# robin-karlsson0/ViT-Adapter

Hardware: AMD Instinct MI355X
Metric: images/sec ViT-Adapter-B 1024x1024 fwd+bwd (+AdamW step) (higher is better)
Workload: dtype bf16; 1 GPU; ViT-Adapter-base_det (det) 1024x1024, per-GPU batch 2, train mode, drop_path 0.3, SyncBN, step = fwd+bwd+AdamW; global_batch=2, parallelism=dp1, hip_graph=True, rccl_ranks=1, gemm_candidates_rejected=0

## Files before the change

vit-adapter_amd/_vah.py:

```python
import ctypes
import os

import torch

_HERE = os.path.dirname(os.path.abspath(__file__))
LIB_PATH = os.path.join(_HERE, 'lib', 'libvitadapter_hip.so')
ABI_VERSION = 37

if not os.path.exists(LIB_PATH):
    raise ImportError(
        'libvitadapter_hip.so is missing (%s): build it with `python vit-adapter_amd/build.py` '
        '(hipcc --offload-arch=gfx950).  There is no CPU or PyTorch fallback.' % LIB_PATH)

lib = ctypes.CDLL(LIB_PATH)

_int, _i64, _f, _p, _str, _pi64 = (ctypes.c_int, ctypes.c_int64, ctypes.c_float, ctypes.c_void_p, ctypes.c_char_p,
                                   ctypes.POINTER(ctypes.c_int64))

SIGNATURES = {
    'vah_abi_version': (_int, []),
    'vah_last_error': (_str, []),
    'vah_msda_forward_f32': (_int, [_p, _p, _p, _p, _p, _i64, _i64, _i64, _i64, _i64, _i64, _i64, _p, _p]),
    'vah_msda_forward_f64': (_int, [_p, _p, _p, _p, _p, _i64, _i64, _i64, _i64, _i64, _i64, _i64, _p, _p]),
    'vah_msda_backward_f32': (_int, [_p, _p, _p, _p, _p, _p, _i64, _i64, _i64, _i64, _i64, _i64, _i64, _p, _p, _p, _p]),
# ... 54 lines not shown
    'vah_conv_taps_nhwc_bf16': (_int, [_p, _i64, _i64, _i64, _i64, _p, _i64, _int, _p, _p, _int, _p, _i64, _i64, _i64, _i64, _int, _int, _int, _p]),
    'vah_conv3x3_dgrad_nhwc_bf16': (_int, [_p, _i64, _i64, _i64, _i64, _p, _i64, _int, _p, _i64, _i64, _p]),
    'vah_conv3x3_wgrad_ws_floats': (_i64, [_i64, _i64]),
    'vah_conv3x3_wgrad_nhwc_bf16': (_int, [_p, _i64, _i64, _i64, _i64, _p, _i64, _i64, _i64, _int, _p, _i64, _p, _p]),
    'vah_image_to_nhwc16_bf16': (_int, [_p, _i64, _i64, _i64, _p, _p]),
    'vah_patchify_bf16': (_int, [_p, _i64, _i64, _i64, _i64, _i64, _p, _p]),
    'vah_bn_nhwc_ws_floats': (_i64, [_i64]),
    'vah_bn_nhwc_stats': (_int, [_p, _i64, _i64, _p, _p, _p]),
    'vah_bn_nhwc_apply': (_int, [_p, _i64, _i64, _p, _p, _p, _p, _int, _p, _p]),
    'vah_bn_nhwc_bwd_stats': (_int, [_p, _p, _i64, _i64, _p, _p, _p, _p, _int, _p, _p, _p]),
    'vah_bn_nhwc_bwd_apply': (_int, [_p, _p, _i64, _i64, _p, _p, _p, _p, _int, _p, _p, _p, _p]),
    'vah_maxpool3s2_nhwc_fwd_bf16': (_int, [_p, _i64, _i64, _i64, _i64, _p, _p, _p]),
    'vah_maxpool3s2_nhwc_bwd_bf16': (_int, [_p, _p, _i64, _i64, _i64, _i64, _p, _p]),
    'vah_gemm_set_tuning': (_int, [_int, _int]),
    'vah_gemm_bf16': (_int, [_int, _int, _i64, _i64, _i64, _p, _i64, _p, _i64, _p, _i64, _int, _int, _p, _int, _p, _i64, _p]),
    'vah_gemm_bf16_fin': (_int, [_int, _int, _i64, _i64, _i64, _p, _i64, _p, _i64, _p, _i64, _int, _p, _i64, _p, _i64, _i64, _p, _p]),
    'vah_gemm_library_version': (_i64, []),
    'vah_gemm_rejected_candidates': (_i64, []),
    'vah_gemm_table_dump': (_i64, [_str, _i64]),
    'vah_gemm_table_load': (_int, [_str]),
    'vah_scale_residual_fwd': (_int, [_p, _p, _p, _p, _i64, _i64, _i64, _p, _p]),
    'vah_scale_residual_bwd': (_int, [_p, _p, _p, _p, _i64, _i64, _i64, _p, _p, _p, _p]),
    'vah_dwconv3x3_tokens_bf16': (_int, [_p, _p, _p, _i64, _i64, _i64, _i64, _int, _p, _p]),
    'vah_dwconv3x3_tokens_wgrad_bf16': (_int, [_p, _p, _i64, _i64, _i64, _i64, _p, _p, _p, _p]),
    'vah_prof_enable': (_int, [_int]),
    'vah_prof_filter': (_int, [_str]),
    'vah_prof_report': (_i64, [_str, _i64]),
}

ATTN_F16_TWINS = {
    'vah_attn_fwd_bf16': 'vah_attn_fwd_f16', 'vah_attn_bwd_bf16': 'vah_attn_bwd_f16',
    'vah_attn_win_fwd_bf16': 'vah_attn_win_fwd_f16', 'vah_attn_win_bwd_bf16': 'vah_attn_win_bwd_f16',
    'vah_attn_bias_fwd_bf16': 'vah_attn_bias_fwd_f16', 'vah_attn_bias_bwd_bf16': 'vah_attn_bias_bwd_f16',
    'vah_relpos_bias_build': 'vah_relpos_bias_build_f16', 'vah_relpos_bias_grad': 'vah_relpos_bias_grad_f16',
}
FUSED_F16_TWINS = {
    'vah_layernorm_fwd_f32_bf16': 'vah_layernorm_fwd_f32_f16', 'vah_layernorm_bwd_f32_bf16': 'vah_layernorm_bwd_f32_f16',
    'vah_residual_layernorm_fwd': 'vah_residual_layernorm_fwd_f16', 'vah_residual_layernorm_bwd': 'vah_residual_layernorm_bwd_f16',
    'vah_layernorm_dual_fwd': 'vah_layernorm_dual_fwd_f16', 'vah_layernorm_dual_bwd': 'vah_layernorm_dual_bwd_f16',
    'vah_scale_residual_fwd': 'vah_scale_residual_fwd_f16', 'vah_scale_residual_bwd': 'vah_scale_residual_bwd_f16',
    'vah_dwconv3x3_tokens_bf16': 'vah_dwconv3x3_tokens_f16', 'vah_dwconv3x3_tokens_wgrad_bf16': 'vah_dwconv3x3_tokens_wgrad_f16',
}
LINEAR_F16_TWINS = {
    'vah_gemm_bf16': 'vah_gemm_f16', 'vah_gemm_bf16_fin': 'vah_gemm_f16_fin',
    'vah_colsum_bf16': 'vah_colsum_f16', 'vah_colsum_bf16_partials': 'vah_colsum_f16_partials',
    'vah_gelu_bwd_bsum_bf16': 'vah_gelu_bwd_bsum_f16',
    'vah_residual_layernorm_bwd_bsum': 'vah_residual_layernorm_bwd_f16_bsum',
    'vah_scale_residual_bwd_bsum': 'vah_scale_residual_bwd_f16_bsum',
}
SPM_F16_TWINS = {
    'vah_conv_taps_nhwc_bf16': 'vah_conv_taps_nhwc_f16', 'vah_conv3x3_dgrad_nhwc_bf16': 'vah_conv3x3_dgrad_nhwc_f16',
    'vah_conv3x3_wgrad_nhwc_bf16': 'vah_conv3x3_wgrad_nhwc_f16', 'vah_image_to_nhwc16_bf16': 'vah_image_to_nhwc16_f16',
    'vah_bn_nhwc_stats': 'vah_bn_nhwc_stats_f16', 'vah_bn_nhwc_apply': 'vah_bn_nhwc_apply_f16',
    'vah_bn_nhwc_bwd_stats': 'vah_bn_nhwc_bwd_stats_f16', 'vah_bn_nhwc_bwd_apply': 'vah_bn_nhwc_bwd_apply_f16',
    'vah_maxpool3s2_nhwc_fwd_bf16': 'vah_maxpool3s2_nhwc_fwd_f16', 'vah_maxpool3s2_nhwc_bwd_bf16': 'vah_maxpool3s2_nhwc_bwd_f16',
}
TAIL_F16_TWINS = {
    'vah_bn_tail_stats': 'vah_bn_tail_stats_f16', 'vah_bn_tail_apply': 'vah_bn_tail_apply_f16',
    'vah_bn_tail_bwd_stats': 'vah_bn_tail_bwd_stats_f16', 'vah_bn_tail_bwd_apply': 'vah_bn_tail_bwd_apply_f16',
    'vah_transpose_tokens': 'vah_transpose_tokens_f16', 'vah_maxpool3s2_fwd_bf16': 'vah_maxpool3s2_fwd_f16',
    'vah_maxpool3s2_bwd_bf16': 'vah_maxpool3s2_bwd_f16', 'vah_pixel_shuffle2_bf16': 'vah_pixel_shuffle2_f16',
}
F16_TWINS = {**ATTN_F16_TWINS, **FUSED_F16_TWINS, **LINEAR_F16_TWINS, **SPM_F16_TWINS, **TAIL_F16_TWINS}

EXPORTS = tuple(SIGNATURES) + tuple(F16_TWINS.values())

_PARENT = {f16: b16 for b16, f16 in F16_TWINS.items()}
for _name in EXPORTS:
    _fn = getattr(lib, _name)
    _fn.restype, _fn.argtypes = SIGNATURES[_PARENT.get(_name, _name)]

BOX_SIGNATURES = {
    'vah_msda_fused_forward_box': (_int, [_p, _int, _p, _p, _p, _p, _int, _i64, _i64, _p, _i64, _i64, _i64, _i64, _i64, _i64, _i64, _i64, _i64,
                                          _i64, _p, _p]),
    'vah_msda_fused_backward_tiled_box': (_int, [_p, _int, _p, _p, _p, _p, _int, _i64, _i64, _p, _i64, _i64, _i64, _p, _i64, _i64, _i64, _i64, _i64,
                                                 _i64, _i64, _p, _int, _p, _p, _int, _i64, _i64, _p, _i64, _p]),
}
for _name, (_res, _args) in BOX_SIGNATURES.items():
    _fn = getattr(lib, _name)
    _fn.restype, _fn.argtypes = _res, _args

_t = [_p, _int, _i64, _i64]
GN_SIGNATURES = {
    'vah_group_norm_supported': (_int, [_i64, _i64]),
    'vah_group_norm_ws_floats': (_i64, [_i64, _i64, _i64, _i64]),
    'vah_group_norm_stats': (_int, _t + [_i64, _i64, _i64, _i64, _f, _p, _p, _p, _i64, _p]),
    'vah_group_norm_apply': (_int, _t + [_i64, _i64, _i64, _i64, _p, _p, _p, _p, _int, _p] + _t + [_p]),
    'vah_group_norm_bwd_stats': (_int, _t + _t + [_i64, _i64, _i64, _i64, _p, _p, _p, _p, _int, _p, _p, _p, _p, _i64, _p]),
    'vah_group_norm_bwd_apply': (_int, _t + _t + [_i64, _i64, _i64, _i64, _p, _p, _p, _p, _int, _p] + _t + [_p]),
}
for _name, (_res, _args) in GN_SIGNATURES.items():
    _fn = getattr(lib, _name)
    _fn.restype, _fn.argtypes = _res, _args

RESIZE_SIGNATURES = {
    'vah_resize_rows_ws_bytes': (_i64, [_i64, _i64, _i64, _i64]),
    'vah_resize_rows_forward': (_int, _t + [_i64, _i64, _i64, _i64, _i64, _i64, _int] + _t + [_p, _i64, _p]),
    'vah_resize_rows_backward': (_int, _t + [_i64, _i64, _i64, _i64, _i64, _i64, _int] + _t + [_p, _i64, _p]),
}
for _name, (_res, _args) in RESIZE_SIGNATURES.items():
    _fn = getattr(lib, _name)
    _fn.restype, _fn.argtypes = _res, _args

_mca_dims = [_i64, _i64, _i64, _i64, _i64, _f]
MCA_SIGNATURES = {
    'vah_mca_splits': (_i64, [_i64]),
    'vah_mca_ws_bytes': (_i64, [_i64, _i64, _i64, _i64]),
    'vah_mca_pack_mask': (_int, _t + [_i64, _i64, _i64, _p, _p]),
    'vah_mca_forward': (_int, _t + _t + _t + [_p] + _mca_dims + _t + [_p, _p, _i64, _p]),
    'vah_mca_backward': (_int, _t + _t + _t + [_p] + _t + _t + [_p] + _mca_dims + _t + _t + _t + [_p, _i64, _p]),
}
for _name, (_res, _args) in MCA_SIGNATURES.items():
    _fn = getattr(lib, _name)
    _fn.restype, _fn.argtypes = _res, _args

POINTS_SIGNATURES = {
    'vah_pts_sample': (_int, [_p, _int, _i64, _i64, _i64, _i64, _i64, _p, _i64, _i64, _p, _p, _i64, _p, _p]),
    'vah_pts_match_cost': (_int, [_p, _p, _p, _p, _p, _i64, _i64, _i64, _i64, _i64, _i64, _f, _f, _f, _f, _p, _p]),
}
for _name, (_res, _args) in POINTS_SIGNATURES.items():
    _fn = getattr(lib, _name)
    _fn.restype, _fn.argtypes = _res, _args

PML_SIGNATURES = {
    'vah_pml_ws_bytes': (_i64, [_i64, _i64, _i64, _i64]),
    'vah_pml_forward': (_int, [_p, _i64, _i64, _i64, _i64, _i64, _p, _int, _i64, _i64, _i64, _i64, _i64, _p, _i64, _p, _p, _i64, _f,
                               _p, _p, _p, _p, _p, _p, _i64, _p]),
    'vah_pml_backward': (_int, [_p, _p, _p, _p, _p, _p, _i64, _i64, _i64, _i64, _f, _p, _p, _i64, _p]),
}
for _name, (_res, _args) in PML_SIGNATURES.items():
    _fn = getattr(lib, _name)
    _fn.restype, _fn.argtypes = _res, _args

_pl = [_p, _i64, _i64, _i64]
SEG_SIGNATURES = {
    'vah_seg_resize_add': (_int, _pl + [_i64, _i64, _i64, _i64, _i64, _i64, _int] + _pl + [_i64, _i64, _i64, _i64, _int, _p]),
    'vah_seg_finish': (_int, _pl + [_i64, _i64, _i64, _i64, _p, _p, _int, _i64, _i64, _int, _int] + _pl + [_int, _p, _i64, _i64, _p]),
    'vah_seg_argmax': (_int, _pl + [_i64, _i64, _i64, _i64, _f, _p, _i64, _i64, _p]),
}
for _name, (_res, _args) in SEG_SIGNATURES.items():
    _fn = getattr(lib, _name)
    _fn.restype, _fn.argtypes = _res, _args

_sce = [_p, _int, _i64, _i64, _i64, _i64, _i64, _i64, _i64, _p, _i64, _i64, _i64, _i64, _int, _i64, _p]
SCE_SIGNATURES = {
    'vah_sce_ws_bytes': (_i64, [_i64, _i64, _i64, _i64, _i64, _i64]),
    'vah_sce_forward': (_int, _sce + [_p, _p, _p, _p, _i64, _p]),
    'vah_sce_backward': (_int, _sce + [_p, _p] + _pl + [_p, _i64, _p]),
}
for _name, (_res, _args) in SCE_SIGNATURES.items():
    _fn = getattr(lib, _name)
    _fn.restype, _fn.argtypes = _res, _args

if lib.vah_abi_version() != ABI_VERSION:
    raise ImportError('libvitadapter_hip.so ABI %d != binding ABI %d: rebuild the library'
                      % (lib.vah_abi_version(), ABI_VERSION))


class _NoSwitch:

    def __enter__(self):
        return None

    def __exit__(self, *exc):
        return False


_NO_SWITCH = _NoSwitch()


def on(device):
    import torch
    if device.index is None or torch.cuda.current_device() == device.index:
        return _NO_SWITCH
    return torch.cuda.device(device)


def raw_stream(device):
    import torch
    idx = device.index if device.index is not None else torch.cuda.current_device()
    try:
        return torch._C._cuda_getCurrentRawStream(idx)
    except AttributeError:
        return torch.cuda.current_stream(device).cuda_stream


def check(rc, what):
    if rc != 0:
        msg = lib.vah_last_error().decode('utf-8', 'replace')
        raise RuntimeError('%s failed (code %d): %s' % (what, rc, msg))


_SYM = {(b16, torch.bfloat16): getattr(lib, b16) for b16 in SIGNATURES}
_SYM.update(((b16, torch.float16), getattr(lib, f16)) for b16, f16 in F16_TWINS.items())


def sym(name, dtype):
    try:
        return _SYM[name, dtype]
    except KeyError:
        raise ValueError('no entry point %s for %s operands' % (name, dtype)) from None


def call(name, dtype, *args):
    fn = sym(name, dtype)
    check(fn(*args), fn.__name__)


def prof_enable(on, prefix=''):
    lib.vah_prof_filter(prefix.encode())
    lib.vah_prof_enable(1 if on else 0)


def prof_report():
    need = lib.vah_prof_report(None, 0)
    buf = ctypes.create_string_buffer(int(need) + 64)
    lib.vah_prof_report(buf, len(buf))
    out = {}
    for line in buf.value.decode().splitlines():
        name, calls, ms, nbytes, dbytes, flops = line.split()
        out[name] = dict(calls=int(calls), total_ms=float(ms), bytes=int(nbytes), def_bytes=int(dbytes),
                         flops=int(flops))
    return out


GEMM_EPI_NONE, GEMM_EPI_BIAS = 0, 1


def gemm_table_dump():
    n = lib.vah_gemm_table_dump(None, 0)
    buf = ctypes.create_string_buffer(int(n))
    lib.vah_gemm_table_dump(buf, n)
    return '#hipblaslt %d\n' % lib.vah_gemm_library_version() + buf.value.decode()


def gemm_table_load(text):
    first = text.split('\n', 1)[0].split()
    if len(first) == 2 and first[0] == '#hipblaslt' and int(first[1]) != lib.vah_gemm_library_version():
        return 0
    n = lib.vah_gemm_table_load(text.encode())
    if n < 0:
        check(n, 'gemm_table_load')
    return n
```

vit-adapter_amd/csrc/gemm.hip:

```cpp
#include <hip/hip_runtime.h>
#include <hipblaslt/hipblaslt-ext.hpp>
#include <hipblaslt/hipblaslt.h>

#include <algorithm>
#include <cstdio>
#include <cstdlib>
#include <cstring>
#include <map>
#include <memory>
#include <mutex>
#include <sstream>
#include <string>
#include <tuple>
#include <type_traits>
#include <vector>

#include "../../include/vitadapter_hip.h"
#include "common.h"

namespace vah {
namespace {

struct Key {
    int f16;
    int ta, tb, d32, epi, bias32;
    int64_t M, N, K, lda, ldb, ldd;
    bool operator<(const Key &o) const {
        return std::tie(f16, ta, tb, d32, epi, bias32, M, N, K, lda, ldb, ldd) <
               std::tie(o.f16, o.ta, o.tb, o.d32, o.epi, o.bias32, o.M, o.N, o.K, o.lda, o.ldb, o.ldd);
    }
    hipDataType t16() const { return f16 ? HIP_R_16F : HIP_R_16BF; }
};

struct Choice {
    hipblasLtMatmulAlgo_t algo;
    size_t workspace = 0;
    int index = -1;
    int split = 1;
    float us = 0.f;
    bool resolved = false;
};

struct Problem;
struct State {
    std::mutex mu;
    hipblasLtHandle_t handle = nullptr;
    std::map<Key, Choice> table;
    std::map<Key, std::shared_ptr<Problem>> problems;
    int mode = 1;
    int candidates = 32;
    void *probe = nullptr;
    int rejected = 0;
};

State &state() {
    static State s;
    return s;
}

const char *status_name(hipblasStatus_t s) {
    switch (s) {
    case HIPBLAS_STATUS_SUCCESS: return "success";
    case HIPBLAS_STATUS_NOT_INITIALIZED: return "not initialized";
    case HIPBLAS_STATUS_ALLOC_FAILED: return "alloc failed";
    case HIPBLAS_STATUS_INVALID_VALUE: return "invalid value";
    case HIPBLAS_STATUS_NOT_SUPPORTED: return "not supported";
    case HIPBLAS_STATUS_EXECUTION_FAILED: return "execution failed";
    default: return "error";
    }
}

struct Problem {
    hipblasLtMatmulDesc_t desc = nullptr;
    hipblasLtMatrixLayout_t la = nullptr, lb = nullptr, ld = nullptr;
    ~Problem() {
        if (la) hipblasLtMatrixLayoutDestroy(la);
        if (lb) hipblasLtMatrixLayoutDestroy(lb);
        if (ld) hipblasLtMatrixLayoutDestroy(ld);
        if (desc) hipblasLtMatmulDescDestroy(desc);
    }
};

struct Call {
    Key k;
    const void *A, *B, *bias;
    void *D;
    void *ws;
    size_t ws_bytes;
    hipStream_t st;
    const float *fin_part = nullptr;
    int fin_nparts = 0, fin_C = 0;
    float *fin_out = nullptr;
    const float *ref = nullptr;
};

hipblasStatus_t make_problem(const Call &c, Problem &p, int split) {
    const Key &k0 = c.k;
    Key k = k0;
    k.K = k0.K / split;
    if (split > 1) {
        k.d32 = 1;
        k.ldd = k0.N;
    }
    hipblasStatus_t s = hipblasLtMatmulDescCreate(&p.desc, HIPBLAS_COMPUTE_32F, HIP_R_32F);
    if (s != HIPBLAS_STATUS_SUCCESS) return s;
    const hipblasOperation_t op1 = k.tb ? HIPBLAS_OP_T : HIPBLAS_OP_N, op2 = k.ta ? HIPBLAS_OP_T : HIPBLAS_OP_N;
    hipblasLtMatmulDescSetAttribute(p.desc, HIPBLASLT_MATMUL_DESC_TRANSA, &op1, sizeof(op1));
    hipblasLtMatmulDescSetAttribute(p.desc, HIPBLASLT_MATMUL_DESC_TRANSB, &op2, sizeof(op2));
    s = hipblasLtMatrixLayoutCreate(&p.la, k.t16(), k.tb ? k.K : k.N, k.tb ? k.N : k.K, k.ldb);
    if (s != HIPBLAS_STATUS_SUCCESS) return s;
    s = hipblasLtMatrixLayoutCreate(&p.lb, k.t16(), k.ta ? k.M : k.K, k.ta ? k.K : k.M, k.lda);
    if (s != HIPBLAS_STATUS_SUCCESS) return s;
    s = hipblasLtMatrixLayoutCreate(&p.ld, k.d32 ? HIP_R_32F : k.t16(), k.N, k.M, k.ldd);
    if (s != HIPBLAS_STATUS_SUCCESS) return s;
    if (split > 1) {
        const int32_t batch = split;
        const int64_t sa = k.ta ? k.K * k.lda : k.K, sb = k.tb ? k.K : k.K * k.ldb, sd = k.M * k.N;
        hipblasLtMatrixLayoutSetAttribute(p.la, HIPBLASLT_MATRIX_LAYOUT_BATCH_COUNT, &batch, sizeof(batch));
        hipblasLtMatrixLayoutSetAttribute(p.lb, HIPBLASLT_MATRIX_LAYOUT_BATCH_COUNT, &batch, sizeof(batch));
        hipblasLtMatrixLayoutSetAttribute(p.ld, HIPBLASLT_MATRIX_LAYOUT_BATCH_COUNT, &batch, sizeof(batch));
        hipblasLtMatrixLayoutSetAttribute(p.la, HIPBLASLT_MATRIX_LAYOUT_STRIDED_BATCH_OFFSET, &sb, sizeof(sb));
        hipblasLtMatrixLayoutSetAttribute(p.lb, HIPBLASLT_MATRIX_LAYOUT_STRIDED_BATCH_OFFSET, &sa, sizeof(sa));
        hipblasLtMatrixLayoutSetAttribute(p.ld, HIPBLASLT_MATRIX_LAYOUT_STRIDED_BATCH_OFFSET, &sd, sizeof(sd));
    }
    uint32_t epi = HIPBLASLT_EPILOGUE_DEFAULT;
    switch (k.epi) {
    case VAH_GEMM_EPI_NONE: break;
    case VAH_GEMM_EPI_BIAS: epi = HIPBLASLT_EPILOGUE_BIAS; break;
    default: return HIPBLAS_STATUS_INVALID_VALUE;
    }
    hipblasLtMatmulDescSetAttribute(p.desc, HIPBLASLT_MATMUL_DESC_EPILOGUE, &epi, sizeof(epi));
    if (c.bias) {
        hipblasLtMatmulDescSetAttribute(p.desc, HIPBLASLT_MATMUL_DESC_BIAS_POINTER, &c.bias, sizeof(c.bias));
        const int32_t bt = k.bias32 ? HIP_R_32F : k.t16();
        hipblasLtMatmulDescSetAttribute(p.desc, HIPBLASLT_MATMUL_DESC_BIAS_DATA_TYPE, &bt, sizeof(bt));
    }
    return HIPBLAS_STATUS_SUCCESS;
}

size_t partial_bytes(const Key &k, int split) {
    return split > 1 ? ((size_t)split * k.M * k.N * sizeof(float) + 255) / 256 * 256 : 0;
}

template <int G, bool FIRST>
__device__ __forceinline__ void add_slices(const float *__restrict__ p, int64_t MN, float4 &acc) {
    float4 v[G];
#pragma unroll
    for (int u = 0; u < G; ++u) v[u] = *reinterpret_cast<const float4 *>(p + u * MN);
#pragma unroll
    for (int u = 0; u < G; ++u) {
        if (FIRST && u == 0) {
            acc = v[0];
        } else {
            acc.x += v[u].x;
            acc.y += v[u].y;
            acc.z += v[u].z;
            acc.w += v[u].w;
        }
    }
}

template <typename OT>
__global__ __launch_bounds__(256) void reduce_splits(const float *__restrict__ part, int split, int64_t MN, int N,
                                                     int64_t ldd, int vec, OT *__restrict__ out, int reduce_blocks,
                                                     const float *__restrict__ fin_part, int fin_nparts, int fin_C,
                                                     float *__restrict__ fin_out) {
    if ((int)blockIdx.x >= reduce_blocks) {
        __shared__ float s_acc[8][32];
        const int col = threadIdx.x & 31, pl = threadIdx.x >> 5;
        const int k = ((int)blockIdx.x - reduce_blocks) * 32 + col;
        float a8[8] = {0.f, 0.f, 0.f, 0.f, 0.f, 0.f, 0.f, 0.f};
        if (k < fin_C) {
            int p = pl;
            for (; p + 56 < fin_nparts; p += 64) {
#pragma unroll
                for (int u = 0; u < 8; ++u) a8[u] += fin_part[(int64_t)(p + 8 * u) * fin_C + k];
            }
            for (; p < fin_nparts; p += 8) a8[0] += fin_part[(int64_t)p * fin_C + k];
        }
        s_acc[pl][col] = ((a8[0] + a8[1]) + (a8[2] + a8[3])) + ((a8[4] + a8[5]) + (a8[6] + a8[7]));
        __syncthreads();
        if (pl == 0 && k < fin_C) {
            float t = 0.f;
#pragma unroll
            for (int u = 0; u < 8; ++u) t += s_acc[u][col];
            fin_out[k] = t;
        }
        return;
    }
    for (int64_t i = ((int64_t)blockIdx.x * 256 + threadIdx.x) * 4; i < MN; i += (int64_t)reduce_blocks * 1024) {
        const float *p = part + i;
        float4 acc;
        int s;
        if (split >= 8) {
            add_slices<8, true>(p, MN, acc);
            s = 8;
        } else if (split >= 4) {
            add_slices<4, true>(p, MN, acc);
            s = 4;
        } else if (split >= 2) {
            add_slices<2, true>(p, MN, acc);
            s = 2;
        } else {
            add_slices<1, true>(p, MN, acc);
            s = 1;
        }
        for (; s + 8 <= split; s += 8) add_slices<8, false>(p + s * MN, MN, acc);
        if (s + 4 <= split) {
            add_slices<4, false>(p + s * MN, MN, acc);
            s += 4;
        }
        if (s + 2 <= split) {
            add_slices<2, false>(p + s * MN, MN, acc);
            s += 2;
        }
        if (s < split) add_slices<1, false>(p + s * MN, MN, acc);
        int64_t o = i;
        if (ldd != N) {
            const int64_t row = i / N;
            o = row * ldd + (i - row * N);
        }
        typedef OT ov4 __attribute__((ext_vector_type(4)));
        ov4 r;
        r[0] = (OT)acc.x;
        r[1] = (OT)acc.y;
        r[2] = (OT)acc.z;
        r[3] = (OT)acc.w;
        if (vec) {
            *reinterpret_cast<ov4 *>(out + o) = r;
        } else {
            out[o] = r[0];
            out[o + 1] = r[1];
            out[o + 2] = r[2];
            out[o + 3] = r[3];
        }
    }
}

template <typename T>
__global__ __launch_bounds__(256) void ref_gemm(int ta, int tb, int M, int N, int K, const T *__restrict__ A, int64_t lda,
                                                const T *__restrict__ B, int64_t ldb, const void *__restrict__ bias,
                                                int bias32, float *__restrict__ ref) {
    __shared__ float sa[16][65], sb[16][65];
    const int tm = blockIdx.y * 64, tn = blockIdx.x * 64;
    const int tx = threadIdx.x & 15, ty = threadIdx.x >> 4;
    float acc[4][4] = {};
    for (int k0 = 0; k0 < K; k0 += 16) {
        for (int i = threadIdx.x; i < 1024; i += 256) {
            const int ma = ta ? (i & 63) : (i >> 4), ka = ta ? (i >> 6) : (i & 15);
            const int m = tm + ma, k = k0 + ka;
            sa[ka][ma] = (m < M && k < K) ? (float)(ta ? A[(int64_t)k * lda + m] : A[(int64_t)m * lda + k]) : 0.f;
            const int nb = tb ? (i >> 4) : (i & 63), kb = tb ? (i & 15) : (i >> 6);
            const int n = tn + nb, k2 = k0 + kb;
            sb[kb][nb] = (n < N && k2 < K) ? (float)(tb ? B[(int64_t)n * ldb + k2] : B[(int64_t)k2 * ldb + n]) : 0.f;
        }
        __syncthreads();
#pragma unroll
        for (int kk = 0; kk < 16; ++kk) {
            float a[4], b[4];
#pragma unroll
            for (int i = 0; i < 4; ++i) {
                a[i] = sa[kk][ty * 4 + i];
                b[i] = sb[kk][tx * 4 + i];
            }
#pragma unroll
            for (int i = 0; i < 4; ++i)
#pragma unroll
                for (int j = 0; j < 4; ++j) acc[i][j] += a[i] * b[j];
        }
        __syncthreads();
    }
    for (int i = 0; i < 4; ++i)
        for (int j = 0; j < 4; ++j) {
            const int m = tm + ty * 4 + i, n = tn + tx * 4 + j;
            if (m >= M || n >= N) continue;
            float v = acc[i][j];
            if (bias) v += bias32 ? ((const float *)bias)[n] : (float)((const T *)bias)[n];
            ref[(int64_t)m * N + n] = v;
        }
}

template <typename OT>
__global__ __launch_bounds__(256) void full_compare(const OT *__restrict__ D, int64_t ldd, int64_t MN, int N,
                                                    const float *__restrict__ ref, unsigned *__restrict__ out2) {
    float md = 0.f, mr = 0.f;
    bool bad = false;
    for (int64_t i = (int64_t)blockIdx.x * 256 + threadIdx.x; i < MN; i += (int64_t)gridDim.x * 256) {
        const int64_t r = i / N;
        float v = (float)D[r * ldd + (i - r * N)];
        const float w = ref[i];
        if constexpr (std::is_same<OT, _Float16>::value) {
            if (isinf(v)) v = v == (float)(_Float16)w ? w : copysignf(65520.f, v);
        }
        const float d = fabsf(v - w);
        bad = bad || !(d == d);
        md = fmaxf(md, d == d ? d : 0.f);
        mr = fmaxf(mr, fabsf(w));
    }
    if (bad || md > 0.f) atomicMax(out2, __float_as_uint(bad ? INFINITY : md));
    if (mr > 0.f) atomicMax(out2 + 1, __float_as_uint(mr));
}

float *make_reference(const Call &c) {
    const Key &k = c.k;
    if (k.M > (64 << 16) || k.N > (int64_t)INT32_MAX || k.K > (int64_t)INT32_MAX) return nullptr;
    float *ref = nullptr;
    if (hipMalloc((void **)&ref, (size_t)k.M * k.N * sizeof(float)) != hipSuccess) return nullptr;
    const dim3 grid((unsigned)((k.N + 63) / 64), (unsigned)((k.M + 63) / 64));
    if (k.f16)
        hipLaunchKernelGGL(ref_gemm<_Float16>, grid, dim3(256), 0, c.st, k.ta, k.tb, (int)k.M, (int)k.N, (int)k.K,
                           (const _Float16 *)c.A, k.lda, (const _Float16 *)c.B, k.ldb, c.bias, k.bias32, ref);
    else
        hipLaunchKernelGGL(ref_gemm<__bf16>, grid, dim3(256), 0, c.st, k.ta, k.tb, (int)k.M, (int)k.N, (int)k.K,
                           (const __bf16 *)c.A, k.lda, (const __bf16 *)c.B, k.ldb, c.bias, k.bias32, ref);
    if (hipGetLastError() != hipSuccess) {
        (void)hipFree(ref);
        return nullptr;
    }
    return ref;
}

hipblasStatus_t run(State &S, const Call &c, Problem &p, const hipblasLtMatmulAlgo_t &algo, size_t ws_need, int split);

bool validate(State &S, const Call &c, Problem &p, const hipblasLtMatmulAlgo_t &algo, size_t ws_need, int split, const float *ref) {
    if (!ref) return true;
    if (!S.probe && hipMalloc(&S.probe, 2 * sizeof(unsigned)) != hipSuccess) return true;
    unsigned *out2 = (unsigned *)S.probe;
    const Key &k = c.k;
    const size_t es = k.d32 ? 4 : 2;
    const int64_t MN = k.M * k.N;
    const unsigned blocks = (unsigned)std::min<int64_t>(4096, (MN + 255) / 256);
    if (c.ws_bytes && hipMemsetAsync(c.ws, 0x01, c.ws_bytes, c.st) != hipSuccess) return true;
    for (int pass = 0; pass < 2; ++pass) {
        if (hipMemsetAsync(out2, 0, 8, c.st) != hipSuccess) return true;
        if (hipMemset2DAsync(c.D, (size_t)k.ldd * es, 0xFF, (size_t)k.N * es, (size_t)k.M, c.st) != hipSuccess) return true;
        if (run(S, c, p, algo, ws_need, split) != HIPBLAS_STATUS_SUCCESS) return false;
        if (k.d32)
            hipLaunchKernelGGL(full_compare<float>, dim3(blocks), dim3(256), 0, c.st, (const float *)c.D, k.ldd, MN, (int)k.N, ref, out2);
        else if (k.f16)
            hipLaunchKernelGGL(full_compare<_Float16>, dim3(blocks), dim3(256), 0, c.st, (const _Float16 *)c.D, k.ldd, MN, (int)k.N, ref, out2);
        else
            hipLaunchKernelGGL(full_compare<__bf16>, dim3(blocks), dim3(256), 0, c.st, (const __bf16 *)c.D, k.ldd, MN, (int)k.N, ref, out2);
        float h[2] = {0.f, 0.f};
        if (hipMemcpyAsync(h, out2, 8, hipMemcpyDeviceToHost, c.st) != hipSuccess || hipStreamSynchronize(c.st) != hipSuccess) return true;
        if (!(h[0] <= 0.015625f * fmaxf(h[1], 1e-20f))) return false;
    }
    return true;
}

hipblasStatus_t run(State &S, const Call &c, Problem &p, const hipblasLtMatmulAlgo_t &algo, size_t ws_need, int split) {
    const size_t pb = partial_bytes(c.k, split);
    if (pb + ws_need > c.ws_bytes) return HIPBLAS_STATUS_ALLOC_FAILED;
    const float alpha = 1.f, beta = 0.f;
    void *d = split > 1 ? c.ws : c.D;
    const hipblasStatus_t s = hipblasLtMatmul(S.handle, p.desc, &alpha, c.B, p.la, c.A, p.lb, &beta, d, p.ld, d, p.ld, &algo,
                                              (char *)c.ws + pb, c.ws_bytes - pb, c.st);
    if (s != HIPBLAS_STATUS_SUCCESS) return s;
    const bool fin = c.fin_part != nullptr;
    if (split == 1 && !fin) return s;
    const int64_t MN = c.k.M * c.k.N;
    const unsigned rblocks = split > 1 ? (unsigned)std::min<int64_t>(8192, (MN / 4 + 255) / 256) : 0u;
    const unsigned fblocks = fin ? (unsigned)((c.fin_C + 31) / 32) : 0u;
    const int vec = c.k.N % 4 == 0 && c.k.ldd % 4 == 0 && (uintptr_t)c.D % (c.k.d32 ? 16 : 8) == 0;
    if (c.k.d32)
        hipLaunchKernelGGL(reduce_splits<float>, dim3(rblocks + fblocks), dim3(256), 0, c.st, (const float *)c.ws, split, MN,
                           (int)c.k.N, c.k.ldd, vec, (float *)c.D, (int)rblocks, c.fin_part, c.fin_nparts, c.fin_C, c.fin_out);
    else if (c.k.f16)
        hipLaunchKernelGGL(reduce_splits<_Float16>, dim3(rblocks + fblocks), dim3(256), 0, c.st, (const float *)c.ws, split, MN,
                           (int)c.k.N, c.k.ldd, vec, (_Float16 *)c.D, (int)rblocks, c.fin_part, c.fin_nparts, c.fin_C, c.fin_out);
    else
        hipLaunchKernelGGL(reduce_splits<__bf16>, dim3(rblocks + fblocks), dim3(256), 0, c.st, (const float *)c.ws, split, MN,
                           (int)c.k.N, c.k.ldd, vec, (__bf16 *)c.D, (int)rblocks, c.fin_part, c.fin_nparts, c.fin_C, c.fin_out);
    return HIPBLAS_STATUS_SUCCESS;
}

float time_algo(State &S, const Call &c, Problem &p, const hipblasLtMatmulAlgo_t &algo, size_t ws_need, int split,
                hipEvent_t e0, hipEvent_t e1, int reps) {
    if (run(S, c, p, algo, ws_need, split) != HIPBLAS_STATUS_SUCCESS) return -1.f;
    if (hipEventRecord(e0, c.st) != hipSuccess) return -1.f;
    for (int i = 0; i < reps; ++i)
        if (run(S, c, p, algo, ws_need, split) != HIPBLAS_STATUS_SUCCESS) return -1.f;
    if (hipEventRecord(e1, c.st) != hipSuccess || hipEventSynchronize(e1) != hipSuccess) return -1.f;
    float ms = 0.f;
    if (hipEventElapsedTime(&ms, e0, e1) != hipSuccess) return -1.f;
    return ms * 1000.f / reps;
}

hipblasStatus_t choose_for_split(State &S, const Call &c, Problem &p, int split, bool must_time, Choice &out) {
    const size_t pb = partial_bytes(c.k, split);
    if (pb >= c.ws_bytes) return HIPBLAS_STATUS_ALLOC_FAILED;
    const size_t ws_lib = c.ws_bytes - pb;
    std::vector<hipblasLtMatmulHeuristicResult_t> cand;
    const bool d32 = split > 1 || c.k.d32;
    if (S.mode == 2) {
        std::vector<hipblasLtMatmulHeuristicResult_t> all;
        const Key &k = c.k;
        hipblasStatus_t s = hipblaslt_ext::getAllAlgos(
            S.handle, hipblaslt_ext::GemmType::HIPBLASLT_GEMM, k.tb ? HIPBLAS_OP_T : HIPBLAS_OP_N,
            k.ta ? HIPBLAS_OP_T : HIPBLAS_OP_N, k.t16(), k.t16(), d32 ? HIP_R_32F : k.t16(),
            d32 ? HIP_R_32F : k.t16(), HIPBLAS_COMPUTE_32F, all);
        if (s == HIPBLAS_STATUS_SUCCESS)
            for (auto &r : all) {
                size_t need = 0;
                const float one = 1.f, zero = 0.f;
                if (hipblaslt_ext::matmulIsAlgoSupported(S.handle, p.desc, &one, p.la, p.lb, &zero, p.ld, p.ld, r.algo,
                                                         need) == HIPBLAS_STATUS_SUCCESS &&
                    need <= ws_lib) {
                    r.workspaceSize = need;
                    cand.push_back(r);
                }
            }
    }
    if (cand.empty()) {
        hipblasLtMatmulPreference_t pref = nullptr;
        hipblasStatus_t s = hipblasLtMatmulPreferenceCreate(&pref);
        if (s != HIPBLAS_STATUS_SUCCESS) return s;
        const uint64_t wsmax = ws_lib;
        hipblasLtMatmulPreferenceSetAttribute(pref, HIPBLASLT_MATMUL_PREF_MAX_WORKSPACE_BYTES, &wsmax, sizeof(wsmax));
        const int want = S.mode == 0 ? 1 : (split > 1 ? std::min(S.candidates, 12) : S.candidates);
        cand.resize(want);
        int got = 0;
        s = hipblasLtMatmulAlgoGetHeuristic(S.handle, p.desc, p.la, p.lb, p.ld, p.ld, pref, want, cand.data(), &got);
        hipblasLtMatmulPreferenceDestroy(pref);
        if (s != HIPBLAS_STATUS_SUCCESS) return s;
        cand.resize(std::max(got, 0));
        if (cand.empty()) return HIPBLAS_STATUS_NOT_SUPPORTED;
    }
    out.split = split;
    if (S.mode == 0 || (cand.size() == 1 && !must_time)) {
        if (!validate(S, c, p, cand[0].algo, cand[0].workspaceSize, split, c.ref)) {
            ++S.rejected;
            return HIPBLAS_STATUS_EXECUTION_FAILED;
        }
        out.algo = cand[0].algo;
        out.workspace = cand[0].workspaceSize;
        out.index = hipblaslt_ext::getIndexFromAlgo(out.algo);
        out.resolved = true;
        return HIPBLAS_STATUS_SUCCESS;
    }
    hipEvent_t e0, e1;
    if (hipEventCreate(&e0) != hipSuccess || hipEventCreate(&e1) != hipSuccess) return HIPBLAS_STATUS_ALLOC_FAILED;
    float best = -1.f;
    size_t best_i = 0;
    std::vector<std::pair<float, size_t>> timed;
    for (size_t i = 0; i < cand.size(); ++i) {
        const float us = time_algo(S, c, p, cand[i].algo, cand[i].workspaceSize, split, e0, e1, 3);
        if (us > 0.f) timed.emplace_back(us, i);
    }
    std::sort(timed.begin(), timed.end());
    int looked = 0;
    for (size_t j = 0; j < timed.size() && looked < 4; ++j) {
        const size_t i = timed[j].second;
        if (!validate(S, c, p, cand[i].algo, cand[i].workspaceSize, split, c.ref)) {
            ++S.rejected;
            continue;
        }
        ++looked;
        const float us = time_algo(S, c, p, cand[i].algo, cand[i].workspaceSize, split, e0, e1, 20);
        if (us > 0.f && (best < 0.f || us < best)) {
            best = us;
            best_i = i;
        }
    }
    (void)hipEventDestroy(e0);
    (void)hipEventDestroy(e1);
    if (best < 0.f) return HIPBLAS_STATUS_EXECUTION_FAILED;
    out.algo = cand[best_i].algo;
    out.workspace = cand[best_i].workspaceSize;
    out.index = hipblaslt_ext::getIndexFromAlgo(out.algo);
    out.us = best;
    out.resolved = true;
    return HIPBLAS_STATUS_SUCCESS;
}

std::vector<int> split_candidates(const State &S, const Call &c) {
    std::vector<int> v{1};
    const Key &k = c.k;
    if (S.mode == 0 || c.bias || k.K < 4096 || k.N % 4) return v;
    const int64_t tiles = ((k.M + 127) / 128) * ((k.N + 127) / 128);
    if (tiles >= 256) return v;
    for (int s = 2; s <= 64; s *= 2) {
        if (k.K % s || k.K / s < 512 || tiles * s > 4096) break;
        if (partial_bytes(k, s) + (8u << 20) > c.ws_bytes) break;
        v.push_back(s);
    }
    return v;
}

hipblasStatus_t choose(State &S, const Call &call, Choice &out) {
    Call c = call;
    c.fin_part = nullptr;
    const std::vector<int> splits = split_candidates(S, c);
    float *ref = S.mode != 0 ? make_reference(c) : nullptr;
    c.ref = ref;
    hipblasStatus_t last = HIPBLAS_STATUS_NOT_SUPPORTED;
    bool have = false;
    for (int split : splits) {
        Problem p;
        hipblasStatus_t s = make_problem(c, p, split);
        Choice ch;
        if (s == HIPBLAS_STATUS_SUCCESS) s = choose_for_split(S, c, p, split, splits.size() > 1, ch);
        if (s != HIPBLAS_STATUS_SUCCESS) {
            last = s;
            continue;
        }
        if (!have || (ch.us > 0.f && ch.us < out.us)) out = ch;
        have = true;
    }
    if (ref) {
        (void)hipStreamSynchronize(c.st);
        (void)hipFree(ref);
    }
    return have ? HIPBLAS_STATUS_SUCCESS : last;
}

bool resolve(State &S, const Call &c, Problem &p, Choice &ch) {
    std::vector<int> idx{ch.index};
    std::vector<hipblasLtMatmulHeuristicResult_t> res;
    if (ch.index < 0 || hipblaslt_ext::getAlgosFromIndex(S.handle, idx, res) != HIPBLAS_STATUS_SUCCESS || res.empty())
        return false;
    size_t need = 0;
    const float one = 1.f, zero = 0.f;
    if (hipblaslt_ext::matmulIsAlgoSupported(S.handle, p.desc, &one, p.la, p.lb, &zero, p.ld, p.ld, res[0].algo, need) !=
            HIPBLAS_STATUS_SUCCESS || need + partial_bytes(c.k, ch.split) > c.ws_bytes)
        return false;
    Call cc = c;
    cc.fin_part = nullptr;
    float *ref = make_reference(cc);
    const bool ok = validate(S, cc, p, res[0].algo, need, ch.split, ref);
    if (ref) {
        (void)hipStreamSynchronize(c.st);
        (void)hipFree(ref);
    }
    if (!ok) {
        ++S.rejected;
        return false;
    }
    ch.algo = res[0].algo;
    ch.workspace = need;
    ch.resolved = true;
    return true;
}

}
}

extern "C" {

int vah_gemm_set_tuning(int mode, int candidates) {
    using namespace vah;
    clear_error();
    if (mode < 0 || mode > 2 || candidates < 1 || candidates > 4096) return fail(VAH_E_SHAPE, "vah_gemm_set_tuning: bad arguments");
    State &S = state();
    std::lock_guard<std::mutex> lock(S.mu);
    S.mode = mode;
    S.candidates = candidates;
    return VAH_OK;
}

static int gemm_impl(const char *fn, int f16, int trans_a, int trans_b, int64_t M, int64_t N, int64_t K, const void *A, int64_t lda,
                     const void *B, int64_t ldb, void *D, int64_t ldd, int d_is_f32, int epilogue, const void *bias,
                     int bias_is_f32, void *workspace, int64_t workspace_bytes, void *stream, const float *fin_part,
                     int64_t fin_nparts, int64_t fin_C, float *fin_out);

int vah_gemm_bf16(int trans_a, int trans_b, int64_t M, int64_t N, int64_t K, const void *A, int64_t lda,
                  const void *B, int64_t ldb, void *D, int64_t ldd, int d_is_f32, int epilogue, const void *bias,
                  int bias_is_f32, void *workspace, int64_t workspace_bytes, void *stream) {
    return gemm_impl("vah_gemm_bf16", 0, trans_a, trans_b, M, N, K, A, lda, B, ldb, D, ldd, d_is_f32, epilogue, bias, bias_is_f32,
                     workspace, workspace_bytes, stream, nullptr, 0, 0, nullptr);
}

int vah_gemm_bf16_fin(int trans_a, int trans_b, int64_t M, int64_t N, int64_t K, const void *A, int64_t lda,
                      const void *B, int64_t ldb, void *D, int64_t ldd, int d_is_f32, void *workspace,
                      int64_t workspace_bytes, const float *fin_part, int64_t fin_nparts, int64_t fin_C, float *fin_out,
                      void *stream) {
    using namespace vah;
    if (!fin_part || !fin_out || fin_nparts < 1 || fin_C < 1 || fin_nparts > (1 << 20) || fin_C > (1 << 24)) {
        clear_error();
        return fail(VAH_E_SHAPE, "vah_gemm_bf16_fin: bad finalize job");
    }
    return gemm_impl("vah_gemm_bf16_fin", 0, trans_a, trans_b, M, N, K, A, lda, B, ldb, D, ldd, d_is_f32, VAH_GEMM_EPI_NONE, nullptr,
                     0, workspace, workspace_bytes, stream, fin_part, fin_nparts, fin_C, fin_out);
}

int vah_gemm_f16(int trans_a, int trans_b, int64_t M, int64_t N, int64_t K, const void *A, int64_t lda,
                 const void *B, int64_t ldb, void *D, int64_t ldd, int d_is_f32, int epilogue, const void *bias,
                 int bias_is_f32, void *workspace, int64_t workspace_bytes, void *stream) {
    return gemm_impl("vah_gemm_f16", 1, trans_a, trans_b, M, N, K, A, lda, B, ldb, D, ldd, d_is_f32, epilogue, bias, bias_is_f32,
                     workspace, workspace_bytes, stream, nullptr, 0, 0, nullptr);
}

int vah_gemm_f16_fin(int trans_a, int trans_b, int64_t M, int64_t N, int64_t K, const void *A, int64_t lda,
                     const void *B, int64_t ldb, void *D, int64_t ldd, int d_is_f32, void *workspace,
                     int64_t workspace_bytes, const float *fin_part, int64_t fin_nparts, int64_t fin_C, float *fin_out,
                     void *stream) {
    using namespace vah;
    if (!fin_part || !fin_out || fin_nparts < 1 || fin_C < 1 || fin_nparts > (1 << 20) || fin_C > (1 << 24)) {
        clear_error();
        return fail(VAH_E_SHAPE, "vah_gemm_f16_fin: bad finalize job");
    }
    return gemm_impl("vah_gemm_f16_fin", 1, trans_a, trans_b, M, N, K, A, lda, B, ldb, D, ldd, d_is_f32, VAH_GEMM_EPI_NONE, nullptr,
                     0, workspace, workspace_bytes, stream, fin_part, fin_nparts, fin_C, fin_out);
}

static int gemm_impl(const char *fn, int f16, int trans_a, int trans_b, int64_t M, int64_t N, int64_t K, const void *A, int64_t lda,
                     const void *B, int64_t ldb, void *D, int64_t ldd, int d_is_f32, int epilogue, const void *bias,
                     int bias_is_f32, void *workspace, int64_t workspace_bytes, void *stream, const float *fin_part,
                     int64_t fin_nparts, int64_t fin_C, float *fin_out) {
    using namespace vah;
    clear_error();
    if (M < 0 || N < 0 || K < 0) return fail(VAH_E_SHAPE, "%s: negative dimension", fn);
    if (M == 0 || N == 0) return VAH_OK;
    if (K == 0) return fail(VAH_E_SHAPE, "%s: K = 0 (zero-fill the output instead)", fn);
    if (!A || !B || !D) return fail(VAH_E_NULL, "%s: null pointer", fn);
    if (lda < (trans_a ? M : K) || ldb < (trans_b ? K : N) || ldd < N) return fail(VAH_E_SHAPE, "%s: leading dimension too small", fn);
    if (epilogue != VAH_GEMM_EPI_NONE && epilogue != VAH_GEMM_EPI_BIAS) return fail(VAH_E_SHAPE, "%s: unknown epilogue", fn);
    if ((epilogue == VAH_GEMM_EPI_BIAS) != (bias != nullptr)) return fail(VAH_E_NULL, "%s: bias does not match the epilogue", fn);
    if (workspace_bytes < 0 || (workspace_bytes > 0 && !workspace)) return fail(VAH_E_NULL, "%s: workspace", fn);
    if (f16 && bias && !bias_is_f32 && d_is_f32)
        return fail(VAH_E_UNSUPPORTED, "%s: an fp16 bias into an fp32 output is not supported (pass the bias in fp32)", fn);

    State &S = state();
    std::lock_guard<std::mutex> lock(S.mu);
    if (!S.handle) {
        const hipblasStatus_t s = hipblasLtCreate(&S.handle);
        if (s != HIPBLAS_STATUS_SUCCESS) return fail(VAH_E_UNSUPPORTED, "%s: hipblasLtCreate: %s", fn, status_name(s));
    }
    Call c{{f16 ? 1 : 0, trans_a ? 1 : 0, trans_b ? 1 : 0, d_is_f32 ? 1 : 0, epilogue, bias_is_f32 ? 1 : 0, M, N, K, lda, ldb, ldd},
           A, B, bias, D, workspace, (size_t)workspace_bytes, (hipStream_t)stream};
    c.fin_part = fin_part;
    c.fin_nparts = (int)fin_nparts;
    c.fin_C = (int)fin_C;
    c.fin_out = fin_out;
    hipblasStatus_t s = HIPBLAS_STATUS_SUCCESS;
    const char *role = f16 ? (trans_a ? (fin_part ? "gemm_tn_fin_f16" : "gemm_tn_f16") : (trans_b ? "gemm_nt_f16" : "gemm_nn_f16"))
                           : (trans_a ? (fin_part ? "gemm_tn_fin" : "gemm_tn") : (trans_b ? "gemm_nt" : "gemm_nn"));
    LaunchScope scope(role, (M * K + K * N) * 2 + M * N * (d_is_f32 ? 4 : 2), c.st, 0, 2 * M * N * K);
    auto it = S.table.find(c.k);
    if (it != S.table.end() && !it->second.resolved) {
        Problem p;
        const int split = it->second.split;
        if (split < 1 || K % split || make_problem(c, p, split) != HIPBLAS_STATUS_SUCCESS ||
            partial_bytes(c.k, split) >= c.ws_bytes || !resolve(S, c, p, it->second)) {
            S.table.erase(it);
            S.problems.erase(c.k);
            it = S.table.end();
        }
    }
    if (it == S.table.end()) {
        Choice ch;
        s = choose(S, c, ch);
        if (s != HIPBLAS_STATUS_SUCCESS)
            return fail(VAH_E_UNSUPPORTED, "%s: no algorithm for %lldx%lldx%lld ta=%d tb=%d f32=%d epi=%d: %s", fn,
                        (long long)M, (long long)N, (long long)K, trans_a, trans_b, d_is_f32, epilogue, status_name(s));
        it = S.table.emplace(c.k, ch).first;
    }
    std::shared_ptr<Problem> &pp = S.problems[c.k];
    if (!pp) {
        pp = std::make_shared<Problem>();
        s = make_problem(c, *pp, it->second.split);
        if (s != HIPBLAS_STATUS_SUCCESS) {
            S.problems.erase(c.k);
            return fail(VAH_E_UNSUPPORTED, "%s: descriptor: %s", fn, status_name(s));
        }
    } else if (c.bias) {
        hipblasLtMatmulDescSetAttribute(pp->desc, HIPBLASLT_MATMUL_DESC_BIAS_POINTER, &c.bias, sizeof(c.bias));
    }
    Problem &p = *pp;
    s = run(S, c, p, it->second.algo, it->second.workspace, it->second.split);
    if (s != HIPBLAS_STATUS_SUCCESS) return fail(VAH_E_UNSUPPORTED, "%s: hipblasLtMatmul: %s", fn, status_name(s));
    return check_launch(fn);
}

int64_t vah_gemm_rejected_candidates(void) {
    vah::State &S = vah::state();
    std::lock_guard<std::mutex> lock(S.mu);
    return S.rejected;
}

int64_t vah_gemm_library_version(void) {
    using namespace vah;
    clear_error();
    State &S = state();
    std::lock_guard<std::mutex> lock(S.mu);
    if (!S.handle && hipblasLtCreate(&S.handle) != HIPBLAS_STATUS_SUCCESS)
        return fail(VAH_E_UNSUPPORTED, "vah_gemm_library_version: hipblasLtCreate failed");
    int v = 0;
    if (hipblasLtGetVersion(S.handle, &v) != HIPBLAS_STATUS_SUCCESS)
        return fail(VAH_E_UNSUPPORTED, "vah_gemm_library_version: hipblasLtGetVersion failed");
    return v;
}

int64_t vah_gemm_table_dump(char *buf, int64_t cap) {
    using namespace vah;
    State &S = state();
    std::lock_guard<std::mutex> lock(S.mu);
    std::ostringstream os;
    for (auto &kv : S.table) {
        const Key &k = kv.first;
        if (k.f16) os << "f16 ";
        os << k.ta << ' ' << k.tb << ' ' << k.d32 << ' ' << k.epi << ' ' << k.bias32 << ' ' << k.M << ' ' << k.N << ' '
           << k.K << ' ' << k.lda << ' ' << k.ldb << ' ' << k.ldd << ' ' << kv.second.index << ' ' << kv.second.split << ' '
           << kv.second.us << '\n';
    }
    const std::string t = os.str();
    if (buf && cap > 0) {
        const size_t n = std::min<size_t>(t.size(), (size_t)cap - 1);
        memcpy(buf, t.data(), n);
        buf[n] = 0;
    }
    return (int64_t)t.size() + 1;
}

int vah_gemm_table_load(const char *text) {
    using namespace vah;
    clear_error();
    if (!text) return fail(VAH_E_NULL, "vah_gemm_table_load: null text");
    State &S = state();
    std::lock_guard<std::mutex> lock(S.mu);
    S.problems.clear();
    std::istringstream is(text);
    std::string line;
    int n = 0;
    while (std::getline(is, line)) {
        if (line.empty() || line[0] == '#') continue;
        std::istringstream ls(line);
        Key k;
        Choice ch;
        k.f16 = line.compare(0, 4, "f16 ") == 0;
        if (k.f16) ls.ignore(4);
        if (!(ls >> k.ta >> k.tb >> k.d32 >> k.epi >> k.bias32 >> k.M >> k.N >> k.K >> k.lda >> k.ldb >> k.ldd >> ch.index >> ch.split >> ch.us))
            return fail(VAH_E_SHAPE, "vah_gemm_table_load: malformed line '%s'", line.c_str());
        ch.resolved = false;
        S.table[k] = ch;
        ++n;
    }
    return n;
}

}
```

vit-adapter_amd/csrc/tail_ops.hip:

```cpp
#include <hip/hip_runtime.h>

#include <algorithm>
#include <cstdint>
#include <cstdlib>
#include <cstring>

#include "../../include/vitadapter_hip.h"
#include "common.h"
#include "elem16.h"

namespace vah {
namespace {

constexpr int kTilePx = 8192;
constexpr int kTailParts = 512;

struct Operands {
    const void *a, *b;
    const float *x;
    int a_bf16, b_bf16, scale;
    int C, H, W, Hl, Wl;
    int rows_per_block, chunks;
    int relu, y_bf16, dy_bf16;
    const float *shift;
    unsigned quad_magic;
    unsigned oct_magic, lo_magic;
};

struct Tap {
    int i0, i1;
    float w1;
};

__device__ __forceinline__ Tap tap_of(int d, int n_lo, int s) {
    const int sh1 = 32 - __builtin_clz((unsigned)s);
    const int n = max(2 * d + 1 - s, 0);
    Tap t;
    t.i0 = min(n >> sh1, n_lo - 1);
    t.i1 = min(t.i0 + 1, n_lo - 1);
    t.w1 = (float)(n & (2 * s - 1)) * (0.5f / (float)s);
    return t;
}

struct Raw4 {
    uint32_t w0, w1, w2, w3;
};

__device__ __forceinline__ Raw4 load_raw(const void *p, int64_t idx, int is_bf16) {
    Raw4 r;
    r.w0 = r.w1 = r.w2 = r.w3 = 0u;
    if (is_bf16) {
        const uint2 v = *reinterpret_cast<const uint2 *>(reinterpret_cast<const uint16_t *>(p) + idx);
        r.w0 = v.x;
        r.w1 = v.y;
    } else {
        const uint4 v = *reinterpret_cast<const uint4 *>(reinterpret_cast<const float *>(p) + idx);
        r.w0 = v.x;
        r.w1 = v.y;
        r.w2 = v.z;
        r.w3 = v.w;
    }
    return r;
}

template <typename T>
__device__ __forceinline__ float4 widen4(uint32_t w0, uint32_t w1);
template <>
__device__ __forceinline__ float4 widen4<__bf16>(uint32_t w0, uint32_t w1) {
    return make_float4(__uint_as_float(w0 << 16), __uint_as_float(w0 & 0xffff0000u), __uint_as_float(w1 << 16),
                       __uint_as_float(w1 & 0xffff0000u));
}
template <>
__device__ __forceinline__ float4 widen4<_Float16>(uint32_t w0, uint32_t w1) {
    const f16x2 lo = __builtin_bit_cast(f16x2, w0), hi = __builtin_bit_cast(f16x2, w1);
    return make_float4((float)lo[0], (float)lo[1], (float)hi[0], (float)hi[1]);
}

template <typename T>
__device__ __forceinline__ float4 decode(const Raw4 &r, int is_bf16) {
    const float4 h = widen4<T>(r.w0, r.w1);
    const float4 f = make_float4(__uint_as_float(r.w0), __uint_as_float(r.w1), __uint_as_float(r.w2),
                                 __uint_as_float(r.w3));
    return is_bf16 ? h : f;
}

template <typename T>
__device__ __forceinline__ void store4(void *p, int64_t idx, int is_bf16, float4 v) {
    if (is_bf16) {
        vec4<T> o;
        o[0] = (T)v.x;
        o[1] = (T)v.y;
        o[2] = (T)v.z;
        o[3] = (T)v.w;
        *reinterpret_cast<vec4<T> *>(reinterpret_cast<T *>(p) + idx) = o;
    } else {
        *reinterpret_cast<float4 *>(reinterpret_cast<float *>(p) + idx) = v;
    }
}

template <typename T>
__device__ __forceinline__ float4 sum4(const Operands &o, int64_t plane, int y, int x4, const void *dy = nullptr,
                                       Raw4 *dy_raw = nullptr) {
    const int64_t idx = (plane * o.H + y) * o.W + x4;
    const Raw4 ra = load_raw(o.a, idx, o.a_bf16);
    Raw4 rb;
    rb.w0 = rb.w1 = rb.w2 = rb.w3 = 0u;
    if (o.b) rb = load_raw(o.b, idx, o.b_bf16);
    if (dy) *dy_raw = load_raw(dy, idx, o.dy_bf16);
    float sft = 0.f;
    if (o.shift) sft = o.shift[plane % o.C];
    float4 xs = make_float4(0.f, 0.f, 0.f, 0.f);
    float c0[4] = {0.f, 0.f, 0.f, 0.f}, c1[4] = {0.f, 0.f, 0.f, 0.f};
    Tap ty;
    ty.i0 = ty.i1 = 0;
    ty.w1 = 0.f;
    int nx0 = 0, bcol = 0;
    const int sc = o.scale, sh1 = 32 - __builtin_clz((unsigned)sc), mask = 2 * sc - 1;
    if (o.x) {
        const float *xp = o.x + plane * o.Hl * o.Wl;
        if (sc == 1) {
            xs = *reinterpret_cast<const float4 *>(xp + (int64_t)y * o.Wl + x4);
        } else {
            ty = tap_of(y, o.Hl, sc);
            const float *r0 = xp + (int64_t)ty.i0 * o.Wl, *r1 = xp + (int64_t)ty.i1 * o.Wl;
            nx0 = 2 * x4 + 1 - sc;
            bcol = nx0 >> sh1;
#pragma unroll
            for (int j = 0; j < 4; ++j) {
                const int cj = min(max(bcol + j, 0), o.Wl - 1);
                c0[j] = r0[cj];
                c1[j] = r1[cj];
            }
        }
    }
    __builtin_amdgcn_sched_barrier(0);
    float4 t = decode<T>(ra, o.a_bf16);
    const float4 vb = decode<T>(rb, o.b_bf16);
    t.x += sft + vb.x;
    t.y += sft + vb.y;
    t.z += sft + vb.z;
    t.w += sft + vb.w;
    if (o.x) {
        if (sc == 1) {
            t.x += xs.x;
            t.y += xs.y;
            t.z += xs.z;
            t.w += xs.w;
        } else {
            float u[4];
            if (sc == 4) {
                const float t0 = c0[0] + 0.625f * (c0[1] - c0[0]), b0 = c1[0] + 0.625f * (c1[1] - c1[0]);
                const float t1 = c0[0] + 0.875f * (c0[1] - c0[0]), b1 = c1[0] + 0.875f * (c1[1] - c1[0]);
                const float t2 = c0[1] + 0.125f * (c0[2] - c0[1]), b2 = c1[1] + 0.125f * (c1[2] - c1[1]);
                const float t3 = c0[1] + 0.375f * (c0[2] - c0[1]), b3 = c1[1] + 0.375f * (c1[2] - c1[1]);
                u[0] = t0 + ty.w1 * (b0 - t0);
                u[1] = t1 + ty.w1 * (b1 - t1);
                u[2] = t2 + ty.w1 * (b2 - t2);
                u[3] = t3 + ty.w1 * (b3 - t3);
            } else if (sc == 2) {
                const float t0 = c0[0] + 0.75f * (c0[1] - c0[0]), b0 = c1[0] + 0.75f * (c1[1] - c1[0]);
// ... 388 lines not shown
    const int64_t plane = blockIdx.x / o.chunks;
    const int chunk = blockIdx.x % o.chunks;
    const int c = (int)(plane % o.C);
    const int r0 = chunk * o.rows_per_block, r1 = min(o.H, r0 + o.rows_per_block);
    const int wv4 = o.W >> 2;
    const float add = (SHIFT ? o.shift[c] : 0.f) + 0.f;
    const float sc = rstd[c] * (gamma ? gamma[c] : 1.f);
    const float sh = (beta ? beta[c] : 0.f) - mean[c] * sc;
    for (int i = threadIdx.x; i < (r1 - r0) * wv4; i += 256) {
        const int iy = (int)__umulhi((unsigned)i, o.quad_magic), yy = r0 + iy, x4 = (i - iy * wv4) * 4;
        const float4 t = sum4_form<T, A16, S>(o, plane, yy, x4, add);
        *reinterpret_cast<float4 *>(y + (plane * o.H + yy) * o.W + x4) =
            make_float4(t.x * sc + sh, t.y * sc + sh, t.z * sc + sh, t.w * sc + sh);
    }
}

template <typename T, bool A16, int S, bool SHIFT>
__global__ __launch_bounds__(256) void tail_bwd_stats_form_kernel(Operands o, const float *__restrict__ mean,
                                                                  const float *__restrict__ rstd,
                                                                  const float *__restrict__ dy, float *__restrict__ part) {
    __shared__ float s_red[4];
    const int64_t plane = blockIdx.x / o.chunks;
    const int chunk = blockIdx.x % o.chunks;
    const int c = (int)(plane % o.C);
    const int64_t n = plane / o.C;
    const int r0 = chunk * o.rows_per_block, r1 = min(o.H, r0 + o.rows_per_block);
    const int wv8 = o.W >> 3;
    const float add = (SHIFT ? o.shift[c] : 0.f) + 0.f;
    const float mu = mean[c], rs = rstd[c];
    float s1 = 0.f, s2 = 0.f;
    for (int i = threadIdx.x; i < (r1 - r0) * wv8; i += 256) {
        int yy, x8;
        item8(o, i, wv8, r0, yy, x8);
        float t[8], g[8];
        sum8<T, A16, S, true>(o, plane, yy, x8, add, dy, t, g);
        s1 += (g[0] + g[1]) + (g[2] + g[3]);
        s2 += (g[0] * (t[0] - mu) + g[1] * (t[1] - mu)) + (g[2] * (t[2] - mu) + g[3] * (t[3] - mu));
        s1 += (g[4] + g[5]) + (g[6] + g[7]);
        s2 += (g[4] * (t[4] - mu) + g[5] * (t[5] - mu)) + (g[6] * (t[6] - mu) + g[7] * (t[7] - mu));
    }
    s1 = block_sum(s1, s_red);
    s2 = block_sum(s2, s_red) * rs;
    if (threadIdx.x == 0) {
        float *row = part + (n * o.chunks + chunk) * 2 * o.C;
        row[c] = s1;
        row[o.C + c] = s2;
    }
}

template <int S, bool TILE>
__device__ __forceinline__ float adjoint_taps(const float *p, int stride, int j, int n_lo, int lo, int hi) {
    float acc = 0.f;
#pragma unroll
    for (int u = 0; u < 2 * S; ++u) {
        const float wc = (float)(u < S ? 2 * u + 1 : 4 * S - 2 * u - 1) * (0.5f / (float)S);
        const int pos = S * j - S / 2 + u;
        const bool inner = u >= S / 2 && u < S + S / 2;
        const bool at_border = u < S ? j == 0 : j == n_lo - 1;
        const float w = inner && at_border ? 1.f : wc;
        if (!TILE && inner) {
            acc = __builtin_fmaf(w, p[pos * stride], acc);
        } else {
            const bool there = (inner || !at_border) && (!TILE || (pos >= lo && pos < hi));
            const int at = TILE ? min(max(pos, lo), hi - 1) - lo : (u < S ? max(pos, 0) : min(pos, S * n_lo - 1));
            const float sum = __builtin_fmaf(w, p[at * stride], acc);
            acc = there ? sum : acc;
        }
    }
    return acc;
}

template <typename T, bool A16, int S, bool SHIFT>
__global__ __launch_bounds__(256) void tail_bwd_apply_form_kernel(Operands o, const float *__restrict__ mean,
                                                                  const float *__restrict__ rstd,
                                                                  const float *__restrict__ gamma,
                                                                  const float *__restrict__ dy,
                                                                  const float *__restrict__ mdy,
                                                                  const float *__restrict__ mdyx, void *__restrict__ da,
                                                                  float *__restrict__ dxlo) {
    extern __shared__ __attribute__((aligned(16))) float s_tile[];
    const int64_t plane = blockIdx.x / o.chunks;
    const int chunk = blockIdx.x % o.chunks;
    const int c = (int)(plane % o.C);
    const int r0 = chunk * o.rows_per_block, r1 = min(o.H, r0 + o.rows_per_block);
    const int rows = r1 - r0;
    const int wv8 = o.W >> 3;
    const float add = (SHIFT ? o.shift[c] : 0.f) + 0.f;
    const float mu = mean[c], rs = rstd[c];
    const float k = rs * (gamma ? gamma[c] : 1.f), m1 = mdy[c], m2 = mdyx[c];
    for (int i = threadIdx.x; i < rows * wv8; i += 256) {
        int yy, x8;
        item8(o, i, wv8, r0, yy, x8);
        const int64_t idx = (plane * o.H + yy) * o.W + x8;
        float t[8], g[8], d[8];
        sum8<T, A16, S, true>(o, plane, yy, x8, add, dy, t, g);
#pragma unroll
        for (int e = 0; e < 8; ++e) d[e] = k * (g[e] - m1 - (t[e] - mu) * rs * m2);
        const float4 d0 = make_float4(d[0], d[1], d[2], d[3]), d1 = make_float4(d[4], d[5], d[6], d[7]);
        if constexpr (A16) {
            vec8<T> v;
#pragma unroll
            for (int e = 0; e < 8; ++e) v[e] = (T)d[e];
            *reinterpret_cast<vec8<T> *>(reinterpret_cast<T *>(da) + idx) = v;
        } else {
            *reinterpret_cast<float4 *>(reinterpret_cast<float *>(da) + idx) = d0;
            *reinterpret_cast<float4 *>(reinterpret_cast<float *>(da) + idx + 4) = d1;
        }
        float *lo = S == 1 ? dxlo + idx : s_tile + (yy - r0) * o.W + x8;
        *reinterpret_cast<float4 *>(lo) = d0;
        *reinterpret_cast<float4 *>(lo + 4) = d1;
    }
    if constexpr (S > 1) {
        __syncthreads();
        float *s_col = s_tile + rows * o.W;
        const int Wl = o.Wl;
        for (int i = threadIdx.x; i < rows * Wl; i += 256) {
            const int ry = (int)__umulhi((unsigned)i, o.lo_magic), j = i - ry * Wl;
            s_col[i] = adjoint_taps<S, false>(s_tile + ry * o.W, 1, j, Wl, 0, o.W);
        }
        __syncthreads();
        const int i_lo = tap_of(r0, o.Hl, S).i0, i_hi = tap_of(r1 - 1, o.Hl, S).i1;
        float *out = dxlo + plane * o.Hl * Wl;
        for (int i = threadIdx.x; i < (i_hi - i_lo + 1) * Wl; i += 256) {
            const int ly = (int)__umulhi((unsigned)i, o.lo_magic), li = i_lo + ly, j = i - ly * Wl;
            const float acc = adjoint_taps<S, true>(s_col + j, Wl, li, o.Hl, r0, r1);
            const bool owned = S * (li - 1) >= r0 && S * (li + 2) - 1 <= r1 - 1;
            if (owned || (li == 0 && r0 == 0 && S * (li + 2) - 1 <= r1 - 1) ||
                (li == o.Hl - 1 && r1 == o.H && S * (li - 1) >= r0))
                out[(int64_t)li * Wl + j] += acc;
            else
                atomicAdd(out + (int64_t)li * Wl + j, acc);
        }
    }
}

__global__ __launch_bounds__(256) void tail_finalize(const float *__restrict__ part, int nparts, int K,
                                                     float *__restrict__ out) {
    __shared__ float s_acc[8][32];
    const int col = threadIdx.x & 31, pl = threadIdx.x >> 5;
    const int k = blockIdx.x * 32 + col;
    float acc = 0.f;
    if (k < K)
        for (int p = pl; p < nparts; p += 8) acc += part[(int64_t)p * K + k];
    s_acc[pl][col] = acc;
    __syncthreads();
    if (pl == 0 && k < K) {
        float t = 0.f;
#pragma unroll
        for (int u = 0; u < 8; ++u) t += s_acc[u][col];
        out[k] = t;
    }
}

__global__ __launch_bounds__(256) void bn_finalize_kernel(const float *__restrict__ sums, int C, float eps, float momentum,
                                                          float *__restrict__ running_mean,
                                                          float *__restrict__ running_var, float *__restrict__ mean,
                                                          float *__restrict__ rstd) {
    const int c = blockIdx.x * 256 + threadIdx.x;
    if (c >= C) return;
    const float count = sums[2 * C];
    const float mu = sums[c] / count;
    const float var = nanmax(sums[C + c] / count - mu * mu, 0.f);
    mean[c] = mu;
    rstd[c] = rsqrtf(var + eps);
    if (running_mean) {
        running_mean[c] = (1.f - momentum) * running_mean[c] + momentum * mu;
        running_var[c] = (1.f - momentum) * running_var[c] + momentum * var * (count / fmaxf(count - 1.f, 1.f));
    }
}

template <typename E, bool TO_PLANES>
__global__ __launch_bounds__(256) void transpose_tokens_kernel(const void *__restrict__ src, void *__restrict__ dst,
                                                               int64_t T_total, int64_t t0, int T, int C,
                                                               int planes_bf16, const float *__restrict__ vec) {
    __shared__ float tile[32][33];
    const int b = blockIdx.z;
    const int tt = blockIdx.x * 32, cc = blockIdx.y * 32;
    const int lx = threadIdx.x & 31, ly = threadIdx.x >> 5;
    const int64_t tok_off = ((int64_t)b * T_total + t0) * C;
    const int64_t plane_base = (int64_t)b * C * T;
    if (TO_PLANES) {
        const float *tok = reinterpret_cast<const float *>(src) + tok_off;
        float v4[4];
#pragma unroll
        for (int u = 0; u < 4; ++u)
            v4[u] = tok[(int64_t)min(tt + ly + 8 * u, T - 1) * C + min(cc + lx, C - 1)];
        __builtin_amdgcn_sched_barrier(0);
#pragma unroll
        for (int u = 0; u < 4; ++u) tile[ly + 8 * u][lx] = (tt + ly + 8 * u < T && cc + lx < C) ? v4[u] : 0.f;
        __syncthreads();
#pragma unroll
        for (int r = ly; r < 32; r += 8)
            if (cc + r < C && tt + lx < T) {
                const int64_t o = plane_base + (int64_t)(cc + r) * T + tt + lx;
                if (planes_bf16) reinterpret_cast<E *>(dst)[o] = (E)tile[lx][r];
                else reinterpret_cast<float *>(dst)[o] = tile[lx][r];
            }
    } else {
        float v4[4];
        int64_t o4[4];
#pragma unroll
        for (int u = 0; u < 4; ++u)
            o4[u] = plane_base + (int64_t)min(cc + ly + 8 * u, C - 1) * T + min(tt + lx, T - 1);
        if (planes_bf16) {
#pragma unroll
            for (int u = 0; u < 4; ++u) v4[u] = (float)reinterpret_cast<const E *>(src)[o4[u]];
        } else {
#pragma unroll
            for (int u = 0; u < 4; ++u) v4[u] = reinterpret_cast<const float *>(src)[o4[u]];
        }
        __builtin_amdgcn_sched_barrier(0);
#pragma unroll
        for (int u = 0; u < 4; ++u) tile[ly + 8 * u][lx] = (cc + ly + 8 * u < C && tt + lx < T) ? v4[u] : 0.f;
        __syncthreads();
        float *tok = reinterpret_cast<float *>(dst) + tok_off;
        const float add = (vec && cc + lx < C) ? vec[cc + lx] : 0.f;
#pragma unroll
        for (int r = ly; r < 32; r += 8)
            if (tt + r < T && cc + lx < C) tok[(int64_t)(tt + r) * C + cc + lx] = tile[lx][r] + add;
    }
}

template <typename T>
__global__ __launch_bounds__(256) void maxpool3s2_fwd_kernel(const T *__restrict__ x, int H, int W, int Ho, int Wo,
                                                             T *__restrict__ y, unsigned char *__restrict__ idx) {
    const int ox = blockIdx.x * 64 + (threadIdx.x & 63);
    const int oy = blockIdx.y * 4 + (threadIdx.x >> 6);
    if (ox >= Wo || oy >= Ho) return;
    const int64_t plane = blockIdx.z;
    const T *xp = x + plane * H * W;
    float win[9];
#pragma unroll
    for (int k = 0; k < 9; ++k) {
        const int iy = min(max(2 * oy - 1 + k / 3, 0), H - 1), ix = min(max(2 * ox - 1 + k % 3, 0), W - 1);
        win[k] = (float)xp[(int64_t)iy * W + ix];
    }
    __builtin_amdgcn_sched_barrier(0);
    float best = -INFINITY;
    int pos = 0;
    bool any = false;
#pragma unroll
    for (int k = 0; k < 9; ++k) {
        const int iy = 2 * oy - 1 + k / 3, ix = 2 * ox - 1 + k % 3;
        const bool in = iy >= 0 && iy < H && ix >= 0 && ix < W;
        const float v = win[k];
        if (in && (!any || v > best || v != v)) {
            best = v;
            pos = k;
            any = true;
        }
    }
    const int64_t o = (plane * Ho + oy) * Wo + ox;
    y[o] = (T)best;
    idx[o] = (unsigned char)pos;
}

template <typename T>
__global__ __launch_bounds__(256) void maxpool3s2_bwd_kernel(const T *__restrict__ gy,
                                                             const unsigned char *__restrict__ idx, int H, int W, int Ho,
                                                             int Wo, T *__restrict__ gx) {
    const int ix0 = (blockIdx.x * 64 + (threadIdx.x & 63)) * 8;
    const int iy = blockIdx.y * 4 + (threadIdx.x >> 6);
    if (ix0 >= W || iy >= H) return;
    const int64_t plane = blockIdx.z;
    const T *gp = gy + plane * Ho * Wo;
    const unsigned char *ip = idx + plane * Ho * Wo;
    float acc[8] = {0.f, 0.f, 0.f, 0.f, 0.f, 0.f, 0.f, 0.f};
    const int oy0 = iy >> 1, oy1 = (iy + 1) >> 1;
    const int oxb = ix0 >> 1;
    float g[2][5];
    int p[2][5];
#pragma unroll
    for (int a = 0; a < 2; ++a) {
        const int oyc = min(a == 0 ? oy0 : oy1, Ho - 1);
#pragma unroll
        for (int u = 0; u < 5; ++u) {
            const int64_t at = (int64_t)oyc * Wo + min(oxb + u, Wo - 1);
            g[a][u] = (float)gp[at];
            p[a][u] = (int)ip[at];
        }
    }
    __builtin_amdgcn_sched_barrier(0);
#pragma unroll
    for (int a = 0; a < 2; ++a) {
        const int oy = a == 0 ? oy0 : oy1;
        if ((a == 1 && oy1 == oy0) || oy >= Ho) continue;
        const int ky3 = (iy - (2 * oy - 1)) * 3;
#pragma unroll
        for (int u = 0; u < 5; ++u)
            if (oxb + u >= Wo) p[a][u] = -1;
#pragma unroll
        for (int e = 0; e < 8; ++e) {
            const int u0 = e >> 1;
            const int kx0 = (e & 1) ? 2 : 1;
            if (p[a][u0] == ky3 + kx0) acc[e] += g[a][u0];
            if (e & 1)
                if (p[a][u0 + 1] == ky3 + 0) acc[e] += g[a][u0 + 1];
        }
    }
    T *o = gx + (plane * H + iy) * (int64_t)W + ix0;
    if (ix0 + 8 <= W && (W & 7) == 0) {
        vec8<T> v;
#pragma unroll
        for (int e = 0; e < 8; ++e) v[e] = (T)acc[e];
        *reinterpret_cast<vec8<T> *>(o) = v;
    } else {
        for (int e = 0; e < 8 && ix0 + e < W; ++e) o[e] = (T)acc[e];
    }
}

constexpr size_t kTailLdsMax = 150 * 1024;

int plan_tail(const char *fn, Operands &o, int has_x, int scale, int64_t N, int64_t C, int64_t H, int64_t W) {
    if (N < 1 || C < 1 || H < 1 || W < 4 || W % 4 || W > kTilePx) return fail(VAH_E_SHAPE, "%s: bad shape", fn);
    if (scale != 1 && scale != 2 && scale != 4 && scale != 8) return fail(VAH_E_SHAPE, "%s: scale must be 1, 2, 4 or 8", fn);
    if (has_x && (H % scale || W % scale || (W / scale) % 4)) return fail(VAH_E_SHAPE, "%s: H, W not multiples of the scale", fn);
    if (N * C * H * W >= ((int64_t)1 << 40)) return fail(VAH_E_SHAPE, "%s: too large", fn);
    if (N > kTailParts) return fail(VAH_E_SHAPE, "%s: batch %lld above %d", fn, (long long)N, kTailParts);
    o.scale = scale;
    o.C = (int)C;
// ... 210 lines not shown

template <typename T>
int transpose_tokens_launch(const char *fn, const void *src, int64_t B, int64_t T_total, int64_t t0, int64_t Tn, int64_t C,
                            void *dst, int to_planes, int planes_bf16, const float *vec, void *stream) {
    clear_error();
    if (B < 0 || T_total < 0 || t0 < 0 || Tn < 0 || t0 + Tn > T_total || C < 1 || B > 65535 || C > 65535 * 32 || Tn >= ((int64_t)1 << 31))
        return fail(VAH_E_SHAPE, "%s: bad dims", fn);
    if (B == 0 || Tn == 0) return VAH_OK;
    if (!src || !dst) return fail(VAH_E_NULL, "%s: null pointer", fn);
    if (to_planes && vec) return fail(VAH_E_UNSUPPORTED, "%s: vec only applies to planes -> tokens", fn);
    const dim3 grid((unsigned)((Tn + 31) / 32), (unsigned)((C + 31) / 32), (unsigned)B);
    hipStream_t st = (hipStream_t)stream;
    LaunchScope scope(tname<T>("transpose_tokens", "transpose_tokens_f16"), B * Tn * C * (4 + (planes_bf16 ? 2 : 4)), st);
    if (to_planes)
        hipLaunchKernelGGL((transpose_tokens_kernel<T, true>), grid, dim3(256), 0, st, src, dst, T_total, t0, (int)Tn, (int)C,
                           planes_bf16, vec);
    else
        hipLaunchKernelGGL((transpose_tokens_kernel<T, false>), grid, dim3(256), 0, st, src, dst, T_total, t0, (int)Tn, (int)C,
                           planes_bf16, vec);
    return check_launch(fn);
}

template <typename T>
int maxpool_fwd_launch(const char *fn, const void *x, int64_t planes, int64_t H, int64_t W, void *y, void *idx, void *stream) {
    clear_error();
    if (planes < 0 || H < 1 || W < 1 || H > (1 << 20) || W > (1 << 20)) return fail(VAH_E_SHAPE, "%s: bad dims", fn);
    const int64_t Ho = (H - 1) / 2 + 1, Wo = (W - 1) / 2 + 1, total = planes * Ho * Wo;
    if (total == 0) return VAH_OK;
    if (!x || !y || !idx) return fail(VAH_E_NULL, "%s: null pointer", fn);
    hipStream_t st = (hipStream_t)stream;
    LaunchScope scope(tname<T>("maxpool_fwd", "maxpool_fwd_f16"), planes * (H * W * 2 + Ho * Wo * 3), st);
    if (planes > 65535 || (Ho + 3) / 4 > 65535) return fail(VAH_E_SHAPE, "%s: too many planes / rows", fn);
    hipLaunchKernelGGL(maxpool3s2_fwd_kernel<T>, dim3((unsigned)((Wo + 63) / 64), (unsigned)((Ho + 3) / 4), (unsigned)planes),
                       dim3(256), 0, st, (const T *)x, (int)H, (int)W, (int)Ho, (int)Wo, (T *)y, (unsigned char *)idx);
    return check_launch(fn);
}

template <typename T>
int maxpool_bwd_launch(const char *fn, const void *gy, const void *idx, int64_t planes, int64_t H, int64_t W, void *gx,
                       void *stream) {
    clear_error();
    if (planes < 0 || H < 1 || W < 1 || H > (1 << 20) || W > (1 << 20)) return fail(VAH_E_SHAPE, "%s: bad dims", fn);
    const int64_t Ho = (H - 1) / 2 + 1, Wo = (W - 1) / 2 + 1, total = planes * H * W;
    if (total == 0) return VAH_OK;
    if (!gy || !idx || !gx) return fail(VAH_E_NULL, "%s: null pointer", fn);
    hipStream_t st = (hipStream_t)stream;
    LaunchScope scope(tname<T>("maxpool_bwd", "maxpool_bwd_f16"), planes * (H * W * 2 + Ho * Wo * 3), st);
    if (planes > 65535 || (H + 3) / 4 > 65535) return fail(VAH_E_SHAPE, "%s: too many planes / rows", fn);
    if ((uintptr_t)gx % 16) return fail(VAH_E_ALIGN, "%s: misaligned", fn);
    hipLaunchKernelGGL(maxpool3s2_bwd_kernel<T>, dim3((unsigned)((W + 511) / 512), (unsigned)((H + 3) / 4), (unsigned)planes),
                       dim3(256), 0, st, (const T *)gy, (const unsigned char *)idx, (int)H, (int)W, (int)Ho, (int)Wo, (T *)gx);
    return check_launch(fn);
}

template <typename T>
int pixel_shuffle2_launch(const char *fn, const void *src, int64_t B, int64_t C, int64_t h, int64_t w, void *dst, int inverse,
                          const void *add, void *stream) {
    clear_error();
    if (B < 0 || C < 1 || h < 1 || w < 8 || w % 8) return fail(VAH_E_SHAPE, "%s: w must be a multiple of 8", fn);
    if (B == 0) return VAH_OK;
    if (!src || !dst) return fail(VAH_E_NULL, "%s: null pointer", fn);
    if (((uintptr_t)src | (uintptr_t)dst) % 16) return fail(VAH_E_ALIGN, "%s: 16-byte alignment", fn);
    const int64_t items = B * C * 2 * h * (w / 8);
    hipStream_t st = (hipStream_t)stream;
    LaunchScope scope(tname<T>("pixel_shuffle2", "pixel_shuffle2_f16"), B * C * 4 * h * w * 4, st);
    if (add && (inverse || (uintptr_t)add % 16)) return fail(VAH_E_SHAPE, "%s: add is a forward-only, 16-byte aligned operand", fn);
    if (inverse)
        hipLaunchKernelGGL((pixel_shuffle2_kernel<T, true>), dim3((unsigned)((items + 255) / 256)), dim3(256), 0, st, (const T *)src,
                           (T *)dst, (const T *)nullptr, (int)B, (int)C, (int)h, (int)w, items);
    else
        hipLaunchKernelGGL((pixel_shuffle2_kernel<T, false>), dim3((unsigned)((items + 255) / 256)), dim3(256), 0, st, (const T *)src,
                           (T *)dst, (const T *)add, (int)B, (int)C, (int)h, (int)w, items);
    return check_launch(fn);
}

}
}

extern "C" {

int64_t vah_bn_tail_ws_floats(int64_t C) { return (int64_t)vah::kTailParts * 2 * C; }

int vah_bn_tail_supported(int64_t N, int64_t C, int64_t H, int64_t W, int scale, int has_x) {
    using namespace vah;
    clear_error();
    Operands o;
    return plan_tail("vah_bn_tail_supported", o, has_x != 0, scale, N, C, H, W) == VAH_OK ? 1 : 0;
}

int vah_bn_tail_stats(const void *a, int a_bf16, const void *b, int b_bf16, const float *x, int scale, int64_t N,
                      int64_t C, int64_t H, int64_t W, const float *shift, float *sums, float *ws, void *stream) {
    return vah::tail_stats_launch<__bf16>("vah_bn_tail_stats", a, a_bf16, b, b_bf16, x, scale, N, C, H, W, shift, sums, ws, stream);
}
int vah_bn_tail_stats_f16(const void *a, int a_f16, const void *b, int b_f16, const float *x, int scale, int64_t N,
                          int64_t C, int64_t H, int64_t W, const float *shift, float *sums, float *ws, void *stream) {
    return vah::tail_stats_launch<_Float16>("vah_bn_tail_stats_f16", a, a_f16, b, b_f16, x, scale, N, C, H, W, shift, sums, ws, stream);
}

int vah_bn_tail_apply(const void *a, int a_bf16, const void *b, int b_bf16, const float *x, int scale, int64_t N,
                      int64_t C, int64_t H, int64_t W, const float *mean, const float *rstd, const float *gamma,
                      const float *beta, int relu, const float *shift, void *y, int y_bf16, void *stream) {
    return vah::tail_apply_launch<__bf16>("vah_bn_tail_apply", a, a_bf16, b, b_bf16, x, scale, N, C, H, W, mean, rstd, gamma, beta,
                                          relu, shift, y, y_bf16, stream);
}
int vah_bn_tail_apply_f16(const void *a, int a_f16, const void *b, int b_f16, const float *x, int scale, int64_t N,
                          int64_t C, int64_t H, int64_t W, const float *mean, const float *rstd, const float *gamma,
                          const float *beta, int relu, const float *shift, void *y, int y_f16, void *stream) {
    return vah::tail_apply_launch<_Float16>("vah_bn_tail_apply_f16", a, a_f16, b, b_f16, x, scale, N, C, H, W, mean, rstd, gamma,
                                            beta, relu, shift, y, y_f16, stream);
}

int vah_bn_tail_bwd_stats(const void *a, int a_bf16, const void *b, int b_bf16, const float *x, int scale, int64_t N,
                          int64_t C, int64_t H, int64_t W, const float *mean, const float *rstd, const float *gamma,
                          const float *beta, int relu, const float *shift, const void *dy, int dy_bf16, float *sums,
                          float *ws, void *stream) {
    return vah::tail_bwd_stats_launch<__bf16>("vah_bn_tail_bwd_stats", a, a_bf16, b, b_bf16, x, scale, N, C, H, W, mean, rstd, gamma,
                                              beta, relu, shift, dy, dy_bf16, sums, ws, stream);
}
int vah_bn_tail_bwd_stats_f16(const void *a, int a_f16, const void *b, int b_f16, const float *x, int scale, int64_t N,
                              int64_t C, int64_t H, int64_t W, const float *mean, const float *rstd, const float *gamma,
                              const float *beta, int relu, const float *shift, const void *dy, int dy_f16, float *sums,
                              float *ws, void *stream) {
    return vah::tail_bwd_stats_launch<_Float16>("vah_bn_tail_bwd_stats_f16", a, a_f16, b, b_f16, x, scale, N, C, H, W, mean, rstd,
                                                gamma, beta, relu, shift, dy, dy_f16, sums, ws, stream);
}

int vah_bn_tail_bwd_apply(const void *a, int a_bf16, const void *b, int b_bf16, const float *x, int scale, int64_t N,
                          int64_t C, int64_t H, int64_t W, const float *mean, const float *rstd, const float *gamma,
                          const float *beta, int relu, const float *shift, const void *dy, int dy_bf16, const float *mdy,
                          const float *mdyx, void *da, void *db, float *dxlo, void *stream) {
    return vah::tail_bwd_apply_launch<__bf16>("vah_bn_tail_bwd_apply", a, a_bf16, b, b_bf16, x, scale, N, C, H, W, mean, rstd, gamma,
                                              beta, relu, shift, dy, dy_bf16, mdy, mdyx, da, db, dxlo, stream);
}
int vah_bn_tail_bwd_apply_f16(const void *a, int a_f16, const void *b, int b_f16, const float *x, int scale, int64_t N,
                              int64_t C, int64_t H, int64_t W, const float *mean, const float *rstd, const float *gamma,
                              const float *beta, int relu, const float *shift, const void *dy, int dy_f16, const float *mdy,
                              const float *mdyx, void *da, void *db, float *dxlo, void *stream) {
    return vah::tail_bwd_apply_launch<_Float16>("vah_bn_tail_bwd_apply_f16", a, a_f16, b, b_f16, x, scale, N, C, H, W, mean, rstd,
                                                gamma, beta, relu, shift, dy, dy_f16, mdy, mdyx, da, db, dxlo, stream);
}

int vah_bn_finalize_stats(const float *sums, int64_t C, float eps, float momentum, float *running_mean,
                          float *running_var, float *mean, float *rstd, void *stream) {
    using namespace vah;
    clear_error();
    const char *fn = "vah_bn_finalize_stats";
    if (C < 1) return fail(VAH_E_SHAPE, "%s: bad C", fn);
    if (!sums || !mean || !rstd || ((running_mean != nullptr) != (running_var != nullptr))) return fail(VAH_E_NULL, "%s: null pointer", fn);
    hipLaunchKernelGGL(bn_finalize_kernel, dim3((unsigned)((C + 255) / 256)), dim3(256), 0, (hipStream_t)stream, sums, (int)C, eps,
                       momentum, running_mean, running_var, mean, rstd);
    return check_launch(fn);
}

int vah_transpose_tokens(const void *src, int64_t B, int64_t T_total, int64_t t0, int64_t T, int64_t C, void *dst,
                         int to_planes, int planes_bf16, const float *vec, void *stream) {
    return vah::transpose_tokens_launch<__bf16>("vah_transpose_tokens", src, B, T_total, t0, T, C, dst, to_planes, planes_bf16, vec,
                                                stream);
}
int vah_transpose_tokens_f16(const void *src, int64_t B, int64_t T_total, int64_t t0, int64_t T, int64_t C, void *dst,
                             int to_planes, int planes_f16, const float *vec, void *stream) {
    return vah::transpose_tokens_launch<_Float16>("vah_transpose_tokens_f16", src, B, T_total, t0, T, C, dst, to_planes, planes_f16,
                                                  vec, stream);
}

int vah_maxpool3s2_fwd_bf16(const void *x, int64_t planes, int64_t H, int64_t W, void *y, void *idx, void *stream) {
    return vah::maxpool_fwd_launch<__bf16>("vah_maxpool3s2_fwd_bf16", x, planes, H, W, y, idx, stream);
}
int vah_maxpool3s2_fwd_f16(const void *x, int64_t planes, int64_t H, int64_t W, void *y, void *idx, void *stream) {
    return vah::maxpool_fwd_launch<_Float16>("vah_maxpool3s2_fwd_f16", x, planes, H, W, y, idx, stream);
}

int vah_maxpool3s2_bwd_bf16(const void *gy, const void *idx, int64_t planes, int64_t H, int64_t W, void *gx, void *stream) {
    return vah::maxpool_bwd_launch<__bf16>("vah_maxpool3s2_bwd_bf16", gy, idx, planes, H, W, gx, stream);
}
int vah_maxpool3s2_bwd_f16(const void *gy, const void *idx, int64_t planes, int64_t H, int64_t W, void *gx, void *stream) {
    return vah::maxpool_bwd_launch<_Float16>("vah_maxpool3s2_bwd_f16", gy, idx, planes, H, W, gx, stream);
}

int vah_pixel_shuffle2_bf16(const void *src, int64_t B, int64_t C, int64_t h, int64_t w, void *dst, int inverse, const void *add,
                            void *stream) {
    return vah::pixel_shuffle2_launch<__bf16>("vah_pixel_shuffle2_bf16", src, B, C, h, w, dst, inverse, add, stream);
}
int vah_pixel_shuffle2_f16(const void *src, int64_t B, int64_t C, int64_t h, int64_t w, void *dst, int inverse, const void *add,
                           void *stream) {
    return vah::pixel_shuffle2_launch<_Float16>("vah_pixel_shuffle2_f16", src, B, C, h, w, dst, inverse, add, stream);
}

}
```

vit-adapter_amd/vitadapter/fused.py:

```python
import math
import os

import torch
import torch.nn.functional as F

import _vah

ENABLED = {'pair_core': True, 'layer_norm': True, 'residual': True, 'residual_ln': True, 'dwconv': True, 'linear': True, 'bn_tail': True,
           'bn_relu': True, 'bias_fold': True, 'keep_feat': True, 'maps': True, 'maps_in': True, 'linear_pair': True, 'maxpool': True, 'conv1x1': True, 'ln_dual': True, 'wgrad_fin': True, 'spm_nhwc': True, 'up_gemm': True, 'patch_gemm': True, 'wgrad_overlap': True, 'drop_pool': True,
           'fp16_rows': True, 'fp16_spm': True, 'fp16_tail': True, 'bias_partials': True,
           'fp16_linear': True,
           'fp16_msda': True,
           'group_norm': True,
           'bilinear_rows': True,
           'masked_attn': True,
           'point_loss': True,
           'point_mask_loss': True,
           'seg_logits': True,
           'seg_ce_loss': True}
for _k in os.environ.get('VAH_FUSED_DISABLE', '').split(','):
    if _k:
        ENABLED[_k.strip()] = False


def _stream(t):
    return _vah.raw_stream(t.device)


def _scratch(K, device):
    return torch.empty(_vah.lib.vah_reduce_ws_floats(K), dtype=torch.float32, device=device)


def _bf16_autocast():
    return torch.is_autocast_enabled() and torch.get_autocast_dtype('cuda') == torch.bfloat16


def takes_16(dtype, switch):
    return dtype == torch.bfloat16 or (dtype == torch.float16 and ENABLED[switch])


def autocast_16(switch):
    if not torch.is_autocast_enabled():
        return None
    dtype = torch.get_autocast_dtype('cuda')
    return dtype if takes_16(dtype, switch) else None


def tail_dtype():
    return autocast_16('fp16_tail')


_tail_dtype = tail_dtype


class _LayerNormBF16(torch.autograd.Function):

    @staticmethod
    def forward(ctx, x, weight, bias, eps, keep, dtype=torch.bfloat16):
        C = x.shape[-1]
        xc = x.contiguous()
        x2 = xc.view(-1, C)
        rows = x2.shape[0]
        y = torch.empty(x.shape, dtype=dtype, device=x.device)
        mean = torch.empty(rows, dtype=torch.float32, device=x.device)
        rstd = torch.empty(rows, dtype=torch.float32, device=x.device)
        w, b = weight.contiguous(), bias.contiguous()
        with _vah.on(x.device):
            _vah.call('vah_layernorm_fwd_f32_bf16', dtype, x2.data_ptr(), w.data_ptr(), b.data_ptr(), rows, C, float(eps), y.data_ptr(),
                      mean.data_ptr(), rstd.data_ptr(), _stream(x))
        ctx.save_for_backward(x2, w, mean, rstd)
        ctx.shape, ctx.dtype = x.shape, dtype
        ctx.set_materialize_grads(False)
        if keep:
            return xc, y
        return y

    @staticmethod
    def backward(ctx, *grads):
        gres, g = grads if len(grads) == 2 else (None, grads[0])
        x2, w, mean, rstd = ctx.saved_tensors
        rows, C = x2.shape
        if g is None:
            return (gres, None, None, None, None, None)
        g = g.contiguous().to(ctx.dtype)
        if gres is not None:
            gres = gres.contiguous().float()
        dx = torch.empty_like(x2)
        dwb = torch.empty(2, C, dtype=torch.float32, device=x2.device)
        ws = _scratch(2 * C, x2.device)
        with _vah.on(x2.device):
            _vah.call('vah_layernorm_bwd_f32_bf16', ctx.dtype, x2.data_ptr(), g.data_ptr(), w.data_ptr(), mean.data_ptr(), rstd.data_ptr(),
                      gres.data_ptr() if gres is not None else None, rows, C, dx.data_ptr(), dwb[0].data_ptr(), dwb[1].data_ptr(), ws.data_ptr(),
                      _stream(x2))
        return dx.view(ctx.shape), dwb[0], dwb[1], None, None, None


def _ln_fusable(norm, x):
    return (ENABLED['layer_norm'] and x.is_cuda and x.dtype == torch.float32 and autocast_16('fp16_rows') is not None
            and isinstance(norm, torch.nn.LayerNorm) and norm.elementwise_affine
            and x.shape[-1] % 4 == 0 and x.shape[-1] <= 2048 and x.numel() > 0)


class _LayerNormDualBF16(torch.autograd.Function):

    @staticmethod
    def forward(ctx, x, wa, ba, wb, bb, eps, dtype=torch.bfloat16):
        C = x.shape[-1]
        xc = x.contiguous()
        x2 = xc.view(-1, C)
        rows = x2.shape[0]
        ya = torch.empty(x.shape, dtype=dtype, device=x.device)
        yb = torch.empty(x.shape, dtype=dtype, device=x.device)
        mean = torch.empty(rows, dtype=torch.float32, device=x.device)
        rstd = torch.empty(rows, dtype=torch.float32, device=x.device)
        wa, ba, wb, bb = (t.contiguous() for t in (wa, ba, wb, bb))
        with _vah.on(x.device):
            _vah.call('vah_layernorm_dual_fwd', dtype, x2.data_ptr(), wa.data_ptr(), ba.data_ptr(), wb.data_ptr(), bb.data_ptr(), rows, C,
                      float(eps), ya.data_ptr(), yb.data_ptr(), mean.data_ptr(), rstd.data_ptr(), _stream(x))
        ctx.save_for_backward(x2, wa, wb, mean, rstd)
        ctx.shape, ctx.dtype = x.shape, dtype
        ctx.set_materialize_grads(False)
        return xc, ya, yb

    @staticmethod
    def backward(ctx, gres, ga, gb):
        x2, wa, wb, mean, rstd = ctx.saved_tensors
        rows, C = x2.shape
        if ga is None and gb is None:
            return (gres, None, None, None, None, None, None)
        ga = ga.contiguous().to(ctx.dtype) if ga is not None else None
        gb = gb.contiguous().to(ctx.dtype) if gb is not None else None
        if gres is not None:
            gres = gres.contiguous().float()
        dx = torch.empty_like(x2)
        dp = torch.empty(4, C, dtype=torch.float32, device=x2.device)
        ws = _scratch(2 * C, x2.device)
        with _vah.on(x2.device):
            _vah.call('vah_layernorm_dual_bwd', ctx.dtype, x2.data_ptr(), ga.data_ptr() if ga is not None else None,
                      gb.data_ptr() if gb is not None else None, wa.data_ptr(), wb.data_ptr(), mean.data_ptr(), rstd.data_ptr(),
                      gres.data_ptr() if gres is not None else None, rows, C, dx.data_ptr(), dp.data_ptr(), ws.data_ptr(), _stream(x2))
        return dx.view(ctx.shape), dp[0], dp[1], dp[2], dp[3], None, None


def layer_norm_dual_ok(norm_a, norm_b, x):
    return (ENABLED['ln_dual'] and _ln_fusable(norm_a, x) and _ln_fusable(norm_b, x) and norm_a.eps == norm_b.eps
            and x.shape[-1] <= 1024)


def layer_norm_dual_keep(norm_a, norm_b, x):
    if layer_norm_dual_ok(norm_a, norm_b, x):
        return _LayerNormDualBF16.apply(x, norm_a.weight, norm_a.bias, norm_b.weight, norm_b.bias, norm_a.eps, autocast_16('fp16_rows'))
    x, ya = layer_norm_keep(norm_a, x, fan_out=True)
    x, yb = layer_norm_keep(norm_b, x)
    return x, ya, yb


def layer_norm(norm, x):
    if _ln_fusable(norm, x):
        return _LayerNormBF16.apply(x, norm.weight, norm.bias, norm.eps, False, autocast_16('fp16_rows'))
    return norm(x)


def layer_norm_keep(norm, x, fan_out=False):
    if fan_out and not ENABLED['keep_feat']:
        return x, layer_norm(norm, x)
    if _ln_fusable(norm, x):
        return _LayerNormBF16.apply(x, norm.weight, norm.bias, norm.eps, True, autocast_16('fp16_rows'))
    return x, norm(x)


class _Bf16Copies:

    def __init__(self):
        self.entries = {}
        self.epoch = 0

    def get(self, p, dtype=torch.bfloat16):
        e = self.entries.get((id(p), dtype))
        if (e is not None and e[2] == self.epoch and (self.epoch & 1) and e[0]() is p and e[1].device == p.device
                and e[1].dtype == dtype):
            return e[1]
        return p.detach().to(dtype)

    def begin(self, params, dtype=torch.bfloat16):
        import weakref
        self.epoch += 1 if (self.epoch & 1) == 0 else 2
        if not params:
            return
        flat = torch.empty(sum(p.numel() for p in params), dtype=dtype, device=params[0].device)
        views = [v.view(p.shape) for v, p in zip(flat.split([p.numel() for p in params]), params)]
        torch._foreach_copy_(views, [p.detach() for p in params])
        if len(self.entries) > 4096:
            self.entries = {k: v for k, v in self.entries.items() if v[0]() is not None}
        for p, v in zip(params, views):
            self.entries[(id(p), dtype)] = (weakref.ref(p), v, self.epoch)

    def end(self):
        if self.epoch & 1:
            self.epoch += 1


BF16_COPIES = _Bf16Copies()


class _DropPool:

    def __init__(self):
        self.rows = self.seq = self.module = None
        self.pos, self.recording = 0, []

    def begin(self, module, device):
        self.module, self.recording, self.pos, self.rows = module, [], 0, None
        d = module.__dict__
        self.seq = d.get('_vah_drop_trace')
        if 'vah_drop_pool_ok' not in d:
            d['vah_drop_pool_ok'] = not any(getattr(m, 'with_cp', False) for m in module.modules())
        if not (self.seq and d['vah_drop_pool_ok'] and ENABLED.get('drop_pool', True)):
            self.seq = None
            return
        keeps = d.get('_vah_drop_keeps')
        if keeps is None or keeps.device != device or keeps.shape[0] != len(self.seq):
            keeps = d['_vah_drop_keeps'] = torch.tensor([k for k, _ in self.seq], dtype=torch.float32, device=device)[:, None]
        B = self.seq[0][1]
        if any(b != B for _, b in self.seq):
            self.seq = None
            return
        self.rows = torch.rand((len(self.seq), B), device=device).add_(keeps).floor_().div_(keeps)

    def take(self, x, keep):
        B = x.shape[0]
        if self.module is not None:
            self.recording.append((keep, B))
            if self.rows is not None:
                if self.pos < len(self.seq) and self.seq[self.pos] == (keep, B) and self.rows.device == x.device:
                    self.pos += 1
                    return self.rows[self.pos - 1]
                self.rows = None
        return x.new_empty((B,)).bernoulli_(keep).div_(keep)

    def end(self):
        if self.module is not None:
            d = self.module.__dict__
            if d.get('_vah_drop_trace') != self.recording:
                d['_vah_drop_trace'] = self.recording
                d.pop('_vah_drop_keeps', None)
        self.module = self.rows = self.seq = None


DROP_POOL = _DropPool()


class forward_epoch:

    def __init__(self, module):
        self.module = module

    def __enter__(self):
        module = self.module
        t16 = autocast_16('fp16_linear')
        if not (ENABLED['linear'] and t16 is not None):
            return self
        params = module.__dict__.get('_vah_linear_params')
        if params is None:
            params = [p for m in module.modules() if isinstance(m, torch.nn.Linear)
                      for p in (m.weight, m.bias) if p is not None]
            module.__dict__['_vah_linear_params'] = params
        live = [p for p in params if p.dtype == torch.float32 and p.is_cuda]
        if live:
            BF16_COPIES.begin(live, t16)
            SIDE.begin_epoch()
            BIAS_PARTIALS.begin_epoch()
            if module.training:
                DROP_POOL.begin(module, live[0].device)
        return self

    def __exit__(self, *exc):
        BF16_COPIES.end()
        DROP_POOL.end()
        return False


_GEMM_WS_BYTES = 32 << 20
WGRAD_F32 = os.environ.get('VAH_LINEAR_WGRAD', 'f32') == 'f32'
GEMM_TABLE = os.path.join(os.path.dirname(os.path.dirname(os.path.abspath(__file__))), 'tuning',
                          'gemm_table_mi355x_base_det_1024.txt')
GEMM_TABLE_F16 = GEMM_TABLE[:-len('.txt')] + '_f16.txt'


def _configure_gemm():
    spec = os.environ.get('VAH_GEMM_TUNING')
    if spec:
        parts = [int(v) for v in spec.split(',')]
        _vah.check(_vah.lib.vah_gemm_set_tuning(parts[0], parts[1] if len(parts) > 1 else 32), 'gemm_set_tuning')
    dump = os.environ.get('VAH_GEMM_TABLE_DUMP')
    if dump:
        import atexit
        atexit.register(lambda: open(dump, 'w').write(_vah.gemm_table_dump()))


_configure_gemm()
_GEMM_TABLE_LOADED = False


def _load_gemm_table():
    global _GEMM_TABLE_LOADED
    _GEMM_TABLE_LOADED = True
    path = os.environ.get('VAH_GEMM_TABLE')
    for path in ((GEMM_TABLE, GEMM_TABLE_F16) if path is None else (path,)):
        if path and os.path.exists(path):
            _vah.gemm_table_load(open(path).read())


def gemm_16(a, b, trans_a=False, trans_b=False, out_dtype=None, bias=None, out=None):
    t16 = a.dtype
    assert t16 in (torch.bfloat16, torch.float16) and b.dtype == t16, (a.dtype, b.dtype)
    if out_dtype is None:
        out_dtype = t16
    assert out_dtype in (t16, torch.float32) and (bias is None or bias.dtype in (t16, torch.float32))
    M, K = (a.shape[1], a.shape[0]) if trans_a else a.shape
    N = b.shape[0] if trans_b else b.shape[1]
    assert (b.shape[1] if trans_b else b.shape[0]) == K and a.is_contiguous() and b.is_contiguous()
    if out is not None:
        assert out.shape == (M, N) and out.is_contiguous()
        d, out_dtype = out, out.dtype
    else:
        d = torch.empty((M, N), dtype=out_dtype, device=a.device)
    if M == 0 or N == 0:
        return d
    if K == 0:
        return d.zero_()
    if bias is not None and bias.dtype == torch.float16 and out_dtype == torch.float32:
        bias = bias.float()
    if not _GEMM_TABLE_LOADED:
        _load_gemm_table()
    ws_bytes = _GEMM_WS_BYTES
    if bias is None and K >= 4096:
        ws_bytes += min(64 * M * N * 4, 160 << 20)
    ws = torch.empty(ws_bytes, dtype=torch.uint8, device=a.device)
    epilogue = _vah.GEMM_EPI_BIAS if bias is not None else _vah.GEMM_EPI_NONE
    with _vah.on(a.device):
        _vah.call('vah_gemm_bf16', t16, int(trans_a), int(trans_b), M, N, K, a.data_ptr(), a.shape[1], b.data_ptr(), b.shape[1], d.data_ptr(), N,
                  int(out_dtype == torch.float32), epilogue, bias.data_ptr() if bias is not None else None,
                  int(bias is not None and bias.dtype == torch.float32), ws.data_ptr(), ws_bytes, _stream(a))
    return d


gemm_bf16 = gemm_16


def _wgrad_bgrad(g2, x2, partials=None):
    import ctypes
    R, N = g2.shape
    K = x2.shape[1]
    t16 = g2.dtype
    assert x2.dtype == t16
    if not _GEMM_TABLE_LOADED:
        _load_gemm_table()
    dev = g2.device
    gw = torch.empty((N, K), dtype=torch.float32, device=dev)
    gb = torch.empty(N, dtype=torch.float32, device=dev)
    ws_bytes = _GEMM_WS_BYTES + (min(64 * N * K * 4, 160 << 20) if R >= 4096 else 0)
    ws = torch.empty(ws_bytes, dtype=torch.uint8, device=dev)
    with _vah.on(dev):
        st = _stream(g2)
        if partials is not None:
            cws, nparts = partials[0], ctypes.c_int64(partials[1])
        else:
            cws, nparts = _scratch(N, dev), ctypes.c_int64(0)
            _vah.call('vah_colsum_bf16_partials', t16, g2.data_ptr(), R, N, cws.data_ptr(), ctypes.byref(nparts), st)
        _vah.call('vah_gemm_bf16_fin', t16, 1, 0, N, K, R, g2.data_ptr(), N, x2.data_ptr(), K, gw.data_ptr(), K, 1, ws.data_ptr(), ws_bytes,
                  cws.data_ptr(), nparts.value, N, gb.data_ptr(), st)
    return gw, gb


class _SideStream:

    def __init__(self):
        self.streams = {}
        self.pending = {}

    def begin_epoch(self):
        for idx in list(self.pending):
            self.join(idx)

    def note(self, weight, bias):
        import weakref
        if not weight.is_leaf or (bias is not None and not bias.is_leaf) or not (BF16_COPIES.epoch & 1):
            return None
        if not weight.requires_grad or (bias is not None and not bias.requires_grad):
            return None
        return tuple(weakref.ref(p) for p in (weight, bias) if p is not None)

    @staticmethod
    def _only_accumulated(p):
        if p is None or getattr(p, '_backward_hooks', None) or getattr(p, '_post_accumulate_grad_hooks', None):
            return False
        with torch.enable_grad():
            acc = p.view_as(p).grad_fn.next_functions[0][0]
        try:
            return bool(torch._C._will_engine_execute_node(acc))
        except RuntimeError:
            return False

    def may_defer(self, token, dev):
        if token is None or not (ENABLED['wgrad_overlap'] and dev.type == 'cuda'):
            return False
        if torch.cuda.is_current_stream_capturing():
            return False
        import torch.distributed as dist
        if dist.is_available() and dist.is_initialized():
            return False
        return all(self._only_accumulated(r()) for r in token)

    def fork(self, dev, keep):
        idx = dev.index if dev.index is not None else torch.cuda.current_device()
        side = self.streams.get(idx)
        if side is None:
            side = self.streams[idx] = torch.cuda.Stream(device=dev)
        cur = torch.cuda.current_stream(dev)
        side.wait_stream(cur)
        entry = self.pending.get(idx)
        if entry is None:
            self.pending[idx] = entry = (cur, [], [])
            torch.autograd.Variable._execution_engine.queue_callback(lambda: self.join(idx))
        entry[1].extend(keep)
        return side

    def deliver(self, dev, token, grads):
        idx = dev.index if dev.index is not None else torch.cuda.current_device()
        self.pending[idx][2].extend((r(), g) for r, g in zip(token, grads))

    def join(self, idx):
        entry = self.pending.pop(idx, None)
        if entry is None:
            return
        main, keep, grads = entry
        main.wait_stream(self.streams[idx])
        with torch.no_grad(), torch.cuda.stream(main):
            for p, g in grads:
                if p is None:
                    continue
                if g.dtype != p.dtype:
                    g = g.to(p.dtype)
                if p.grad is None:
                    p.grad = g.view_as(p)
                else:
                    p.grad.add_(g.view_as(p))
        keep.clear()


SIDE = _SideStream()


class _BiasPartials:

    ATTR = '_vah_bias_dy'

    def __init__(self):
        self.passes = {}

    @staticmethod
    def mark(y, bias):
        if ENABLED['bias_partials'] and bias is not None and bias.requires_grad and torch.is_grad_enabled():
            setattr(y, _BiasPartials.ATTR, True)
        return y

    @staticmethod
    def wanted(z):
        return bool(ENABLED['bias_partials'] and getattr(z, _BiasPartials.ATTR, False) and takes_16(z.dtype, 'fp16_linear')
                    and z.shape[-1] % 8 == 0)

    @staticmethod
    def _key(t):
        return (t.untyped_storage().data_ptr(), t.storage_offset())

    def record(self, dz, bpart, nparts):
        idx = dz.device.index
        entries = self.passes.get(idx)
        if entries is None:
            entries = self.passes[idx] = {}
            try:
                torch.autograd.Variable._execution_engine.queue_callback(lambda: self.end_pass(idx))
            except RuntimeError:
                pass
        entries[self._key(dz)] = (dz, dz._version, bpart, int(nparts))

    def take(self, g2):
        entries = self.passes.get(g2.device.index)
        if not entries:
            return None
        key = self._key(g2)
        e = entries.get(key)
        if e is None:
            return None
        dz, version, bpart, nparts = e
        if (g2.dim() != 2 or not g2.is_contiguous() or not dz.is_contiguous() or dz.dtype != g2.dtype
                or dz.shape[-1] != g2.shape[1] or dz.numel() != g2.numel() or dz._version != version
                or g2._version != version or nparts < 1):
            return None
        del entries[key]
        return bpart, nparts

    def end_pass(self, idx):
        self.passes.pop(idx, None)

    def begin_epoch(self):
        self.passes.clear()


BIAS_PARTIALS = _BiasPartials()


def _bias_partials_out(C, device):
    import ctypes
    return torch.empty(_vah.lib.vah_reduce_ws_floats(C), dtype=torch.float32, device=device), ctypes.c_int64(0)


class _LinearBF16(torch.autograd.Function):

    @staticmethod
    def forward(ctx, x, weight, bias, t16=torch.bfloat16):
        K = x.shape[-1]
        x2 = x.reshape(-1, K)
        if x2.dtype != t16:
            x2 = x2.to(t16)
        x2 = x2.contiguous()
        wb = BF16_COPIES.get(weight, t16)
        y = gemm_16(x2, wb, trans_b=True, bias=bias.detach() if bias is not None else None)
        ctx.save_for_backward(x2, wb)
        ctx.has_bias = bias is not None
        ctx.side = SIDE.note(weight, bias)
        ctx.in_shape = x.shape
        ctx.in_dtype = x.dtype
        return y.view(*x.shape[:-1], weight.shape[0])

    @staticmethod
    def backward(ctx, g):
        x2, wb = ctx.saved_tensors
        N = wb.shape[0]
        t16 = wb.dtype
        g2 = g.reshape(-1, N)
        if g2.dtype != t16:
            g2 = g2.to(t16)
        g2 = g2.contiguous()
        gx = gw = gb = None
        want_b = ctx.has_bias and ctx.needs_input_grad[2]
        fin = ctx.needs_input_grad[1] and want_b and WGRAD_F32 and g2.shape[0] > 0 and ENABLED['wgrad_fin']
        partials = BIAS_PARTIALS.take(g2) if fin else None
        deferred = fin and SIDE.may_defer(ctx.side, g2.device)
        if deferred:
            keep = (g2, x2) if partials is None else (g2, x2, partials[0])
            with torch.cuda.stream(SIDE.fork(g2.device, keep)):
                SIDE.deliver(g2.device, ctx.side, _wgrad_bgrad(g2, x2, partials))
        if ctx.needs_input_grad[0]:
            gx = gemm_16(g2, wb).view(ctx.in_shape)
            if gx.dtype != ctx.in_dtype:
                gx = gx.to(ctx.in_dtype)
        if deferred:
            pass
        elif fin:
            gw, gb = _wgrad_bgrad(g2, x2, partials)
        else:
            if ctx.needs_input_grad[1]:
                if WGRAD_F32:
                    gw = gemm_16(g2, x2, trans_a=True, out_dtype=torch.float32)
                else:
                    gw = gemm_16(g2, x2, trans_a=True).float()
            if want_b:
                gb = torch.empty(N, dtype=torch.float32, device=g2.device)
                ws = _scratch(N, g2.device)
                with _vah.on(g2.device):
                    _vah.call('vah_colsum_bf16', t16, g2.data_ptr(), g2.shape[0], N, gb.data_ptr(), ws.data_ptr(), _stream(g2))
        return gx, gw, gb, None


class _PairCopies:

    def __init__(self):
        self.entries = {}

    def get(self, a, b, dtype=torch.bfloat16):
        key = (id(a.weight), id(b.weight), dtype)
        epoch = BF16_COPIES.epoch
        e = self.entries.get(key)
        if e is not None and e[0] == epoch and (epoch & 1) and e[1].device == a.weight.device and e[3]() is a.weight:
            return e[1], e[2]
        import weakref
        with torch.no_grad():
            w = torch.cat([a.weight.detach(), b.weight.detach()], 0).to(dtype)
            bias = torch.cat([a.bias.detach(), b.bias.detach()], 0).float()
        if len(self.entries) > 1024:
            self.entries.clear()
        self.entries[key] = (epoch, w, bias, weakref.ref(a.weight))
        return w, bias


PAIR_COPIES = _PairCopies()


class _LinearPairBF16(torch.autograd.Function):

    @staticmethod
    def forward(ctx, x, wa, ba, wb, bb, pair, f32_out=False):
        K = x.shape[-1]
        x2 = x.reshape(-1, K)
        w, bias = pair
        t16 = w.dtype
        if x2.dtype != t16:
            x2 = x2.to(t16)
        x2 = x2.contiguous()
        y = gemm_16(x2, w, trans_b=True, bias=bias, out_dtype=torch.float32 if f32_out else t16)
        na = wa.shape[0]
        ctx.save_for_backward(x2, w)
        ctx.na, ctx.in_shape, ctx.in_dtype = na, x.shape, x.dtype
        lead = x.shape[:-1]
        return y[:, :na].contiguous().view(*lead, na), y[:, na:].contiguous().view(*lead, w.shape[0] - na)

    @staticmethod
    def backward(ctx, ga, gb):
        x2, w = ctx.saved_tensors
        na = ctx.na
        nb = w.shape[0] - na
        R = x2.shape[0]
        g = torch.empty((R, na + nb), dtype=w.dtype, device=x2.device)
        g[:, :na] = ga.reshape(R, na) if ga is not None else 0
        g[:, na:] = gb.reshape(R, nb) if gb is not None else 0
        gx = gw = gbias = None
        if ctx.needs_input_grad[0]:
            gx = gemm_16(g, w).view(ctx.in_shape)
            if gx.dtype != ctx.in_dtype:
                gx = gx.to(ctx.in_dtype)
        want_w = ctx.needs_input_grad[1] or ctx.needs_input_grad[3]
        want_b = ctx.needs_input_grad[2] or ctx.needs_input_grad[4]
        if want_w and want_b and R > 0 and ENABLED['wgrad_fin']:
            gw, gbias = _wgrad_bgrad(g, x2)
        else:
            if want_w:
                gw = gemm_16(g, x2, trans_a=True, out_dtype=torch.float32)
            if want_b:
                gbias = torch.empty(na + nb, dtype=torch.float32, device=g.device)
                ws = _scratch(na + nb, g.device)
                with _vah.on(g.device):
                    _vah.call('vah_colsum_bf16', g.dtype, g.data_ptr(), R, na + nb, gbias.data_ptr(), ws.data_ptr(), _stream(g))
        return (gx, gw[:na] if gw is not None else None, gbias[:na] if gbias is not None else None,
                gw[na:] if gw is not None else None, gbias[na:] if gbias is not None else None, None, None)


def linear_pair(lin_a, lin_b, x, f32_out=False):
    wa, wb = lin_a.weight, lin_b.weight
    t16 = autocast_16('fp16_linear')
    if f32_out and t16 != torch.bfloat16:
        t16 = None
    if (ENABLED['linear'] and ENABLED['linear_pair'] and x.is_cuda and t16 is not None and wa.dtype == torch.float32
            and wb.dtype == torch.float32 and lin_a.bias is not None and lin_b.bias is not None
            and x.dtype in (t16, torch.float32) and (wa.shape[0] + wb.shape[0]) % 8 == 0
            and wa.shape[1] % 8 == 0 and wa.shape[1] == wb.shape[1] and x.numel() > 0
            and type(lin_a) is torch.nn.Linear and type(lin_b) is torch.nn.Linear):
        return _LinearPairBF16.apply(x, wa, lin_a.bias, wb, lin_b.bias, PAIR_COPIES.get(lin_a, lin_b, t16), f32_out)
    if f32_out and x.is_cuda and _bf16_autocast():
        with torch.autocast('cuda', enabled=False):
            xf = x.float()
            return torch.nn.functional.linear(xf, wa.float(), lin_a.bias), torch.nn.functional.linear(xf, wb.float(), lin_b.bias)
    return linear(lin_a, x), linear(lin_b, x)


class _PairCoreCopies:

    def __init__(self):
        self.entries = {}

    def get(self, a, b, M):
        key = (id(a.weight), id(b.weight))
        epoch = BF16_COPIES.epoch
        e = self.entries.get(key)
        if e is not None and e[0] == epoch and (epoch & 1) and e[1].device == a.weight.device and e[4]() is a.weight:
            return e[1], e[2], e[3]
        import weakref
        na, nb = a.weight.shape[0], b.weight.shape[0]
        po, pl = na // M, nb // M
        dev = a.weight.device
        if e is not None and e[4]() is a.weight and e[3][0].device == dev and e[3][0].numel() == na + nb:
            perm = e[3]
        else:
            fw = torch.cat([torch.cat((torch.arange(m * po, (m + 1) * po), na + torch.arange(m * pl, (m + 1) * pl))) for m in range(M)])
            inv = torch.empty_like(fw)
            inv[fw] = torch.arange(fw.numel())
            perm = (fw.to(dev), inv.to(dev))
        with torch.no_grad():
            w = torch.cat([a.weight.detach(), b.weight.detach()], 0).index_select(0, perm[0]).to(torch.bfloat16)
            bias = torch.cat([a.bias.detach(), b.bias.detach()], 0).float().index_select(0, perm[0])
        if len(self.entries) > 1024:
            self.entries.clear()
        self.entries[key] = (epoch, w, bias, perm, weakref.ref(a.weight))
        return w, bias, perm


PAIR_CORE_COPIES = _PairCoreCopies()


class _MSDAPairCore(torch.autograd.Function):

    @staticmethod
    def forward(ctx, query, value, shapes, lsi, ref, wa, ba, wb, bb, copies, M, L, P):
        from ops.functions import ms_deform_attn_fused as mf
        K = query.shape[-1]
        x2 = query.reshape(-1, K)
        if x2.dtype != torch.bfloat16:
            x2 = x2.to(torch.bfloat16)
        x2 = x2.contiguous()
        w, bias, perm = copies
        y = gemm_16(x2, w, trans_b=True, bias=bias, out_dtype=torch.float32)
        N, Lq = query.shape[0], query.shape[1]
        PS = 3 * L * P
        yv = y.view(N, Lq, M, PS)
        offsets = yv[..., :2 * L * P].unflatten(-1, (L, P, 2))
        logits = yv[..., 2 * L * P:]
        value = value.contiguous()
        refc = ref.detach().float().contiguous().view(ref.shape[0], Lq, -1, ref.shape[-1])
        out = mf.fused_forward(value, shapes, lsi, offsets, logits, PS, PS, refc, carrier=ref if refc.shape[0] == 1 else None,
                               token=BF16_COPIES.epoch)
        ctx.save_for_backward(x2, w, y, value, shapes, lsi, refc, perm[1])
        ctx.dims = (N, Lq, M, L, P, wa.shape[0])
        ctx.in_shape, ctx.in_dtype = query.shape, query.dtype
        return out

    @staticmethod
    @torch.autograd.function.once_differentiable
    def backward(ctx, gout):
        x2, w, y, value, shapes, lsi, refc, inv = ctx.saved_tensors
        N, Lq, M, L, P, na = ctx.dims
        S, D = value.shape[1], value.shape[3]
        PS = 3 * L * P
        R = x2.shape[0]
        gout = gout.contiguous().to(value.dtype)
        g = torch.empty((R, M * PS), dtype=torch.bfloat16, device=x2.device)
        grad_value = torch.empty_like(value)
        ws_bytes = _vah.lib.vah_msda_tile_ws_bytes(N, S, M * (D // 32), L, Lq, P)
        ws = torch.empty(ws_bytes, dtype=torch.uint8, device=value.device)
        from ops.functions.ms_deform_attn_fused import box_entry
        name, comps = box_entry('vah_msda_fused_backward_tiled', refc.shape[3])
        with _vah.on(value.device):
            rc = getattr(_vah.lib, name)(
                value.data_ptr(), 1, shapes.data_ptr(), lsi.data_ptr(), y.data_ptr(), y.data_ptr() + 2 * L * P * 4, 0, PS, PS,
                refc.data_ptr(), refc.shape[2], refc.shape[0], *comps, gout.data_ptr(), N, S, M, D, L, Lq, P, grad_value.data_ptr(), 1,
                g.data_ptr(), g.data_ptr() + 2 * L * P * 2, 1, PS, PS, ws.data_ptr(), ws_bytes, _stream(value))
        _vah.check(rc, name)
        gx = gw = gbias = None
        if ctx.needs_input_grad[0]:
            gx = gemm_16(g, w).view(ctx.in_shape)
            if gx.dtype != ctx.in_dtype:
                gx = gx.to(ctx.in_dtype)
        if any(ctx.needs_input_grad[5:9]):
            gwp, gbp = _wgrad_bgrad(g, x2)
            gw, gbias = gwp.index_select(0, inv), gbp.index_select(0, inv)
        return (gx, grad_value if ctx.needs_input_grad[1] else None, None, None, None,
                gw[:na] if gw is not None else None, gbias[:na] if gbias is not None else None,
                gw[na:] if gw is not None else None, gbias[na:] if gbias is not None else None, None, None, None, None)


def msda_pair_core_ok(mod, query, value, reference_points):
    import os
    from ops.functions.ms_deform_attn_fused import ref_points_ok
    a, b = mod.sampling_offsets, mod.attention_weights
    M, L, P = mod.n_heads, mod.n_levels, mod.n_points
    return (ENABLED['linear'] and ENABLED['linear_pair'] and ENABLED['pair_core'] and query.is_cuda and _bf16_autocast()
            and value.dtype == torch.bfloat16 and value.dim() == 4 and value.shape[-1] in (32, 64) and P == 4 and L in (1, 3, 4)
            and (M * 3 * L * P) % 8 == 0
            and type(a) is torch.nn.Linear and type(b) is torch.nn.Linear and a.bias is not None and b.bias is not None
            and a.weight.dtype == torch.float32 and b.weight.dtype == torch.float32 and a.weight.shape[1] % 8 == 0
            and ref_points_ok(reference_points, value.shape[0], L)
            and query.numel() > 0 and value.numel() > 0 and query.dtype in (torch.bfloat16, torch.float32)
            and os.environ.get('VAH_MSDA_FUSED', '1') != '0' and os.environ.get('VAH_MSDA_TILED', '1') != '0'
            and _vah.lib.vah_msda_tile_ws_bytes(value.shape[0], value.shape[1], M * (value.shape[-1] // 32), L,
                                                query.shape[1], P) >= 0)


def msda_pair_core(mod, query, value, shapes, lsi, reference_points):
    a, b = mod.sampling_offsets, mod.attention_weights
    return _MSDAPairCore.apply(query, value, shapes, lsi, reference_points, a.weight, a.bias, b.weight, b.bias,
                               PAIR_CORE_COPIES.get(a, b, mod.n_heads), mod.n_heads, mod.n_levels, mod.n_points)


class _Conv1x1BF16(torch.autograd.Function):

    @staticmethod
    def forward(ctx, x, weight):
        B, Ci, H, W = x.shape
        Co = weight.shape[0]
        x = x.contiguous()
        wb = BF16_COPIES.get(weight).view(Co, Ci)
        out = torch.empty((B, Co, H, W), dtype=torch.bfloat16, device=x.device)
        for b in range(B):
            gemm_16(wb, x[b].view(Ci, H * W), out=out[b].view(Co, H * W))
        ctx.save_for_backward(x, wb)
        return out

    @staticmethod
    def backward(ctx, g):
        x, wb = ctx.saved_tensors
        B, Ci, H, W = x.shape
        Co = wb.shape[0]
        g = g.contiguous().to(torch.bfloat16)
        dx = dw = None
        if ctx.needs_input_grad[0]:
            dx = torch.empty_like(x)
            for b in range(B):
                gemm_16(wb, g[b].view(Co, H * W), trans_a=True, out=dx[b].view(Ci, H * W))
        if ctx.needs_input_grad[1]:
            for b in range(B):
                part = gemm_16(g[b].view(Co, H * W), x[b].view(Ci, H * W), trans_b=True, out_dtype=torch.float32)
                dw = part if dw is None else dw.add_(part)
            dw = dw.view(Co, Ci, 1, 1)
        return dx, dw


class _UpFromTokens(torch.autograd.Function):

    @staticmethod
    def forward(ctx, rows, weight, h, w, addend, t16):
        B, T, C = rows.shape
        Co = weight.shape[1]
        xb = rows.detach().to(t16).contiguous()
        if t16 == torch.bfloat16:
            wc = BF16_COPIES.get(weight).permute(2, 3, 1, 0).reshape(4 * Co, C).contiguous()
            U = torch.empty((B, 4 * Co, T), dtype=torch.bfloat16, device=rows.device)
            for b in range(B):
                gemm_16(wc, xb[b], trans_b=True, out=U[b])
        else:
            wc = weight.detach().to(t16).permute(2, 3, 1, 0).reshape(4 * Co, C).contiguous()
            U = torch.bmm(wc.unsqueeze(0).expand(B, 4 * Co, C), xb.transpose(1, 2))
        out = torch.empty((B, Co, 2 * h, 2 * w), dtype=t16, device=rows.device)
        add = addend.contiguous() if addend is not None else None
        with _vah.on(rows.device):
            _vah.call('vah_pixel_shuffle2_bf16', t16, U.data_ptr(), B, Co, h, w, out.data_ptr(), 0, add.data_ptr() if add is not None else None,
                      _stream(rows))
        ctx.save_for_backward(xb, wc)
        ctx.meta = (h, w, Co, rows.dtype, t16)
        return out

    @staticmethod
    def backward(ctx, g):
        xb, wc = ctx.saved_tensors
        h, w, Co, in_dtype, t16 = ctx.meta
        B, T, C = xb.shape
        g = g.contiguous().to(t16)
        dU = torch.empty((B, 4 * Co, T), dtype=t16, device=g.device)
        with _vah.on(g.device):
            _vah.call('vah_pixel_shuffle2_bf16', t16, g.data_ptr(), B, Co, h, w, dU.data_ptr(), 1, None, _stream(g))
        dx = dw = None
        if ctx.needs_input_grad[0]:
            if t16 == torch.bfloat16:
                dx = torch.empty((B, T, C), dtype=torch.bfloat16, device=g.device)
                for b in range(B):
                    gemm_16(dU[b], wc, trans_a=True, out=dx[b])
            else:
                dx = torch.matmul(dU.transpose(1, 2), wc)
            if dx.dtype != in_dtype:
                dx = dx.to(in_dtype)
        if ctx.needs_input_grad[1]:
            if t16 == torch.bfloat16:
                for b in range(B):
                    part = gemm_16(dU[b], xb[b], out_dtype=torch.float32)
                    dw = part if dw is None else dw.add_(part)
            else:
                dw = torch.bmm(dU, xb).float().sum(0)
            dw = dw.view(2, 2, Co, C).permute(3, 2, 0, 1).contiguous()
        return dx, dw, None, None, (g if ctx.needs_input_grad[4] else None), None


def up_from_tokens(up, rows, h, w, addend=None):
    wt = up.weight
    t16 = autocast_16('fp16_tail')
    if (ENABLED['up_gemm'] and ENABLED['linear'] and rows.is_cuda and t16 is not None and isinstance(up, torch.nn.ConvTranspose2d)
            and up.kernel_size == (2, 2) and up.stride == (2, 2) and up.padding == (0, 0) and up.output_padding == (0, 0)
            and up.groups == 1 and up.dilation == (1, 1) and wt.dtype == torch.float32 and rows.dim() == 3
            and rows.shape[1] == h * w and rows.shape[2] == wt.shape[0] and w % 8 == 0 and wt.shape[0] % 8 == 0
            and wt.shape[1] % 8 == 0 and rows.dtype in (torch.float32, t16) and rows.numel() > 0
            and (addend is None or (addend.dtype == t16 and tuple(addend.shape) == (rows.shape[0], wt.shape[1], 2 * h, 2 * w)))):
        return _UpFromTokens.apply(rows, wt, h, w, addend, t16)
    return None


def patch_embed(conv, x):
    w = conv.weight
    ps = conv.kernel_size[0]
    if (ENABLED['patch_gemm'] and ENABLED['linear'] and x.is_cuda and x.dtype == torch.float32 and not x.requires_grad
            and _bf16_autocast() and x.dim() == 4 and isinstance(conv, torch.nn.Conv2d) and conv.kernel_size == (ps, ps)
            and conv.stride == (ps, ps) and conv.padding == (0, 0) and conv.groups == 1 and conv.dilation == (1, 1)
            and ps % 8 == 0 and x.shape[2] % ps == 0 and x.shape[3] % ps == 0 and w.dtype == torch.float32
            and w.shape[0] % 8 == 0 and x.numel() > 0):
        B, C, H, W = x.shape
        x = x.contiguous()
        rows = torch.empty((B * (H // ps) * (W // ps), C * ps * ps), dtype=torch.bfloat16, device=x.device)
        with _vah.on(x.device):
            _vah.check(_vah.lib.vah_patchify_bf16(x.data_ptr(), B, C, H, W, ps, rows.data_ptr(), _stream(x)), 'patchify')
        y = _LinearBF16.apply(rows, w.view(w.shape[0], -1), conv.bias)
        return y.view(B, (H // ps) * (W // ps), w.shape[0]), H // ps, W // ps
    return None


def conv1x1(conv, x):
    w = conv.weight
    if (ENABLED['conv1x1'] and ENABLED['linear'] and x.is_cuda and x.dtype == torch.bfloat16 and _bf16_autocast()
            and x.dim() == 4 and w.dtype == torch.float32 and w.shape[2:] == (1, 1) and conv.stride == (1, 1)
            and conv.padding == (0, 0) and conv.groups == 1 and w.shape[0] % 8 == 0 and w.shape[1] % 8 == 0
            and (x.shape[2] * x.shape[3]) % 8 == 0 and x.numel() > 0):
        return _Conv1x1BF16.apply(x, w)
    return F.conv2d(x, w, None)


def linear(lin, x):
    w = lin.weight
    t16 = autocast_16('fp16_linear')
    if (ENABLED['linear'] and x.is_cuda and t16 is not None and w.dtype == torch.float32
            and x.dtype in (t16, torch.float32) and w.shape[0] % 8 == 0
            and w.shape[1] % 8 == 0 and x.numel() > 0 and type(lin) is torch.nn.Linear):
        return BIAS_PARTIALS.mark(_LinearBF16.apply(x, w, lin.bias, t16), lin.bias)
    return lin(x)


class _GeluBF16(torch.autograd.Function):

    @staticmethod
    def forward(ctx, h):
        ctx.save_for_backward(h)
        return F.gelu(h)

    @staticmethod
    def backward(ctx, da):
        (h,) = ctx.saved_tensors
        C = h.shape[-1]
        hc = h.contiguous()
        da = da.contiguous().to(h.dtype)
        dh = torch.empty(h.shape, dtype=h.dtype, device=h.device)
        bpart, nparts = _bias_partials_out(C, h.device)
        import ctypes
        with _vah.on(h.device):
            _vah.call('vah_gelu_bwd_bsum_bf16', h.dtype, da.data_ptr(), hc.data_ptr(), h.numel() // C, C, dh.data_ptr(), bpart.data_ptr(),
                      ctypes.byref(nparts), _stream(h))
        BIAS_PARTIALS.record(dh, bpart, nparts.value)
        return dh


def gelu(act, h):
    if (isinstance(act, torch.nn.GELU) and act.approximate == 'none' and h.is_cuda and autocast_16('fp16_linear') is not None
            and BIAS_PARTIALS.wanted(h) and h.numel() > 0 and h.requires_grad and torch.is_grad_enabled()):
        return _GeluBF16.apply(h)
    return act(h)


def _scale_residual_bwd(g, z, gp, s, dims, bias_partials):
    import ctypes
    B, rpb, C = dims
    dz = torch.empty_like(z)
    dgamma = torch.empty(C, dtype=torch.float32, device=g.device) if gp is not None else None
    ws = _scratch(C, g.device) if gp is not None else None
    args = (g.data_ptr(), z.data_ptr(), gp.data_ptr() if gp is not None else None,
            s.data_ptr() if s is not None else None, B, rpb, C, dz.data_ptr(),
            dgamma.data_ptr() if dgamma is not None else None, ws.data_ptr() if ws is not None else None)
    with _vah.on(g.device):
        if bias_partials:
            bpart, nparts = _bias_partials_out(C, g.device)
            _vah.call('vah_scale_residual_bwd_bsum', z.dtype, *args, bpart.data_ptr(), ctypes.byref(nparts), _stream(g))
            BIAS_PARTIALS.record(dz, bpart, nparts.value)
        else:
            _vah.call('vah_scale_residual_bwd', z.dtype, *args, _stream(g))
    return dz, dgamma


class _ScaleResidual(torch.autograd.Function):
    @staticmethod
    def forward(ctx, x, z, gamma, s, bias_partials=False):
        B, C = x.shape[0], x.shape[-1]
        rpb = x.numel() // (B * C)
        x, z = x.contiguous(), z.contiguous()
        y = torch.empty_like(x)
        gp = gamma.contiguous() if gamma is not None else None
        with _vah.on(x.device):
            _vah.call('vah_scale_residual_fwd', z.dtype, x.data_ptr(), z.data_ptr(), gp.data_ptr() if gp is not None else None,
                      s.data_ptr() if s is not None else None, B, rpb, C, y.data_ptr(), _stream(x))
        ctx.save_for_backward(z, gp, s)
        ctx.dims = (B, rpb, C)
# ... 1 lines not shown
        return y

    @staticmethod
    def backward(ctx, g):
        z, gp, s = ctx.saved_tensors
        g = g.contiguous()
        dz, dgamma = _scale_residual_bwd(g, z, gp, s, ctx.dims, ctx.bias_partials)
        return g, dz, dgamma, None, None


def residual(x, z, gamma=None, drop_path=None):
    prob = float(getattr(drop_path, 'drop_prob', 0.) or 0.)
    training = bool(getattr(drop_path, 'training', False))
    if (ENABLED['residual'] and x.is_cuda and x.dtype == torch.float32 and takes_16(z.dtype, 'fp16_rows')
            and x.shape == z.shape and x.shape[-1] % 4 == 0 and x.numel() > 0
            and (gamma is None or gamma.dtype == torch.float32)):
        s = None
        if prob > 0. and training:
            s = DROP_POOL.take(x, 1.0 - prob)
        return _ScaleResidual.apply(x, z, gamma, s, BIAS_PARTIALS.wanted(z))
    t = gamma * z if gamma is not None else z
    return x + (drop_path(t) if drop_path is not None else t)


class _ResidualLN(torch.autograd.Function):

    @staticmethod
    def forward(ctx, x, z, gamma, s, weight, bias, eps, bias_partials=False):
        B, C = x.shape[0], x.shape[-1]
        rpb = x.numel() // (B * C)
        x, z = x.contiguous(), z.contiguous()
        t = torch.empty_like(x)
        h = torch.empty(x.shape, dtype=z.dtype, device=x.device)
        rows = B * rpb
        mean = torch.empty(rows, dtype=torch.float32, device=x.device)
        rstd = torch.empty(rows, dtype=torch.float32, device=x.device)
        gp = gamma.contiguous() if gamma is not None else None
        w, b = weight.contiguous(), bias.contiguous()
        with _vah.on(x.device):
            _vah.call('vah_residual_layernorm_fwd', z.dtype, x.data_ptr(), z.data_ptr(), gp.data_ptr() if gp is not None else None,
                      s.data_ptr() if s is not None else None, B, rpb, C, w.data_ptr(), b.data_ptr(), float(eps), t.data_ptr(), h.data_ptr(),
                      mean.data_ptr(), rstd.data_ptr(), _stream(x))
        ctx.save_for_backward(t, z, gp, s, w, mean, rstd)
        ctx.dims = (B, rpb, C)
        ctx.bias_partials = bias_partials
        ctx.set_materialize_grads(False)
        return t, h

    @staticmethod
    def backward(ctx, gt, gh):
        t, z, gp, s, w, mean, rstd = ctx.saved_tensors
        B, rpb, C = ctx.dims
        dev = t.device
        if gt is not None:
            gt = gt.contiguous().float()
        if gh is None:
            if gt is None:
                return (None,) * 8
            dz, dgamma = _scale_residual_bwd(gt, z, gp, s, ctx.dims, ctx.bias_partials)
            return gt, dz, dgamma, None, None, None, None, None
        gh = gh.contiguous().to(z.dtype)
        dt = torch.empty_like(t)
        dz = torch.empty_like(z)
        grads = torch.empty(3, C, dtype=torch.float32, device=dev)
        ws = _scratch(3 * C, dev)
        args = (t.data_ptr(), gh.data_ptr(), w.data_ptr(), mean.data_ptr(), rstd.data_ptr(),
                gt.data_ptr() if gt is not None else None, z.data_ptr(),
                gp.data_ptr() if gp is not None else None, s.data_ptr() if s is not None else None, B, rpb, C,
                dt.data_ptr(), dz.data_ptr(), grads[2].data_ptr() if gp is not None else None,
                grads[0].data_ptr(), grads[1].data_ptr(), ws.data_ptr())
        with _vah.on(dev):
            if ctx.bias_partials and gp is None:
                import ctypes
                bpart, nparts = _bias_partials_out(C, dev)
                _vah.call('vah_residual_layernorm_bwd_bsum', z.dtype, *args, bpart.data_ptr(), ctypes.byref(nparts), _stream(t))
                BIAS_PARTIALS.record(dz, bpart, nparts.value)
            else:
                _vah.call('vah_residual_layernorm_bwd', z.dtype, *args, _stream(t))
        return dt, dz, grads[2] if gp is not None else None, None, grads[0], grads[1], None, None


def _drop_path_scale(x, drop_path):
    prob = float(getattr(drop_path, 'drop_prob', 0.) or 0.)
    if prob > 0. and bool(getattr(drop_path, 'training', False)):
        return DROP_POOL.take(x, 1.0 - prob)
    return None


def residual_ln(x, z, gamma, drop_path, norm):
    if (ENABLED['residual'] and ENABLED['residual_ln'] and _ln_fusable(norm, x) and z.dtype == autocast_16('fp16_rows')
            and x.shape == z.shape
            and x.dim() >= 2 and (gamma is None or gamma.dtype == torch.float32) and x.shape[-1] <= 1024):
        return _ResidualLN.apply(x, z, gamma, _drop_path_scale(x, drop_path), norm.weight, norm.bias, norm.eps,
                                 gamma is None and BIAS_PARTIALS.wanted(z))
    ac = autocast_16('fp16_rows')
    if ENABLED['fp16_rows'] and ac is not None and z.dtype != ac and z.dtype in (torch.bfloat16, torch.float16):
        t = gamma * z if gamma is not None else z
        t = x + (drop_path(t) if drop_path is not None else t)
        return t, norm(t)
    return layer_norm_keep(norm, residual(x, z, gamma, drop_path))


class _DWConvTokens(torch.autograd.Function):
    @staticmethod
    def forward(ctx, x, weight, bias, H, W):
        B, N, C = x.shape
        x = x.contiguous()
        w = weight.detach().float().contiguous()
        b = bias.detach().float().contiguous() if bias is not None else None
        y = torch.empty_like(x)
        with _vah.on(x.device):
            _vah.call('vah_dwconv3x3_tokens_bf16', x.dtype, x.data_ptr(), w.data_ptr(), b.data_ptr() if b is not None else None, B, H, W, C, 0,
                      y.data_ptr(), _stream(x))
        ctx.save_for_backward(x, w)
        ctx.dims = (B, H, W, C, bias is not None, weight.dtype)
        return y

    @staticmethod
    def backward(ctx, g):
        x, w = ctx.saved_tensors
        B, H, W, C, has_bias, wdtype = ctx.dims
        g = g.contiguous().to(x.dtype)
        dx = torch.empty_like(x)
        dw = torch.empty(C * 9 + C, dtype=torch.float32, device=x.device)
        ws = _scratch(10 * C, x.device)
        with _vah.on(x.device):
            _vah.call('vah_dwconv3x3_tokens_bf16', x.dtype, g.data_ptr(), w.data_ptr(), None, B, H, W, C, 1, dx.data_ptr(), _stream(x))
            _vah.call('vah_dwconv3x3_tokens_wgrad_bf16', x.dtype, x.data_ptr(), g.data_ptr(), B, H, W, C, dw.data_ptr(),
                      dw[C * 9:].data_ptr() if has_bias else None, ws.data_ptr(), _stream(x))
        return (dx, dw[:C * 9].view(C, 1, 3, 3).to(wdtype),
                dw[C * 9:].to(wdtype) if has_bias else None, None, None)


def dwconv_tokens(conv, x, H, W):
    B, N, C = x.shape
    if (ENABLED['dwconv'] and x.is_cuda and takes_16(x.dtype, 'fp16_rows') and C % 4 == 0 and C <= 1024
            and H % 2 == 0 and W % 2 == 0 and N == 21 * (H // 2) * (W // 2) and x.numel() > 0
            and conv.weight.shape == (C, 1, 3, 3)):
        return _DWConvTokens.apply(x, conv.weight, conv.bias, H, W)
    return None


def _sync_group(norm):
    import torch.distributed as dist
    if not isinstance(norm, torch.nn.SyncBatchNorm) or not dist.is_available() or not dist.is_initialized():
        return None
    group = norm.process_group if norm.process_group is not None else dist.group.WORLD
    if dist.get_world_size(group) > 1:
        return group
    from . import data_parallel
    return group if data_parallel.one_rank_group() else None


class _BNTail(torch.autograd.Function):

    @staticmethod
    def forward(ctx, a, b, x, weight, bias, shift, norm, scale, relu, out_dtype, t16):
        N, C, H, W = a.shape
        sh = shift.detach().float().contiguous() if shift is not None else None
        shp = sh.data_ptr() if sh is not None else None
        a = a.contiguous()
        b = b.contiguous() if b is not None else None
        x = x.contiguous().float() if x is not None else None
        dev, st = a.device, _stream(a)
        ops = (a.data_ptr(), int(a.dtype == t16), b.data_ptr() if b is not None else None,
               int(b is not None and b.dtype == t16), x.data_ptr() if x is not None else None,
               scale, N, C, H, W)
        training = norm.training or norm.running_mean is None
        group = _sync_group(norm) if training else None
        w = weight.detach().float().contiguous() if weight is not None else None
        bb = bias.detach().float().contiguous() if bias is not None else None
        with _vah.on(dev):
            if training:
                sums = torch.empty(2 * C + 1, dtype=torch.float32, device=dev)
                ws = torch.empty(_vah.lib.vah_bn_tail_ws_floats(C), dtype=torch.float32, device=dev)
                _vah.call('vah_bn_tail_stats', t16, *ops, shp, sums.data_ptr(), ws.data_ptr(), st)
                sums[2 * C:].fill_(float(N * H * W))
                if group is not None:
                    import torch.distributed as dist
                    dist.all_reduce(sums, group=group)
                mean = torch.empty(C, dtype=torch.float32, device=dev)
                rstd = torch.empty(C, dtype=torch.float32, device=dev)
                track = norm.running_mean is not None
                _vah.check(_vah.lib.vah_bn_finalize_stats(
                    sums.data_ptr(), C, float(norm.eps), float(norm.momentum),
                    norm.running_mean.data_ptr() if track else None, norm.running_var.data_ptr() if track else None,
                    mean.data_ptr(), rstd.data_ptr(), st), 'bn_finalize_stats')
                if track:
                    with torch.no_grad():
                        norm.num_batches_tracked += 1
                count = sums[2 * C:]
            else:
                count = None
                mean = norm.running_mean.float().contiguous()
                rstd = torch.rsqrt(norm.running_var.float() + norm.eps)
            y = torch.empty((N, C, H, W), dtype=out_dtype, device=dev)
            _vah.call('vah_bn_tail_apply', t16, *ops, mean.data_ptr(), rstd.data_ptr(), w.data_ptr() if w is not None else None,
                      bb.data_ptr() if bb is not None else None, int(relu), shp, y.data_ptr(), int(out_dtype == t16), st)
        ctx.save_for_backward(a, b, x, mean, rstd, w, bb, count, sh)
        ctx.meta = (scale, training, group, weight is not None, bias is not None, relu, t16)
        return y

    @staticmethod
    def backward(ctx, dy):
        a, b, x, mean, rstd, w, bb, count, sh = ctx.saved_tensors
        scale, training, group, has_w, has_b, relu, t16 = ctx.meta
        shp = sh.data_ptr() if sh is not None else None
        N, C, H, W = a.shape
        dy = dy.contiguous()
        if dy.dtype not in (torch.float32, t16):
            dy = dy.float()
        dy_bf16 = int(dy.dtype == t16)
        dev, st = a.device, _stream(a)
        ops = (a.data_ptr(), int(a.dtype == t16), b.data_ptr() if b is not None else None,
               int(b is not None and b.dtype == t16), x.data_ptr() if x is not None else None,
               scale, N, C, H, W)
        wp = w.data_ptr() if w is not None else None
        bp = bb.data_ptr() if bb is not None else None
        with _vah.on(dev):
            sums = torch.empty(2 * C, dtype=torch.float32, device=dev)
            ws = torch.empty(_vah.lib.vah_bn_tail_ws_floats(C), dtype=torch.float32, device=dev)
            _vah.call('vah_bn_tail_bwd_stats', t16, *ops, mean.data_ptr(), rstd.data_ptr(), wp, bp, int(relu), shp, dy.data_ptr(), dy_bf16,
                      sums.data_ptr(), ws.data_ptr(), st)
            local = sums.clone() if (training and group is not None) else sums
            dweight = local[C:] if has_w else None
            dbias = local[:C] if has_b else None
            if training:
                if group is not None:
                    import torch.distributed as dist
                    dist.all_reduce(sums, group=group)
                means = sums / count
            else:
                means = torch.zeros_like(sums)
            need_a, need_b, need_x = ctx.needs_input_grad[:3]
            da = torch.empty_like(a) if need_a else None
            db = torch.empty_like(b) if (b is not None and need_b) else None
            dx = None
            if x is not None and need_x:
                dx = torch.zeros_like(x) if scale > 1 else torch.empty_like(x)
            if da is not None or db is not None or dx is not None:
                _vah.call('vah_bn_tail_bwd_apply', t16, *ops, mean.data_ptr(), rstd.data_ptr(), wp, bp, int(relu), shp, dy.data_ptr(), dy_bf16,
                          means[:C].data_ptr(), means[C:].data_ptr(), da.data_ptr() if da is not None else None,
                          db.data_ptr() if db is not None else None, dx.data_ptr() if dx is not None else None, st)
        dshift = None
        if sh is not None and ctx.needs_input_grad[5]:
            dshift = torch.zeros_like(sh) if training else (w if w is not None else 1.0) * rstd * local[:C]
        return da, db, dx, dweight, dbias, dshift, None, None, None, None, None


def _bn_fusable(norm, a):
    t16 = autocast_16('fp16_tail')
    return (isinstance(norm, torch.nn.modules.batchnorm._BatchNorm) and a.is_cuda and t16 is not None
            and a.dim() == 4 and a.dtype in (t16, torch.float32) and a.shape[3] <= 8192
            and a.numel() > 0 and norm.momentum is not None
            and (not norm.training or a.shape[0] * a.shape[2] * a.shape[3] > 1)
            and (norm.training or norm.running_mean is not None)
            and (norm.weight is None or norm.weight.dtype == torch.float32))


def _tail_shape_ok(a, scale, has_x):
    N, C, H, W = a.shape
    return bool(_vah.lib.vah_bn_tail_supported(N, C, H, W, scale, int(has_x)))


def tail_takes_conv_bias(norm, ref):
    return ENABLED['bn_tail'] and ENABLED['bias_fold'] and _bn_fusable(norm, ref)


def halve(x):
    if (ENABLED['bn_tail'] and x.is_cuda and autocast_16('fp16_tail') is not None and x.dim() == 4 and x.shape[2] % 2 == 0
            and x.shape[3] % 2 == 0):
        return F.avg_pool2d(x.float(), 2)
    return F.interpolate(x, scale_factor=0.5, mode='bilinear', align_corners=False)


def bn_tail(norm, a, b=None, x=None, scale=1, shift=None):
    t16 = autocast_16('fp16_tail')
    if (ENABLED['bn_tail'] and _bn_fusable(norm, a) and x is not None
            and (b is None or (b.shape == a.shape and b.dtype in (t16, torch.float32)))
            and scale in (1, 2, 4, 8) and a.shape[3] % (4 * scale) == 0 and a.shape[2] % scale == 0
            and tuple(x.shape) == (a.shape[0], a.shape[1], a.shape[2] // scale, a.shape[3] // scale)
            and x.dtype in (t16, torch.float32) and _tail_shape_ok(a, scale, True)):
        return _BNTail.apply(a, b, x, norm.weight, norm.bias, shift, norm, scale, False, torch.float32, t16)
    t = a if b is None else a + b
    if shift is not None:
        t = t + shift.view(1, -1, 1, 1).to(t.dtype)
    if x is not None:
        t = t + (x if scale == 1 else F.interpolate(x, scale_factor=scale, mode='bilinear', align_corners=False))
    return norm(t)


BN_RELU_MIN_NUMEL = int(os.environ.get('VAH_BN_RELU_MIN_NUMEL', 8 << 20))


def bn_relu(norm, a):
    if (ENABLED['bn_relu'] and _bn_fusable(norm, a) and a.shape[3] % 4 == 0 and a.numel() >= BN_RELU_MIN_NUMEL
            and _tail_shape_ok(a, 1, False)):
        return _BNTail.apply(a, None, None, norm.weight, norm.bias, None, norm, 1, True, a.dtype, autocast_16('fp16_tail'))
    return F.relu(norm(a))


class _TokensToMaps(torch.autograd.Function):

    @staticmethod
    def forward(ctx, tokens, hw, t16):
        B, T, C = tokens.shape
        tokens = tokens.contiguous()
        outs, t0 = [], 0
        with _vah.on(tokens.device):
            for h, w in hw:
                o = torch.empty((B, C, h, w), dtype=torch.float32, device=tokens.device)
                _vah.call('vah_transpose_tokens', t16, tokens.data_ptr(), B, T, t0, h * w, C, o.data_ptr(), 1, 0, None, _stream(tokens))
                outs.append(o)
                t0 += h * w
        ctx.hw, ctx.shape, ctx.t16 = hw, (B, T, C), t16
        ctx.set_materialize_grads(False)
        return tuple(outs)

    @staticmethod
    def backward(ctx, *grads):
        B, T, C = ctx.shape
        dev = next(g.device for g in grads if g is not None)
        gt = torch.empty((B, T, C), dtype=torch.float32, device=dev)
        t0 = 0
        with _vah.on(dev):
            for (h, w), g in zip(ctx.hw, grads):
                if g is None:
                    gt[:, t0:t0 + h * w].zero_()
                else:
                    g = g.contiguous().float()
                    _vah.call('vah_transpose_tokens', ctx.t16, g.data_ptr(), B, T, t0, h * w, C, gt.data_ptr(), 0, 0, None, _stream(g))
                t0 += h * w
        return gt, None, None


def _maps_dtype():
    return torch.float16 if autocast_16('fp16_tail') == torch.float16 else torch.bfloat16


def tokens_to_maps(tokens, hw):
    hw = tuple((int(h), int(w)) for h, w in hw)
    assert sum(h * w for h, w in hw) == tokens.shape[1]
    if (ENABLED['maps'] and tokens.is_cuda and tokens.dtype == torch.float32 and tokens.dim() == 3
            and tokens.numel() > 0 and tokens.shape[0] <= 65535):
# ... 653 lines not shown
```

vit-adapter_amd/vitadapter/spm_nhwc.py:

```python
import torch
import torch.nn.functional as F

import _vah
from . import conv, fused


def _stream(t):
    return _vah.raw_stream(t.device)


def image_to_nhwc16(x, dtype=torch.bfloat16):
    N, C, H, W = x.shape
    assert C == 3 and x.dtype == torch.float32
    x = x.contiguous()
    y = torch.empty((N, H, W, 16), dtype=dtype, device=x.device)
    with _vah.on(x.device):
        _vah.call('vah_image_to_nhwc16_bf16', dtype, x.data_ptr(), N, H, W, y.data_ptr(), _stream(x))
    return y


class _Conv3x3(torch.autograd.Function):

    @staticmethod
    def forward(ctx, x, weight, stride):
        cin = x.shape[-1]
        w = weight.detach()
        if w.shape[1] != cin:
            w = F.pad(w, (0, 0, 0, 0, 0, cin - w.shape[1]))
        wb = w.to(x.dtype)
        ctx.save_for_backward(x, wb)
        ctx.stride, ctx.wcin = stride, weight.shape[1]
        return conv.conv3x3_forward(x, conv.forward_weight(wb, x.dtype), stride)

    @staticmethod
    def backward(ctx, gy):
        x, wb = ctx.saved_tensors
        gy = gy.contiguous().to(x.dtype)
        gx = gw = None
        if ctx.needs_input_grad[0]:
            gx = conv.conv3x3_input_grad(gy, conv.dgrad_weight(wb, x.dtype), ctx.stride, x.shape[1:3])
        if ctx.needs_input_grad[1]:
            gw = conv.conv3x3_weight_grad(x, gy, ctx.stride).permute(0, 3, 1, 2)[:, :ctx.wcin].contiguous()
        return gx, gw, None


class _BNRelu(torch.autograd.Function):

    @staticmethod
    def forward(ctx, x, weight, bias, norm, relu):
        C = x.shape[-1]
        rows = x.numel() // C
        x = x.contiguous()
        dev, st = x.device, _stream(x)
        training = norm.training or norm.running_mean is None
        group = fused._sync_group(norm) if training else None
        w = weight.detach().float().contiguous() if weight is not None else None
        b = bias.detach().float().contiguous() if bias is not None else None
        with _vah.on(dev):
            if training:
                sums = torch.empty(2 * C + 1, dtype=torch.float32, device=dev)
                ws = torch.empty(_vah.lib.vah_bn_nhwc_ws_floats(C), dtype=torch.float32, device=dev)
                _vah.call('vah_bn_nhwc_stats', x.dtype, x.data_ptr(), rows, C, sums.data_ptr(), ws.data_ptr(), st)
                sums[2 * C:].fill_(float(rows))
                if group is not None:
                    import torch.distributed as dist
                    dist.all_reduce(sums, group=group)
                mean = torch.empty(C, dtype=torch.float32, device=dev)
                rstd = torch.empty(C, dtype=torch.float32, device=dev)
                track = norm.running_mean is not None
                _vah.check(_vah.lib.vah_bn_finalize_stats(
                    sums.data_ptr(), C, float(norm.eps), float(norm.momentum),
                    norm.running_mean.data_ptr() if track else None, norm.running_var.data_ptr() if track else None,
                    mean.data_ptr(), rstd.data_ptr(), st), 'bn_finalize_stats')
                if track:
                    with torch.no_grad():
                        norm.num_batches_tracked += 1
                count = sums[2 * C:]
            else:
                count = None
                mean = norm.running_mean.float().contiguous()
                rstd = torch.rsqrt(norm.running_var.float() + norm.eps)
            y = torch.empty_like(x)
            _vah.call('vah_bn_nhwc_apply', x.dtype, x.data_ptr(), rows, C, mean.data_ptr(), rstd.data_ptr(), w.data_ptr() if w is not None else None,
                      b.data_ptr() if b is not None else None, int(relu), y.data_ptr(), st)
        ctx.save_for_backward(x, mean, rstd, w, b, count)
        ctx.meta = (training, group, weight is not None, bias is not None, relu)
        return y

    @staticmethod
    def backward(ctx, dy):
        x, mean, rstd, w, b, count = ctx.saved_tensors
        training, group, has_w, has_b, relu = ctx.meta
        C = x.shape[-1]
        rows = x.numel() // C
        dy = dy.contiguous().to(x.dtype)
        dev, st = x.device, _stream(x)
        wp = w.data_ptr() if w is not None else None
        bp = b.data_ptr() if b is not None else None
        with _vah.on(dev):
            sums = torch.empty(2 * C, dtype=torch.float32, device=dev)
            ws = torch.empty(_vah.lib.vah_bn_nhwc_ws_floats(C), dtype=torch.float32, device=dev)
            _vah.call('vah_bn_nhwc_bwd_stats', x.dtype, x.data_ptr(), dy.data_ptr(), rows, C, mean.data_ptr(), rstd.data_ptr(), wp, bp, int(relu),
                      sums.data_ptr(), ws.data_ptr(), st)
            local = sums.clone() if (training and group is not None) else sums
            dweight = local[C:] if has_w else None
            dbias = local[:C] if has_b else None
            dx = None
            if ctx.needs_input_grad[0]:
                if training:
                    if group is not None:
                        import torch.distributed as dist
                        dist.all_reduce(sums, group=group)
                    means = sums / count
                else:
                    means = torch.zeros_like(sums)
                dx = torch.empty_like(x)
                _vah.call('vah_bn_nhwc_bwd_apply', x.dtype, x.data_ptr(), dy.data_ptr(), rows, C, mean.data_ptr(), rstd.data_ptr(), wp, bp,
                          int(relu), means[:C].data_ptr(), means[C:].data_ptr(), dx.data_ptr(), st)
        return dx, dweight, dbias, None, None


class _MaxPool(torch.autograd.Function):

    @staticmethod
    def forward(ctx, x):
        N, H, W, C = x.shape
        x = x.contiguous()
        y = torch.empty((N, (H - 1) // 2 + 1, (W - 1) // 2 + 1, C), dtype=x.dtype, device=x.device)
        idx = torch.empty(y.shape, dtype=torch.uint8, device=x.device)
        with _vah.on(x.device):
            _vah.call('vah_maxpool3s2_nhwc_fwd_bf16', x.dtype, x.data_ptr(), N, H, W, C, y.data_ptr(), idx.data_ptr(), _stream(x))
        ctx.save_for_backward(idx)
        ctx.in_shape, ctx.in_dtype = x.shape, x.dtype
        return y

    @staticmethod
    def backward(ctx, gy):
        idx, = ctx.saved_tensors
        N, H, W, C = ctx.in_shape
        gy = gy.contiguous().to(ctx.in_dtype)
        gx = torch.empty(ctx.in_shape, dtype=ctx.in_dtype, device=gy.device)
        with _vah.on(gy.device):
            _vah.call('vah_maxpool3s2_nhwc_bwd_bf16', ctx.in_dtype, gy.data_ptr(), idx.data_ptr(), N, H, W, C, gx.data_ptr(), _stream(gy))
        return gx


class _Conv1x1ToPlanes(torch.autograd.Function):

    @staticmethod
    def forward(ctx, x, weight):
        B, H, W, Ci = x.shape
        Co = weight.shape[0]
        wb = fused.BF16_COPIES.get(weight).view(Co, Ci)
        out = torch.empty((B, Co, H, W), dtype=torch.bfloat16, device=x.device)
        for b in range(B):
            fused.gemm_bf16(wb, x[b].view(H * W, Ci), trans_b=True, out=out[b].view(Co, H * W))
        ctx.save_for_backward(x, wb)
        return out

    @staticmethod
    def backward(ctx, g):
        x, wb = ctx.saved_tensors
        B, H, W, Ci = x.shape
        Co = wb.shape[0]
        g = g.contiguous().to(torch.bfloat16)
        dx = dw = None
        if ctx.needs_input_grad[0]:
            dx = torch.empty_like(x)
            for b in range(B):
                fused.gemm_bf16(g[b].view(Co, H * W), wb, trans_a=True, out=dx[b].view(H * W, Ci))
        if ctx.needs_input_grad[1]:
            for b in range(B):
                part = fused.gemm_bf16(g[b].view(Co, H * W), x[b].view(H * W, Ci), out_dtype=torch.float32)
                dw = part if dw is None else dw.add_(part)
            dw = dw.view(Co, Ci, 1, 1)
        return dx, dw


def autocast_dtype():
    return fused.autocast_16('fp16_spm')


def takes(spm, x, fold):
    if not (fold or autocast_dtype() == torch.float16):
        return False
    return usable(spm, x) and not (spm.with_cp and x.requires_grad)


def usable(spm, x):
    if not (fused.ENABLED.get('spm_nhwc', True) and x.is_cuda and x.dtype == torch.float32 and not x.requires_grad and x.dim() == 4 and x.shape[1] == 3
            and autocast_dtype() is not None and x.shape[2] % 32 == 0 and x.shape[3] % 32 == 0 and x.numel() > 0):
        return False
    convs = [spm.stem[0], spm.stem[3], spm.stem[6], spm.conv2[0], spm.conv3[0], spm.conv4[0]]
    for i, c in enumerate(convs):
        if not (isinstance(c, torch.nn.Conv2d) and c.kernel_size == (3, 3) and c.padding == (1, 1) and c.bias is None
                and c.groups == 1 and c.dilation == (1, 1) and c.out_channels % 64 == 0 and c.out_channels <= 256
                and (c.out_channels & (c.out_channels - 1)) == 0 and (i == 0 or c.in_channels % 64 == 0)
                and c.weight.dtype == torch.float32):
            return False
    norms = [spm.stem[1], spm.stem[4], spm.stem[7], spm.conv2[1], spm.conv3[1], spm.conv4[1]]
    return all(isinstance(n, torch.nn.modules.batchnorm._BatchNorm) and n.momentum is not None
               and (n.training or n.running_mean is not None) for n in norms)


def _cbr(conv_mod, norm, x):
    y = _Conv3x3.apply(x, conv_mod.weight, conv_mod.stride[0])
    return _BNRelu.apply(y, norm.weight, norm.bias, norm, True)


def _fc1_planes_f16(fc1, c1, with_bias):
    B, H, W, Ci = c1.shape
    Co = fc1.weight.shape[0]
    w = fc1.weight.view(1, Co, Ci).expand(B, Co, Ci)
    rows_t = c1.view(B, H * W, Ci).transpose(1, 2)
    if with_bias and fc1.bias is not None:
        out = torch.baddbmm(fc1.bias.view(1, Co, 1), w, rows_t)
    else:
        out = torch.bmm(w, rows_t)
    return out.view(B, Co, H, W)


def forward(spm, x, level_embed, c1_bias=False):
    dtype = autocast_dtype() or torch.bfloat16
    t = image_to_nhwc16(x, dtype)
    t = _cbr(spm.stem[0], spm.stem[1], t)
    t = _cbr(spm.stem[3], spm.stem[4], t)
    t = _cbr(spm.stem[6], spm.stem[7], t)
    c1 = _MaxPool.apply(t)
    c2 = _cbr(spm.conv2[0], spm.conv2[1], c1)
    c3 = _cbr(spm.conv3[0], spm.conv3[1], c2)
# ... 14 lines not shown
```

Before: 80.23 images/sec.

## Batch per-step weight copies into one epoch kernel and fuse row permutation into GEMM

Adds an epoch_copies kernel that builds every per-step bf16/f32 weight copy and pre-laid-out weight (conv9, upsample, etc.) in one launch from a job table, replacing many small cast/permute kernels. The MSDA weight-gradient GEMM gains a row-map variant that scatters rows during split-K reduction, which removes the separate index_select. BN finalize moves the count fill and the num_batches_tracked increment into one kernel. These changes cut kernel launches and extra passes over memory, at the cost of more layout bookkeeping and new ABI surface.

```diff
diff --git a/include/vitadapter_hip_epoch.h b/include/vitadapter_hip_epoch.h
--- /dev/null
+++ b/include/vitadapter_hip_epoch.h
@@ -0,0 +1,32 @@
+#ifndef VITADAPTER_HIP_EPOCH_H
+#define VITADAPTER_HIP_EPOCH_H
+
+#include <stdint.h>
+
+#ifdef __cplusplus
+extern "C" {
+#endif
+
+int64_t vah_epoch_job_bytes(void);
+int64_t vah_epoch_chunk_elems(void);
+int vah_epoch_copies(const void *jobs, int64_t njobs, const void *chunks, int64_t nchunks, int dtype16,
+                     void *out16, int64_t cap16, float *out32, int64_t cap32, void *stream);
+
+int vah_gemm_bf16_fin_rowmap(int trans_a, int trans_b, int64_t M, int64_t N, int64_t K, const void *A, int64_t lda,
+                             const void *B, int64_t ldb, void *D, int64_t ldd, int d_is_f32, void *workspace,
+                             int64_t workspace_bytes, const float *fin_part, int64_t fin_nparts, int64_t fin_C,
+                             float *fin_out, const int32_t *row_map, int *applied, void *stream);
+int vah_gemm_f16_fin_rowmap(int trans_a, int trans_b, int64_t M, int64_t N, int64_t K, const void *A, int64_t lda,
+                            const void *B, int64_t ldb, void *D, int64_t ldd, int d_is_f32, void *workspace,
+                            int64_t workspace_bytes, const float *fin_part, int64_t fin_nparts, int64_t fin_C,
+                            float *fin_out, const int32_t *row_map, int *applied, void *stream);
+
+int vah_bn_finalize_stats_book(float *sums, int64_t C, float count, float eps, float momentum, float *running_mean,
+                               float *running_var, float *mean, float *rstd, int64_t *num_batches_tracked,
+                               void *stream);
+
+#ifdef __cplusplus
+}
+#endif
+
+#endif
diff --git a/vit-adapter_amd/_vah.py b/vit-adapter_amd/_vah.py
--- a/vit-adapter_amd/_vah.py
+++ b/vit-adapter_amd/_vah.py
@@ -230,6 +230,20 @@
     _fn = getattr(lib, _name)
     _fn.restype, _fn.argtypes = _res, _args
 
+_pint = ctypes.POINTER(ctypes.c_int)
+_fin_rowmap = [_int, _int, _i64, _i64, _i64, _p, _i64, _p, _i64, _p, _i64, _int, _p, _i64, _p, _i64, _i64, _p, _p, _pint, _p]
+EPOCH_SIGNATURES = {
+    'vah_epoch_job_bytes': (_i64, []),
+    'vah_epoch_chunk_elems': (_i64, []),
+    'vah_epoch_copies': (_int, [_p, _i64, _p, _i64, _int, _p, _i64, _p, _i64, _p]),
+    'vah_gemm_bf16_fin_rowmap': (_int, _fin_rowmap),
+    'vah_gemm_f16_fin_rowmap': (_int, _fin_rowmap),
+    'vah_bn_finalize_stats_book': (_int, [_p, _i64, _f, _f, _f, _p, _p, _p, _p, _p, _p]),
+}
+for _name, (_res, _args) in EPOCH_SIGNATURES.items():
+    _fn = getattr(lib, _name)
+    _fn.restype, _fn.argtypes = _res, _args
+
 if lib.vah_abi_version() != ABI_VERSION:
     raise ImportError('libvitadapter_hip.so ABI %d != binding ABI %d: rebuild the library'
                       % (lib.vah_abi_version(), ABI_VERSION))
diff --git a/vit-adapter_amd/csrc/epoch_copies.hip b/vit-adapter_amd/csrc/epoch_copies.hip
--- /dev/null
+++ b/vit-adapter_amd/csrc/epoch_copies.hip
@@ -0,0 +1,123 @@
+#include <hip/hip_runtime.h>
+
+#include <cstdint>
+
+#include "../../include/vitadapter_hip_epoch.h"
+#include "common.h"
+#include "elem16.h"
+
+namespace vah {
+namespace {
+
+constexpr int kChunk = 2048;
+constexpr int64_t kDense = 1, kToF32 = 2;
+
+struct EpochJob {
+    int64_t src, dst, n, d1, d2, d3, s[4], l[4], flags, src_elems;
+};
+static_assert(sizeof(EpochJob) == 128, "the job layout is part of the ABI");
+
+template <typename T>
+__global__ __launch_bounds__(256) void epoch_copies_kernel(const EpochJob *__restrict__ jobs, int njobs,
+                                                           const int2 *__restrict__ chunks, T *__restrict__ out16,
+                                                           int64_t cap16, float *__restrict__ out32, int64_t cap32) {
+    const int2 ch = chunks[blockIdx.x];
+    if (ch.x < 0 || ch.x >= njobs || ch.y < 0) return;
+    const EpochJob &j = jobs[ch.x];
+    const int64_t n = j.n;
+    const int64_t e0 = (int64_t)ch.y * kChunk + threadIdx.x * 8;
+    if (e0 >= n) return;
+    const int cnt = (int)(n - e0 < 8 ? n - e0 : 8);
+    const float *src = reinterpret_cast<const float *>(j.src);
+    const int64_t src_elems = j.src_elems;
+    float v[8];
+#pragma unroll
+    for (int u = 0; u < 8; ++u) v[u] = 0.f;
+    if (j.flags & kDense) {
+        const float *p = src + e0;
+        if (e0 + cnt > src_elems) return;
+        if (cnt == 8 && ((uintptr_t)p & 15) == 0) {
+            const float4 a = *reinterpret_cast<const float4 *>(p), b = *reinterpret_cast<const float4 *>(p + 4);
+            v[0] = a.x, v[1] = a.y, v[2] = a.z, v[3] = a.w, v[4] = b.x, v[5] = b.y, v[6] = b.z, v[7] = b.w;
+        } else {
+#pragma unroll
+            for (int u = 0; u < 8; ++u)
+                if (u < cnt) v[u] = p[u];
+        }
+    } else {
+        const unsigned d1 = (unsigned)j.d1, d2 = (unsigned)j.d2, d3 = (unsigned)j.d3;
+        if (d1 == 0 || d2 == 0 || d3 == 0) return;
+#pragma unroll
+        for (int u = 0; u < 8; ++u) {
+            if (u < cnt) {
+                unsigned t = (unsigned)(e0 + u);
+                const unsigned i3 = t % d3;
+                t /= d3;
+                const unsigned i2 = t % d2;
+                t /= d2;
+                const unsigned i1 = t % d1;
+                const unsigned i0 = t / d1;
+                const int64_t off = i0 * j.s[0] + i1 * j.s[1] + i2 * j.s[2] + i3 * j.s[3];
+                if (i0 < j.l[0] && i1 < j.l[1] && i2 < j.l[2] && i3 < j.l[3] && off >= 0 && off < src_elems) v[u] = src[off];
+            }
+        }
+    }
+    const int64_t o = j.dst + e0;
+    if (j.flags & kToF32) {
+        if (j.dst < 0 || o + cnt > cap32) return;
+        float *q = out32 + o;
+        if (cnt == 8 && ((uintptr_t)q & 15) == 0) {
+            *reinterpret_cast<float4 *>(q) = make_float4(v[0], v[1], v[2], v[3]);
+            *reinterpret_cast<float4 *>(q + 4) = make_float4(v[4], v[5], v[6], v[7]);
+        } else {
+#pragma unroll
+            for (int u = 0; u < 8; ++u)
+                if (u < cnt) q[u] = v[u];
+        }
+    } else {
+        if (j.dst < 0 || o + cnt > cap16) return;
+        T *q = out16 + o;
+        if (cnt == 8 && ((uintptr_t)q & 15) == 0) {
+            store8_f32<T>(q, v);
+        } else {
+#pragma unroll
+            for (int u = 0; u < 8; ++u)
+                if (u < cnt) q[u] = (T)v[u];
+        }
+    }
+}
+
+}
+}
+
+extern "C" {
+
+int64_t vah_epoch_job_bytes(void) { return (int64_t)sizeof(vah::EpochJob); }
+
+int64_t vah_epoch_chunk_elems(void) { return vah::kChunk; }
+
+int vah_epoch_copies(const void *jobs, int64_t njobs, const void *chunks, int64_t nchunks, int dtype16, void *out16,
+                     int64_t cap16, float *out32, int64_t cap32, void *stream) {
+    using namespace vah;
+    const char *fn = "vah_epoch_copies";
+    clear_error();
+    if (njobs < 0 || nchunks < 0 || cap16 < 0 || cap32 < 0 || njobs > (1 << 24) || nchunks > (int64_t)0x7fffffff)
+        return fail(VAH_E_SHAPE, "%s: bad dims", fn);
+    if (dtype16 != 1 && dtype16 != 2) return fail(VAH_E_UNSUPPORTED, "%s: dtype16 is 1 (bf16) or 2 (fp16)", fn);
+    if (nchunks == 0) return VAH_OK;
+    if (njobs == 0) return fail(VAH_E_SHAPE, "%s: chunks without jobs", fn);
+    if (!jobs || !chunks || (cap16 > 0 && !out16) || (cap32 > 0 && !out32)) return fail(VAH_E_NULL, "%s: null pointer", fn);
+    if ((uintptr_t)jobs % 8 || (uintptr_t)chunks % 8 || (uintptr_t)out16 % 16 || (uintptr_t)out32 % 16)
+        return fail(VAH_E_ALIGN, "%s: misaligned pointer (tables 8 bytes, buffers 16)", fn);
+    hipStream_t st = (hipStream_t)stream;
+    LaunchScope scope(dtype16 == 2 ? "epoch_copies_f16" : "epoch_copies", cap16 * 6 + cap32 * 8, st, (cap16 + cap32) * 8);
+    if (dtype16 == 2)
+        hipLaunchKernelGGL(epoch_copies_kernel<_Float16>, dim3((unsigned)nchunks), dim3(256), 0, st, (const EpochJob *)jobs, (int)njobs,
+                           (const int2 *)chunks, (_Float16 *)out16, cap16, out32, cap32);
+    else
+        hipLaunchKernelGGL(epoch_copies_kernel<__bf16>, dim3((unsigned)nchunks), dim3(256), 0, st, (const EpochJob *)jobs, (int)njobs,
+                           (const int2 *)chunks, (__bf16 *)out16, cap16, out32, cap32);
+    return check_launch(fn);
+}
+
+}
diff --git a/vit-adapter_amd/csrc/gemm.hip b/vit-adapter_amd/csrc/gemm.hip
--- a/vit-adapter_amd/csrc/gemm.hip
+++ b/vit-adapter_amd/csrc/gemm.hip
@@ -16,6 +16,7 @@
 #include <vector>
 
 #include "../../include/vitadapter_hip.h"
+#include "../../include/vitadapter_hip_epoch.h"
 #include "common.h"
 
 namespace vah {
@@ -91,6 +92,7 @@
     const float *fin_part = nullptr;
     int fin_nparts = 0, fin_C = 0;
     float *fin_out = nullptr;
+    const int32_t *row_map = nullptr;
     const float *ref = nullptr;
 };
 
@@ -160,11 +162,11 @@
     }
 }
 
-template <typename OT>
-__global__ __launch_bounds__(256) void reduce_splits(const float *__restrict__ part, int split, int64_t MN, int N,
-                                                     int64_t ldd, int vec, OT *__restrict__ out, int reduce_blocks,
-                                                     const float *__restrict__ fin_part, int fin_nparts, int fin_C,
-                                                     float *__restrict__ fin_out) {
+template <typename OT, bool MAPPED>
+__device__ __forceinline__ void reduce_splits_body(const float *__restrict__ part, int split, int64_t MN, int N,
+                                                   int64_t ldd, int vec, OT *__restrict__ out, int reduce_blocks,
+                                                   const float *__restrict__ fin_part, int fin_nparts, int fin_C,
+                                                   float *__restrict__ fin_out, const int32_t *__restrict__ row_map) {
     if ((int)blockIdx.x >= reduce_blocks) {
         __shared__ float s_acc[8][32];
         const int col = threadIdx.x & 31, pl = threadIdx.x >> 5;
@@ -184,7 +186,12 @@
             float t = 0.f;
 #pragma unroll
             for (int u = 0; u < 8; ++u) t += s_acc[u][col];
-            fin_out[k] = t;
+            if constexpr (MAPPED) {
+                const unsigned kk = (unsigned)row_map[k];
+                if (kk < (unsigned)fin_C) fin_out[kk] = t;
+            } else {
+                fin_out[k] = t;
+            }
         }
         return;
     }
@@ -220,6 +227,12 @@
             const int64_t row = i / N;
             o = row * ldd + (i - row * N);
         }
+        if constexpr (MAPPED) {
+            const int64_t row = i / N;
+            const unsigned to = (unsigned)row_map[row];
+            if ((int64_t)to >= MN / N) continue;
+            o = (int64_t)to * ldd + (i - row * N);
+        }
         typedef OT ov4 __attribute__((ext_vector_type(4)));
         ov4 r;
         r[0] = (OT)acc.x;
@@ -235,6 +248,22 @@
             out[o + 3] = r[3];
         }
     }
+}
+
+template <typename OT>
+__global__ __launch_bounds__(256) void reduce_splits(const float *__restrict__ part, int split, int64_t MN, int N,
+                                                     int64_t ldd, int vec, OT *__restrict__ out, int reduce_blocks,
+                                                     const float *__restrict__ fin_part, int fin_nparts, int fin_C,
+                                                     float *__restrict__ fin_out) {
+    reduce_splits_body<OT, false>(part, split, MN, N, ldd, vec, out, reduce_blocks, fin_part, fin_nparts, fin_C, fin_out, nullptr);
+}
+
+template <typename OT>
+__global__ __launch_bounds__(256) void reduce_splits_mapped(const float *__restrict__ part, int split, int64_t MN, int N,
+                                                            int64_t ldd, int vec, OT *__restrict__ out, int reduce_blocks,
+                                                            const float *__restrict__ fin_part, int fin_nparts, int fin_C,
+                                                            float *__restrict__ fin_out, const int32_t *__restrict__ row_map) {
+    reduce_splits_body<OT, true>(part, split, MN, N, ldd, vec, out, reduce_blocks, fin_part, fin_nparts, fin_C, fin_out, row_map);
 }
 
 template <typename T>
@@ -362,6 +391,19 @@
     const unsigned rblocks = split > 1 ? (unsigned)std::min<int64_t>(8192, (MN / 4 + 255) / 256) : 0u;
     const unsigned fblocks = fin ? (unsigned)((c.fin_C + 31) / 32) : 0u;
     const int vec = c.k.N % 4 == 0 && c.k.ldd % 4 == 0 && (uintptr_t)c.D % (c.k.d32 ? 16 : 8) == 0;
+    if (c.row_map && split > 1) {
+        const dim3 grid(rblocks + fblocks);
+        if (c.k.d32)
+            hipLaunchKernelGGL(reduce_splits_mapped<float>, grid, dim3(256), 0, c.st, (const float *)c.ws, split, MN, (int)c.k.N,
+                               c.k.ldd, vec, (float *)c.D, (int)rblocks, c.fin_part, c.fin_nparts, c.fin_C, c.fin_out, c.row_map);
+        else if (c.k.f16)
+            hipLaunchKernelGGL(reduce_splits_mapped<_Float16>, grid, dim3(256), 0, c.st, (const float *)c.ws, split, MN, (int)c.k.N,
+                               c.k.ldd, vec, (_Float16 *)c.D, (int)rblocks, c.fin_part, c.fin_nparts, c.fin_C, c.fin_out, c.row_map);
+        else
+            hipLaunchKernelGGL(reduce_splits_mapped<__bf16>, grid, dim3(256), 0, c.st, (const float *)c.ws, split, MN, (int)c.k.N,
+                               c.k.ldd, vec, (__bf16 *)c.D, (int)rblocks, c.fin_part, c.fin_nparts, c.fin_C, c.fin_out, c.row_map);
+        return HIPBLAS_STATUS_SUCCESS;
+    }
     if (c.k.d32)
         hipLaunchKernelGGL(reduce_splits<float>, dim3(rblocks + fblocks), dim3(256), 0, c.st, (const float *)c.ws, split, MN,
                            (int)c.k.N, c.k.ldd, vec, (float *)c.D, (int)rblocks, c.fin_part, c.fin_nparts, c.fin_C, c.fin_out);
@@ -561,7 +603,7 @@
 static int gemm_impl(const char *fn, int f16, int trans_a, int trans_b, int64_t M, int64_t N, int64_t K, const void *A, int64_t lda,
                      const void *B, int64_t ldb, void *D, int64_t ldd, int d_is_f32, int epilogue, const void *bias,
                      int bias_is_f32, void *workspace, int64_t workspace_bytes, void *stream, const float *fin_part,
-                     int64_t fin_nparts, int64_t fin_C, float *fin_out);
+                     int64_t fin_nparts, int64_t fin_C, float *fin_out, const int32_t *row_map = nullptr, int *applied = nullptr);
 
 int vah_gemm_bf16(int trans_a, int trans_b, int64_t M, int64_t N, int64_t K, const void *A, int64_t lda,
                   const void *B, int64_t ldb, void *D, int64_t ldd, int d_is_f32, int epilogue, const void *bias,
@@ -603,10 +645,48 @@
                      0, workspace, workspace_bytes, stream, fin_part, fin_nparts, fin_C, fin_out);
 }
 
+static int gemm_fin_rowmap(const char *fn, int f16, int trans_a, int trans_b, int64_t M, int64_t N, int64_t K, const void *A,
+                           int64_t lda, const void *B, int64_t ldb, void *D, int64_t ldd, int d_is_f32, void *workspace,
+                           int64_t workspace_bytes, const float *fin_part, int64_t fin_nparts, int64_t fin_C, float *fin_out,
+                           const int32_t *row_map, int *applied, void *stream) {
+    using namespace vah;
+    if (applied) *applied = 0;
+    if (!fin_part || !fin_out || fin_nparts < 1 || fin_C < 1 || fin_nparts > (1 << 20) || fin_C > (1 << 24)) {
+        clear_error();
+        return fail(VAH_E_SHAPE, "%s: bad finalize job", fn);
+    }
+    if (!row_map) {
+        clear_error();
+        return fail(VAH_E_NULL, "%s: null pointer (row_map)", fn);
+    }
+    if (fin_C != M || (uintptr_t)row_map % 4) {
+        clear_error();
+        return fail(VAH_E_SHAPE, "%s: the row map serves D's rows and the finalize sums alike (fin_C == M), 4-byte aligned", fn);
+    }
+    return gemm_impl(fn, f16, trans_a, trans_b, M, N, K, A, lda, B, ldb, D, ldd, d_is_f32, VAH_GEMM_EPI_NONE, nullptr, 0, workspace,
+                     workspace_bytes, stream, fin_part, fin_nparts, fin_C, fin_out, row_map, applied);
+}
+
+int vah_gemm_bf16_fin_rowmap(int trans_a, int trans_b, int64_t M, int64_t N, int64_t K, const void *A, int64_t lda,
+                             const void *B, int64_t ldb, void *D, int64_t ldd, int d_is_f32, void *workspace,
+                             int64_t workspace_bytes, const float *fin_part, int64_t fin_nparts, int64_t fin_C,
+                             float *fin_out, const int32_t *row_map, int *applied, void *stream) {
+    return gemm_fin_rowmap("vah_gemm_bf16_fin_rowmap", 0, trans_a, trans_b, M, N, K, A, lda, B, ldb, D, ldd, d_is_f32, workspace,
+                           workspace_bytes, fin_part, fin_nparts, fin_C, fin_out, row_map, applied, stream);
+}
+
+int vah_gemm_f16_fin_rowmap(int trans_a, int trans_b, int64_t M, int64_t N, int64_t K, const void *A, int64_t lda,
+                            const void *B, int64_t ldb, void *D, int64_t ldd, int d_is_f32, void *workspace,
+                            int64_t workspace_bytes, const float *fin_part, int64_t fin_nparts, int64_t fin_C,
+                            float *fin_out, const int32_t *row_map, int *applied, void *stream) {
+    return gemm_fin_rowmap("vah_gemm_f16_fin_rowmap", 1, trans_a, trans_b, M, N, K, A, lda, B, ldb, D, ldd, d_is_f32, workspace,
+                           workspace_bytes, fin_part, fin_nparts, fin_C, fin_out, row_map, applied, stream);
+}
+
 static int gemm_impl(const char *fn, int f16, int trans_a, int trans_b, int64_t M, int64_t N, int64_t K, const void *A, int64_t lda,
                      const void *B, int64_t ldb, void *D, int64_t ldd, int d_is_f32, int epilogue, const void *bias,
                      int bias_is_f32, void *workspace, int64_t workspace_bytes, void *stream, const float *fin_part,
-                     int64_t fin_nparts, int64_t fin_C, float *fin_out) {
+                     int64_t fin_nparts, int64_t fin_C, float *fin_out, const int32_t *row_map, int *applied) {
     using namespace vah;
     clear_error();
     if (M < 0 || N < 0 || K < 0) return fail(VAH_E_SHAPE, "%s: negative dimension", fn);
@@ -667,6 +747,8 @@
         hipblasLtMatmulDescSetAttribute(pp->desc, HIPBLASLT_MATMUL_DESC_BIAS_POINTER, &c.bias, sizeof(c.bias));
     }
     Problem &p = *pp;
+    c.row_map = it->second.split > 1 ? row_map : nullptr;
+    if (applied) *applied = c.row_map != nullptr;
     s = run(S, c, p, it->second.algo, it->second.workspace, it->second.split);
     if (s != HIPBLAS_STATUS_SUCCESS) return fail(VAH_E_UNSUPPORTED, "%s: hipblasLtMatmul: %s", fn, status_name(s));
     return check_launch(fn);
diff --git a/vit-adapter_amd/csrc/tail_ops.hip b/vit-adapter_amd/csrc/tail_ops.hip
--- a/vit-adapter_amd/csrc/tail_ops.hip
+++ b/vit-adapter_amd/csrc/tail_ops.hip
@@ -6,6 +6,7 @@
 #include <cstring>
 
 #include "../../include/vitadapter_hip.h"
+#include "../../include/vitadapter_hip_epoch.h"
 #include "common.h"
 #include "elem16.h"
 
@@ -700,13 +701,10 @@
     }
 }
 
-__global__ __launch_bounds__(256) void bn_finalize_kernel(const float *__restrict__ sums, int C, float eps, float momentum,
-                                                          float *__restrict__ running_mean,
-                                                          float *__restrict__ running_var, float *__restrict__ mean,
-                                                          float *__restrict__ rstd) {
-    const int c = blockIdx.x * 256 + threadIdx.x;
-    if (c >= C) return;
-    const float count = sums[2 * C];
+__device__ __forceinline__ void bn_finalize_channel(const float *__restrict__ sums, int C, int c, float count, float eps,
+                                                    float momentum, float *__restrict__ running_mean,
+                                                    float *__restrict__ running_var, float *__restrict__ mean,
+                                                    float *__restrict__ rstd) {
     const float mu = sums[c] / count;
     const float var = nanmax(sums[C + c] / count - mu * mu, 0.f);
     mean[c] = mu;
@@ -714,6 +712,29 @@
     if (running_mean) {
         running_mean[c] = (1.f - momentum) * running_mean[c] + momentum * mu;
         running_var[c] = (1.f - momentum) * running_var[c] + momentum * var * (count / fmaxf(count - 1.f, 1.f));
+    }
+}
+
+__global__ __launch_bounds__(256) void bn_finalize_kernel(const float *__restrict__ sums, int C, float eps, float momentum,
+                                                          float *__restrict__ running_mean,
+                                                          float *__restrict__ running_var, float *__restrict__ mean,
+                                                          float *__restrict__ rstd) {
+    const int c = blockIdx.x * 256 + threadIdx.x;
+    if (c >= C) return;
+    bn_finalize_channel(sums, C, c, sums[2 * C], eps, momentum, running_mean, running_var, mean, rstd);
+}
+
+__global__ __launch_bounds__(256) void bn_finalize_book_kernel(float *__restrict__ sums, int C, float count, float eps,
+                                                               float momentum, float *__restrict__ running_mean,
+                                                               float *__restrict__ running_var, float *__restrict__ mean,
+                                                               float *__restrict__ rstd,
+                                                               int64_t *__restrict__ num_batches_tracked) {
+    const int c = blockIdx.x * 256 + threadIdx.x;
+    if (c >= C) return;
+    bn_finalize_channel(sums, C, c, count, eps, momentum, running_mean, running_var, mean, rstd);
+    if (c == 0) {
+        sums[2 * C] = count;
+        if (num_batches_tracked) *num_batches_tracked += 1;
     }
 }
 
@@ -1230,6 +1251,18 @@
     return check_launch(fn);
 }
 
+int vah_bn_finalize_stats_book(float *sums, int64_t C, float count, float eps, float momentum, float *running_mean,
+                               float *running_var, float *mean, float *rstd, int64_t *num_batches_tracked, void *stream) {
+    using namespace vah;
+    clear_error();
+    const char *fn = "vah_bn_finalize_stats_book";
+    if (C < 1 || C > (1 << 24)) return fail(VAH_E_SHAPE, "%s: bad C", fn);
+    if (!sums || !mean || !rstd || ((running_mean != nullptr) != (running_var != nullptr))) return fail(VAH_E_NULL, "%s: null pointer", fn);
+    hipLaunchKernelGGL(bn_finalize_book_kernel, dim3((unsigned)((C + 255) / 256)), dim3(256), 0, (hipStream_t)stream, sums, (int)C,
+                       count, eps, momentum, running_mean, running_var, mean, rstd, num_batches_tracked);
+    return check_launch(fn);
+}
+
 int vah_transpose_tokens(const void *src, int64_t B, int64_t T_total, int64_t t0, int64_t T, int64_t C, void *dst,
                          int to_planes, int planes_bf16, const float *vec, void *stream) {
     return vah::transpose_tokens_launch<__bf16>("vah_transpose_tokens", src, B, T_total, t0, T, C, dst, to_planes, planes_bf16, vec,
diff --git a/vit-adapter_amd/vitadapter/fused.py b/vit-adapter_amd/vitadapter/fused.py
--- a/vit-adapter_amd/vitadapter/fused.py
+++ b/vit-adapter_amd/vitadapter/fused.py
@@ -17,7 +17,8 @@
            'point_loss': True,
            'point_mask_loss': True,
            'seg_logits': True,
-           'seg_ce_loss': True}
+           'seg_ce_loss': True,
+           'epoch_copies': True}
 for _k in os.environ.get('VAH_FUSED_DISABLE', '').split(','):
     if _k:
         ENABLED[_k.strip()] = False
@@ -173,18 +174,39 @@
 
     def __init__(self):
         self.entries = {}
+        self.layouts = {}
         self.epoch = 0
 
-    def get(self, p, dtype=torch.bfloat16):
+    def _hit(self, p, dtype):
         e = self.entries.get((id(p), dtype))
         if (e is not None and e[2] == self.epoch and (self.epoch & 1) and e[0]() is p and e[1].device == p.device
                 and e[1].dtype == dtype):
             return e[1]
+        return None
+
+    def get(self, p, dtype=torch.bfloat16):
+        c = self._hit(p, dtype)
+        if c is not None:
+            return c
+        base = p._base
+        if base is not None and base.numel() == p.numel() and p.is_contiguous() and p.storage_offset() == base.storage_offset():
+            c = self._hit(base, dtype)
+            if c is not None:
+                return c.view(p.shape)
         return p.detach().to(dtype)
+
+    def layout(self, kind, p, dtype):
+        e = self.layouts.get((kind, id(p), dtype))
+        if e is not None and e[2] == self.epoch and (self.epoch & 1) and e[0]() is p:
+            return e[1]
+        return None
+
+    def open(self):
+        self.epoch += 1 if (self.epoch & 1) == 0 else 2
 
     def begin(self, params, dtype=torch.bfloat16):
         import weakref
-        self.epoch += 1 if (self.epoch & 1) == 0 else 2
+        self.open()
         if not params:
             return
         flat = torch.empty(sum(p.numel() for p in params), dtype=dtype, device=params[0].device)
@@ -267,7 +289,8 @@
             module.__dict__['_vah_linear_params'] = params
         live = [p for p in params if p.dtype == torch.float32 and p.is_cuda]
         if live:
-            BF16_COPIES.begin(live, t16)
+            if not (ENABLED['epoch_copies'] and EPOCH_COPIES.begin(module, t16, live[0].device)):
+                BF16_COPIES.begin(live, t16)
             SIDE.begin_epoch()
             BIAS_PARTIALS.begin_epoch()
             if module.training:
@@ -348,7 +371,7 @@
 gemm_bf16 = gemm_16
 
 
-def _wgrad_bgrad(g2, x2, partials=None):
+def _wgrad_bgrad(g2, x2, partials=None, row_map=None):
     import ctypes
     R, N = g2.shape
     K = x2.shape[1]
@@ -368,9 +391,20 @@
         else:
             cws, nparts = _scratch(N, dev), ctypes.c_int64(0)
             _vah.call('vah_colsum_bf16_partials', t16, g2.data_ptr(), R, N, cws.data_ptr(), ctypes.byref(nparts), st)
+        if row_map is not None:
+            applied = ctypes.c_int(0)
+            fn = _vah.lib.vah_gemm_bf16_fin_rowmap if t16 == torch.bfloat16 else _vah.lib.vah_gemm_f16_fin_rowmap
+            _vah.check(fn(1, 0, N, K, R, g2.data_ptr(), N, x2.data_ptr(), K, gw.data_ptr(), K, 1, ws.data_ptr(), ws_bytes,
+                          cws.data_ptr(), nparts.value, N, gb.data_ptr(), row_map.data_ptr(), ctypes.byref(applied), st), fn.__name__)
+            return gw, gb, bool(applied.value)
         _vah.call('vah_gemm_bf16_fin', t16, 1, 0, N, K, R, g2.data_ptr(), N, x2.data_ptr(), K, gw.data_ptr(), K, 1, ws.data_ptr(), ws_bytes,
                   cws.data_ptr(), nparts.value, N, gb.data_ptr(), st)
     return gw, gb
+
+
+def _wgrad_bgrad_mapped(g2, x2, row_map):
+    assert row_map.dtype == torch.int32 and row_map.numel() == g2.shape[1] and row_map.is_contiguous() and row_map.device == g2.device
+    return _wgrad_bgrad(g2, x2, None, row_map)
 
 
 class _SideStream:
@@ -669,6 +703,24 @@
     def __init__(self):
         self.entries = {}
 
+    def perm(self, a, b, M):
+        e = self.entries.get((id(a.weight), id(b.weight)))
+        na, nb = a.weight.shape[0], b.weight.shape[0]
+        po, pl = na // M, nb // M
+        dev = a.weight.device
+        if e is not None and e[4]() is a.weight and e[3][0].device == dev and e[3][0].numel() == na + nb:
+            return e[3]
+        fw = torch.cat([torch.cat((torch.arange(m * po, (m + 1) * po), na + torch.arange(m * pl, (m + 1) * pl))) for m in range(M)])
+        inv = torch.empty_like(fw)
+        inv[fw] = torch.arange(fw.numel())
+        return (fw.to(dev), inv.to(dev), fw.to(torch.int32).to(dev))
+
+    def put(self, a, b, epoch, w, bias, perm):
+        import weakref
+        if len(self.entries) > 1024:
+            self.entries.clear()
+        self.entries[(id(a.weight), id(b.weight))] = (epoch, w, bias, perm, weakref.ref(a.weight))
+
     def get(self, a, b, M):
         key = (id(a.weight), id(b.weight))
         epoch = BF16_COPIES.epoch
@@ -676,16 +728,7 @@
         if e is not None and e[0] == epoch and (epoch & 1) and e[1].device == a.weight.device and e[4]() is a.weight:
             return e[1], e[2], e[3]
         import weakref
-        na, nb = a.weight.shape[0], b.weight.shape[0]
-        po, pl = na // M, nb // M
-        dev = a.weight.device
-        if e is not None and e[4]() is a.weight and e[3][0].device == dev and e[3][0].numel() == na + nb:
-            perm = e[3]
-        else:
-            fw = torch.cat([torch.cat((torch.arange(m * po, (m + 1) * po), na + torch.arange(m * pl, (m + 1) * pl))) for m in range(M)])
-            inv = torch.empty_like(fw)
-            inv[fw] = torch.arange(fw.numel())
-            perm = (fw.to(dev), inv.to(dev))
+        perm = self.perm(a, b, M)
         with torch.no_grad():
             w = torch.cat([a.weight.detach(), b.weight.detach()], 0).index_select(0, perm[0]).to(torch.bfloat16)
             bias = torch.cat([a.bias.detach(), b.bias.detach()], 0).float().index_select(0, perm[0])
@@ -696,6 +739,166 @@
 
 
 PAIR_CORE_COPIES = _PairCoreCopies()
+
+
+class _EpochTable:
+
+    def __init__(self, dtype, device):
+        self.dtype, self.device = dtype, device
+        self.rows, self.params, self.sig, self.serve = [], [], [], []
+        self.n16 = self.n32 = 0
+        self.jobs = self.chunks = None
+        self.nchunks = 0
+
+    def valid(self):
+        for p, (ptr, shape, dtype) in zip(self.params, self.sig):
+            if p.data_ptr() != ptr or p.shape != shape or p.dtype != dtype:
+                return False
+        return True
+
+    def uses(self, p):
+        if not any(q is p for q in self.params):
+            self.params.append(p)
+            self.sig.append((p.data_ptr(), p.shape, p.dtype))
+
+    def alloc(self, n, f32=False):
+        if f32:
+            off, self.n32 = self.n32, self.n32 + (n + 7) // 8 * 8
+        else:
+            off, self.n16 = self.n16, self.n16 + (n + 7) // 8 * 8
+        return off
+
+    def job(self, p, src_off, dst, dims, strides, lims=None, f32=False):
+        dims, strides = (1,) * (4 - len(dims)) + tuple(dims), (0,) * (4 - len(strides)) + tuple(strides)
+        lims = dims if lims is None else (1,) * (4 - len(lims)) + tuple(lims)
+        n = dims[0] * dims[1] * dims[2] * dims[3]
+        assert 0 < n < 2 ** 31 and p.dtype == torch.float32 and p.is_contiguous() and 0 <= src_off < p.numel()
+        last = sum((min(d, l) - 1) * s for d, l, s in zip(dims, lims, strides))
+        assert min(strides) >= 0 and src_off + last < p.numel(), 'a job reads past its parameter'
+        packed = (dims[1] * dims[2] * dims[3], dims[2] * dims[3], dims[3], 1)
+        dense = all(d == 1 or s == c for d, s, c in zip(dims, strides, packed)) and all(l >= d for l, d in zip(lims, dims))
+        self.uses(p)
+        self.rows.append([p.data_ptr() + 4 * src_off, dst, n, dims[1], dims[2], dims[3], *strides, *lims,
+                          (1 if dense else 0) | (2 if f32 else 0), p.numel() - src_off])
+
+    def finish(self):
+        chunk = int(_vah.lib.vah_epoch_chunk_elems())
+        assert _vah.lib.vah_epoch_job_bytes() == 16 * 8
+        if not self.rows:
+            return self
+        jobs = torch.tensor(self.rows, dtype=torch.int64)
+        counts = (jobs[:, 2] + chunk - 1) // chunk
+        job_of = torch.repeat_interleave(torch.arange(len(self.rows)), counts)
+        first = torch.cumsum(counts, 0) - counts
+        k = torch.arange(job_of.numel()) - first[job_of]
+        self.chunks = torch.stack([job_of, k], 1).to(torch.int32).contiguous().to(self.device)
+        self.jobs = jobs.to(self.device)
+        self.nchunks = int(job_of.numel())
+        return self
+
+
+class _EpochCopies:
+
+    ATTR = '_vah_epoch_tables'
+
+    @staticmethod
+    def _ok(p, dev):
+        return (isinstance(p, torch.Tensor) and p.dtype == torch.float32 and p.device == dev and p.is_contiguous()
+                and 0 < p.numel() < 2 ** 31)
+
+    def build(self, module, t16, dev):
+        nn = torch.nn
+        tab = _EpochTable(t16, dev)
+        plain = set()
+
+        def add_plain(p):
+            if self._ok(p, dev) and id(p) not in plain:
+                plain.add(id(p))
+                off = tab.alloc(p.numel())
+                tab.job(p, 0, off, (p.numel(),), (1,))
+                tab.serve.append(('plain', p, off))
+
+        for m in module.modules():
+            if isinstance(m, nn.Linear):
+                add_plain(m.weight)
+                add_plain(m.bias)
+            elif isinstance(m, nn.ConvTranspose2d):
+                w = m.weight
+                if (m.kernel_size == (2, 2) and m.stride == (2, 2) and m.padding == (0, 0) and m.output_padding == (0, 0)
+                        and m.groups == 1 and m.dilation == (1, 1) and self._ok(w, dev)):
+                    C, Co = w.shape[0], w.shape[1]
+                    off = tab.alloc(w.numel())
+                    tab.job(w, 0, off, (2, 2, Co, C), (2, 1, 4, Co * 4))
+                    tab.serve.append(('up', w, off, (4 * Co, C)))
+            elif isinstance(m, nn.Conv2d) and m.groups == 1 and m.dilation == (1, 1) and self._ok(m.weight, dev):
+                w, k = m.weight, m.kernel_size
+                Co, Ci = w.shape[0], w.shape[1]
+                if k == (3, 3) and m.padding == (1, 1) and m.bias is None:
+                    cin = (Ci + 15) // 16 * 16
+                    o9, ot9 = tab.alloc(Co * 9 * cin), tab.alloc(cin * 9 * Co)
+                    tab.job(w, 0, o9, (Co, 3, 3, cin), (Ci * 9, 3, 1, 9), (Co, 3, 3, Ci))
+                    tab.job(w, 0, ot9, (cin, 3, 3, Co), (9, 3, 1, Ci * 9), (Ci, 3, 3, Co))
+                    tab.serve.append(('conv9', w, o9, (Co, 9, cin), ot9, (cin, 9, Co)))
+                elif t16 == torch.bfloat16 and m.padding == (0, 0) and k == m.stride:
+                    add_plain(w)
+            a, b = getattr(m, 'sampling_offsets', None), getattr(m, 'attention_weights', None)
+            M = getattr(m, 'n_heads', None)
+            if (t16 == torch.bfloat16 and type(a) is nn.Linear and type(b) is nn.Linear and isinstance(M, int) and M > 0
+                    and all(self._ok(p, dev) for p in (a.weight, a.bias, b.weight, b.bias))
+                    and a.weight.shape[1] == b.weight.shape[1] and a.weight.shape[0] % M == 0 and b.weight.shape[0] % M == 0):
+                na, nb, K = a.weight.shape[0], b.weight.shape[0], a.weight.shape[1]
+                po, pl = na // M, nb // M
+                ow, ob = tab.alloc((na + nb) * K), tab.alloc(na + nb, f32=True)
+                for h in range(M):
+                    r = h * (po + pl)
+                    tab.job(a.weight, h * po * K, ow + r * K, (po * K,), (1,))
+                    tab.job(b.weight, h * pl * K, ow + (r + po) * K, (pl * K,), (1,))
+                    tab.job(a.bias, h * po, ob + r, (po,), (1,), f32=True)
+                    tab.job(b.bias, h * pl, ob + r + po, (pl,), (1,), f32=True)
+                tab.serve.append(('pair_core', a, b, ow, (na + nb, K), ob, PAIR_CORE_COPIES.perm(a, b, M)))
+        return tab.finish()
+
+    def begin(self, module, t16, dev):
+        tables = module.__dict__.setdefault(self.ATTR, {})
+        tab = tables.get((t16, dev))
+        if tab is None or not tab.valid():
+            if torch.cuda.is_current_stream_capturing():
+                return False
+            tab = tables[(t16, dev)] = self.build(module, t16, dev)
+        if tab.nchunks == 0:
+            return False
+        import weakref
+        out16 = torch.empty(tab.n16, dtype=t16, device=dev)
+        out32 = torch.empty(max(tab.n32, 8), dtype=torch.float32, device=dev)
+        with _vah.on(dev):
+            _vah.check(_vah.lib.vah_epoch_copies(tab.jobs.data_ptr(), tab.jobs.shape[0], tab.chunks.data_ptr(), tab.nchunks,
+                                                 1 if t16 == torch.bfloat16 else 2, out16.data_ptr(), tab.n16, out32.data_ptr(),
+                                                 tab.n32, _vah.raw_stream(dev)), 'epoch_copies')
+        cp = BF16_COPIES
+        cp.open()
+        epoch = cp.epoch
+        if len(cp.entries) > 4096:
+            cp.entries = {k: v for k, v in cp.entries.items() if v[0]() is not None}
+        if len(cp.layouts) > 1024:
+            cp.layouts = {k: v for k, v in cp.layouts.items() if v[0]() is not None}
+        for s in tab.serve:
+            kind, p = s[0], s[1]
+            if kind == 'plain':
+                cp.entries[(id(p), t16)] = (weakref.ref(p), out16[s[2]:s[2] + p.numel()].view(p.shape), epoch)
+            elif kind == 'up':
+                n = s[3][0] * s[3][1]
+                cp.layouts[('up', id(p), t16)] = (weakref.ref(p), out16[s[2]:s[2] + n].view(s[3]), epoch)
+            elif kind == 'conv9':
+                n = s[3][0] * s[3][1] * s[3][2]
+                cp.layouts[('conv9', id(p), t16)] = (weakref.ref(p), (out16[s[2]:s[2] + n].view(s[3]), out16[s[4]:s[4] + n].view(s[5])),
+                                                     epoch)
+            else:
+                a, b, ow, wshape, ob, perm = s[1:]
+                PAIR_CORE_COPIES.put(a, b, epoch, out16[ow:ow + wshape[0] * wshape[1]].view(wshape), out32[ob:ob + wshape[0]], perm)
+        return True
+
+
+EPOCH_COPIES = _EpochCopies()
 
 
 class _MSDAPairCore(torch.autograd.Function):
@@ -719,7 +922,7 @@
         refc = ref.detach().float().contiguous().view(ref.shape[0], Lq, -1, ref.shape[-1])
         out = mf.fused_forward(value, shapes, lsi, offsets, logits, PS, PS, refc, carrier=ref if refc.shape[0] == 1 else None,
                                token=BF16_COPIES.epoch)
-        ctx.save_for_backward(x2, w, y, value, shapes, lsi, refc, perm[1])
+        ctx.save_for_backward(x2, w, y, value, shapes, lsi, refc, perm[1], perm[2])
         ctx.dims = (N, Lq, M, L, P, wa.shape[0])
         ctx.in_shape, ctx.in_dtype = query.shape, query.dtype
         return out
@@ -727,7 +930,7 @@
     @staticmethod
     @torch.autograd.function.once_differentiable
     def backward(ctx, gout):
-        x2, w, y, value, shapes, lsi, refc, inv = ctx.saved_tensors
+        x2, w, y, value, shapes, lsi, refc, inv, row_map = ctx.saved_tensors
         N, Lq, M, L, P, na = ctx.dims
         S, D = value.shape[1], value.shape[3]
         PS = 3 * L * P
@@ -751,8 +954,12 @@
             if gx.dtype != ctx.in_dtype:
                 gx = gx.to(ctx.in_dtype)
         if any(ctx.needs_input_grad[5:9]):
-            gwp, gbp = _wgrad_bgrad(g, x2)
-            gw, gbias = gwp.index_select(0, inv), gbp.index_select(0, inv)
+            if ENABLED['epoch_copies']:
+                gw, gbias, mapped = _wgrad_bgrad_mapped(g, x2, row_map)
+            else:
+                (gw, gbias), mapped = _wgrad_bgrad(g, x2), False
+            if not mapped:
+                gw, gbias = gw.index_select(0, inv), gbias.index_select(0, inv)
         return (gx, grad_value if ctx.needs_input_grad[1] else None, None, None, None,
                 gw[:na] if gw is not None else None, gbias[:na] if gbias is not None else None,
                 gw[na:] if gw is not None else None, gbias[na:] if gbias is not None else None, None, None, None, None)
@@ -821,13 +1028,16 @@
         B, T, C = rows.shape
         Co = weight.shape[1]
         xb = rows.detach().to(t16).contiguous()
+        wc = BF16_COPIES.layout('up', weight, t16)
         if t16 == torch.bfloat16:
-            wc = BF16_COPIES.get(weight).permute(2, 3, 1, 0).reshape(4 * Co, C).contiguous()
+            if wc is None:
+                wc = BF16_COPIES.get(weight).permute(2, 3, 1, 0).reshape(4 * Co, C).contiguous()
             U = torch.empty((B, 4 * Co, T), dtype=torch.bfloat16, device=rows.device)
             for b in range(B):
                 gemm_16(wc, xb[b], trans_b=True, out=U[b])
         else:
-            wc = weight.detach().to(t16).permute(2, 3, 1, 0).reshape(4 * Co, C).contiguous()
+            if wc is None:
+                wc = weight.detach().to(t16).permute(2, 3, 1, 0).reshape(4 * Co, C).contiguous()
             U = torch.bmm(wc.unsqueeze(0).expand(B, 4 * Co, C), xb.transpose(1, 2))
         out = torch.empty((B, Co, 2 * h, 2 * w), dtype=t16, device=rows.device)
         add = addend.contiguous() if addend is not None else None
@@ -1135,6 +1345,32 @@
     return group if data_parallel.one_rank_group() else None
 
 
+def bn_finalize(norm, sums, C, count, group, st):
+    dev = sums.device
+    mean = torch.empty(C, dtype=torch.float32, device=dev)
+    rstd = torch.empty(C, dtype=torch.float32, device=dev)
+    track = norm.running_mean is not None
+    rm = norm.running_mean.data_ptr() if track else None
+    rv = norm.running_var.data_ptr() if track else None
+    nbt = norm.num_batches_tracked if track else None
+    if (group is None and ENABLED['epoch_copies']
+            and (nbt is None or (nbt.dtype == torch.int64 and nbt.device == dev and nbt.numel() == 1))):
+        _vah.check(_vah.lib.vah_bn_finalize_stats_book(
+            sums.data_ptr(), C, float(count), float(norm.eps), float(norm.momentum), rm, rv, mean.data_ptr(), rstd.data_ptr(),
+            nbt.data_ptr() if nbt is not None else None, st), 'bn_finalize_stats_book')
+        return mean, rstd, sums[2 * C:]
+    sums[2 * C:].fill_(float(count))
+    if group is not None:
+        import torch.distributed as dist
+        dist.all_reduce(sums, group=group)
+    _vah.check(_vah.lib.vah_bn_finalize_stats(sums.data_ptr(), C, float(norm.eps), float(norm.momentum), rm, rv, mean.data_ptr(),
+                                              rstd.data_ptr(), st), 'bn_finalize_stats')
+    if nbt is not None:
+        with torch.no_grad():
+            norm.num_batches_tracked += 1
+    return mean, rstd, sums[2 * C:]
+
+
 class _BNTail(torch.autograd.Function):
 
     @staticmethod
@@ -1158,21 +1394,7 @@
                 sums = torch.empty(2 * C + 1, dtype=torch.float32, device=dev)
                 ws = torch.empty(_vah.lib.vah_bn_tail_ws_floats(C), dtype=torch.float32, device=dev)
                 _vah.call('vah_bn_tail_stats', t16, *ops, shp, sums.data_ptr(), ws.data_ptr(), st)
-                sums[2 * C:].fill_(float(N * H * W))
-                if group is not None:
-                    import torch.distributed as dist
-                    dist.all_reduce(sums, group=group)
-                mean = torch.empty(C, dtype=torch.float32, device=dev)
-                rstd = torch.empty(C, dtype=torch.float32, device=dev)
-                track = norm.running_mean is not None
-                _vah.check(_vah.lib.vah_bn_finalize_stats(
-                    sums.data_ptr(), C, float(norm.eps), float(norm.momentum),
-                    norm.running_mean.data_ptr() if track else None, norm.running_var.data_ptr() if track else None,
-                    mean.data_ptr(), rstd.data_ptr(), st), 'bn_finalize_stats')
-                if track:
-                    with torch.no_grad():
-                        norm.num_batches_tracked += 1
-                count = sums[2 * C:]
+                mean, rstd, count = bn_finalize(norm, sums, C, N * H * W, group, st)
             else:
                 count = None
                 mean = norm.running_mean.float().contiguous()
diff --git a/vit-adapter_amd/vitadapter/spm_nhwc.py b/vit-adapter_amd/vitadapter/spm_nhwc.py
--- a/vit-adapter_amd/vitadapter/spm_nhwc.py
+++ b/vit-adapter_amd/vitadapter/spm_nhwc.py
@@ -24,12 +24,17 @@
     @staticmethod
     def forward(ctx, x, weight, stride):
         cin = x.shape[-1]
+        ctx.stride, ctx.wcin = stride, weight.shape[1]
+        made = fused.BF16_COPIES.layout('conv9', weight, x.dtype)
+        ctx.dgrad_ready = made is not None and made[0].shape[2] == cin
+        if ctx.dgrad_ready:
+            ctx.save_for_backward(x, made[1])
+            return conv.conv3x3_forward(x, made[0], stride)
         w = weight.detach()
         if w.shape[1] != cin:
             w = F.pad(w, (0, 0, 0, 0, 0, cin - w.shape[1]))
         wb = w.to(x.dtype)
         ctx.save_for_backward(x, wb)
-        ctx.stride, ctx.wcin = stride, weight.shape[1]
         return conv.conv3x3_forward(x, conv.forward_weight(wb, x.dtype), stride)
 
     @staticmethod
@@ -38,7 +43,8 @@
         gy = gy.contiguous().to(x.dtype)
         gx = gw = None
         if ctx.needs_input_grad[0]:
-            gx = conv.conv3x3_input_grad(gy, conv.dgrad_weight(wb, x.dtype), ctx.stride, x.shape[1:3])
+            wt9 = wb if ctx.dgrad_ready else conv.dgrad_weight(wb, x.dtype)
+            gx = conv.conv3x3_input_grad(gy, wt9, ctx.stride, x.shape[1:3])
         if ctx.needs_input_grad[1]:
             gw = conv.conv3x3_weight_grad(x, gy, ctx.stride).permute(0, 3, 1, 2)[:, :ctx.wcin].contiguous()
         return gx, gw, None
@@ -61,21 +67,7 @@
                 sums = torch.empty(2 * C + 1, dtype=torch.float32, device=dev)
                 ws = torch.empty(_vah.lib.vah_bn_nhwc_ws_floats(C), dtype=torch.float32, device=dev)
                 _vah.call('vah_bn_nhwc_stats', x.dtype, x.data_ptr(), rows, C, sums.data_ptr(), ws.data_ptr(), st)
-                sums[2 * C:].fill_(float(rows))
-                if group is not None:
-                    import torch.distributed as dist
-                    dist.all_reduce(sums, group=group)
-                mean = torch.empty(C, dtype=torch.float32, device=dev)
-                rstd = torch.empty(C, dtype=torch.float32, device=dev)
-                track = norm.running_mean is not None
-                _vah.check(_vah.lib.vah_bn_finalize_stats(
-                    sums.data_ptr(), C, float(norm.eps), float(norm.momentum),
-                    norm.running_mean.data_ptr() if track else None, norm.running_var.data_ptr() if track else None,
-                    mean.data_ptr(), rstd.data_ptr(), st), 'bn_finalize_stats')
-                if track:
-                    with torch.no_grad():
-                        norm.num_batches_tracked += 1
-                count = sums[2 * C:]
+                mean, rstd, count = fused.bn_finalize(norm, sums, C, rows, group, st)
             else:
                 count = None
                 mean = norm.running_mean.float().contiguous()
```

New measurement: 81.36 images/sec, median of 6. 1.4% higher.
